# kimwin2/ORB_SLAM2v2-1

Hardware: AMD Instinct MI355X
Metric: frames/s ORB extract+match @1241x376 8-lvl 1000-feat (higher is better)
Workload: dtype u8; 1 GPU; kitti_stereo_1241x376_1000feat; frame=stereo pair (2 images), width=1241, height=376, nlevels=8, nfeatures=1000, ini_th_fast=20, min_th_fast=7, clock_ramp_steps=200, match=Frame::ComputeStereoMatches, parallelism=frames sharded over 1 GPU(s), world_size_observed=1, gauss_flavour=half_up

## Files before the change

include/orbx_dev.h:

```cpp
#ifndef ORBX_DEV_H
#define ORBX_DEV_H
#include "orbx.h"
#ifdef __cplusplus
extern "C" {
#endif

int orbx_debug_level_points(orbx_extractor_t *h, int b, int level, int stage, int32_t *out_xys, int cap,
                            int *n_out);

int orbx_debug_blur_patches(orbx_extractor_t *h, int enable, uint8_t *out, int n);
int orbx_debug_octree_fallbacks(orbx_extractor_t *h, int32_t *out, int n);
int orbx_debug_blurred_level(orbx_extractor_t *h, int b, int level, uint8_t *dst, int dst_stride, unsigned *mask_out);
int orbm_debug_features_in_area(const orbx_keypoint_t *kun, int n, const orbm_grid_geom_t *g, float x, float y, float r,
                                int min_level, int max_level, int32_t *out_idx, int *n_out, int device);
int orbx_debug_sincosf(const float *angles, int n, float *sin_out, float *cos_out, int device);

#define ORBM_PATH_RES_NONE 0
#define ORBM_PATH_RES_PAR_Q2 1
#define ORBM_PATH_RES_PAR_Q4 2
#define ORBM_PATH_RES_WAVE 3
#define ORBM_PATH_RES_EXACT 4
#define ORBM_PATH_FB_NONE 0
#define ORBM_PATH_FB_N 1
#define ORBM_PATH_FB_INIT_SIZE 2
#define ORBM_PATH_FB_CAND_CAP 3
#define ORBM_PATH_FB_QK 4
#define ORBM_PATH_FB_LDS 5
#define ORBM_PATH_FB_OPTION 6
int orbm_debug_match_path(int64_t *out);
int orbm_debug_resolve_plan(int mode, int m, int n, int device, int64_t *out);
int orbm_debug_stereo_path(int32_t *out);

#define ORBX_DEBUG_PLAN_INPUT_INTS 64
#define ORBX_DEBUG_CHUNK_PLAN_INTS 43
int orbx_debug_plan_chunk(const int32_t *in, int n_in, int32_t *out, int n_out);
int orbx_debug_last_plan(const orbx_extractor_t *h, int32_t *out, int n_out);

#define ORBX_DEBUG_SIZE_PLAN_INTS 176
int orbx_debug_size_plan(int nfeatures, float scale_factor, int nlevels, int w, int h, int pyr_tile, float *tables, int32_t *nfeat_umax,
                         uint8_t *geom, int geom_bytes, int32_t *tab, int tab_cap, int64_t *scalars, int n_scalars);

#define ORBM_DEBUG_THREAD_SCRATCH_INTS 9
int orbm_debug_thread_scratch(int64_t *out, int n_out);

int orbx_debug_set_alloc_fill(int enable, uint32_t word);
int orbx_debug_alloc_fill_stats(int64_t out[2]);

int orbx_debug_stall_stream(void *stream, int microseconds, int device);
int orbx_debug_streams(orbx_extractor_t *h, void **out, int n_out);

#ifdef __cplusplus
}
#endif
#endif
```

orb_slam2v2-1_amd/__init__.py:

```python
import ctypes as C
import os
import numpy as np

_HERE = os.path.dirname(os.path.abspath(__file__))
LIB_PATH = os.environ.get("ORBX_LIB") or os.path.join(_HERE, "lib", "liborbx_hip.so")
DEV_LIB_PATH = os.path.join(_HERE, "lib", "liborbx_hip_dev.so")
default_developer = False

KP_DTYPE = np.dtype([("x", "<f4"), ("y", "<f4"), ("size", "<f4"), ("angle", "<f4"),
                     ("response", "<f4"), ("octave", "<i4"), ("class_id", "<i4")])
MP_DTYPE = np.dtype([("in_view", "<i4"), ("proj_x", "<f4"), ("proj_y", "<f4"), ("proj_xr", "<f4"),
                     ("level", "<i4"), ("view_cos", "<f4"), ("observations", "<i4")])
LASTPT_DTYPE = np.dtype([("has_mp", "<i4"), ("wx", "<f4"), ("wy", "<f4"), ("wz", "<f4"),
                         ("observations", "<i4"), ("octave", "<i4"), ("angle", "<f4")])
WINDOW_DTYPE = np.dtype([("valid", "<i4"), ("u", "<f4"), ("v", "<f4"), ("radius", "<f4"), ("min_level", "<i4"),
                         ("max_level", "<i4"), ("angle", "<f4"), ("blocks", "<i4"), ("ur_c", "<f4"), ("ur_tol", "<f4")])

CLOUD_DTYPE = np.dtype([("x", "<f4"), ("y", "<f4"), ("z", "<f4"), ("b", "u1"), ("g", "u1"), ("r", "u1"), ("a", "u1")])

OCTREE_LEAF_DTYPE = np.dtype([("kx", "<u2"), ("ky", "<u2"), ("kz", "<u2"), ("depth", "<u2")])
OCTOMAP_AXIS_SWAP = np.array([[0, 0, 1, 0], [-1, 0, 0, 0], [0, -1, 0, 0], [0, 0, 0, 1]], np.float32)
POSE_OBS_DTYPE = np.dtype([("valid", "<i4"), ("u", "<f4"), ("v", "<f4"), ("ur", "<f4"), ("inv_sigma2", "<f4"),
                           ("wx", "<f4"), ("wy", "<f4"), ("wz", "<f4")])
POSE_WORLDPOS_DTYPE = np.dtype([("valid", "<i4"), ("wx", "<f4"), ("wy", "<f4"), ("wz", "<f4")])
POSE_INFO_DTYPE = np.dtype({"names": ["correspondences", "bad", "iterations", "trials", "rounds", "t", "q"],
                            "formats": ["<i4", "<i4", ("<i4", 4), ("<i4", 4), "<i4", ("<f8", 3), ("<f8", 4)],
                            "offsets": [0, 4, 8, 24, 40, 48, 72], "itemsize": 104})
INIT_INFO_DTYPE = np.dtype([("SH", "<f4"), ("SF", "<f4"), ("RH", "<f4"), ("model", "<i4"), ("best_iteration", "<i4", (2,)),
                            ("inliers", "<i4", (2,)), ("best_good", "<i4"), ("second_good", "<i4"), ("parallax", "<f4"), ("ncand", "<i4"),
                            ("ngood", "<i4", (8,)), ("cand_parallax", "<f4", (8,)), ("H21", "<f4", (9,)), ("F21", "<f4", (9,))])
SIM3_PAIR_DTYPE = np.dtype([("w1", "<f4", (3,)), ("w2", "<f4", (3,)), ("sigma2_1", "<f4"), ("sigma2_2", "<f4")])
SIM3_PROBLEM_DTYPE = np.dtype([("Tcw1", "<f4", (16,)), ("Tcw2", "<f4", (16,)), ("K1", "<f4", (4,)), ("K2", "<f4", (4,)),
                               ("fix_scale", "<i4"), ("min_inliers", "<i4")])
SIM3_INFO_DTYPE = np.dtype([("n", "<i4"), ("iterations", "<i4"), ("hit_iteration", "<i4"), ("best_iteration", "<i4"),
                            ("best_inliers", "<i4"), ("s", "<f4"), ("R", "<f4", (9,)), ("t", "<f4", (3,)), ("T12", "<f4", (16,))])
SIM3OPT_MATCH_DTYPE = np.dtype([("w1", "<f4", (3,)), ("w2", "<f4", (3,)), ("u1", "<f4"), ("v1", "<f4"), ("u2", "<f4"), ("v2", "<f4"),
                                ("inv_sigma2_1", "<f4"), ("inv_sigma2_2", "<f4")])
SIM3OPT_PROBLEM_DTYPE = np.dtype([("Tcw1", "<f4", (16,)), ("Tcw2", "<f4", (16,)), ("K1", "<f4", (4,)), ("K2", "<f4", (4,)), ("s", "<f4"),
                                  ("R", "<f4", (9,)), ("t", "<f4", (3,)), ("th2", "<f4"), ("fix_scale", "<i4")])
SIM3OPT_INFO_DTYPE = np.dtype([("correspondences", "<i4"), ("bad", "<i4"), ("rounds", "<i4"), ("iterations", "<i4", (2,)),
                               ("trials", "<i4", (2,)), ("reserved", "<i4"), ("q", "<f8", (4,)), ("t", "<f8", (3,)), ("s", "<f8")])
LBA_KEYFRAME_DTYPE = np.dtype([("Tcw", "<f4", (16,)), ("fx", "<f4"), ("fy", "<f4"), ("cx", "<f4"), ("cy", "<f4"), ("bf", "<f4"), ("fixed", "<i4")])
LBA_POINT_DTYPE = np.dtype([("x", "<f4"), ("y", "<f4"), ("z", "<f4")])
LBA_OBSERVATION_DTYPE = np.dtype([("kf", "<i4"), ("pt", "<i4"), ("u", "<f4"), ("v", "<f4"), ("ur", "<f4"), ("inv_sigma2", "<f4")])
LBA_SCHEDULE_DTYPE = np.dtype([("rounds", "<i4"), ("iterations", "<i4", (2,)), ("robust", "<i4", (2,)), ("delta_mono", "<f4"), ("delta_stereo", "<f4"),
                               ("classify", "<i4"), ("check_stop_first", "<i4")])
LBA_INFO_DTYPE = np.dtype([("rounds", "<i4"), ("iterations", "<i4", (2,)), ("trials", "<i4", (2,)), ("free_poses", "<i4", (2,)), ("stopped_at", "<i4"),
                           ("stop_poll", "<i4"), ("polls", "<i4"), ("erased", "<i4")])
LBA_STOP_BEFORE, LBA_STOP_ROUND1, LBA_STOP_BETWEEN, LBA_STOP_ROUND2 = 1, 2, 3, 4
LBA_MAX_ITERATIONS = 100
EG_SIM3_DTYPE = np.dtype([("q", "<f8", (4,)), ("t", "<f8", (3,)), ("s", "<f8")])
EG_VERTEX_DTYPE = np.dtype([("Scw", EG_SIM3_DTYPE), ("Snc", EG_SIM3_DTYPE), ("has_nc", "<i4"), ("fixed", "<i4")])
EG_EDGE_DTYPE = np.dtype([("i", "<i4"), ("j", "<i4"), ("kind", "<i4")])
EG_POINT_DTYPE = np.dtype([("x", "<f4"), ("y", "<f4"), ("z", "<f4"), ("ref", "<i4")])
EG_MAX_ITERATIONS = 64
EG_INFO_DTYPE = np.dtype([("iterations", "<i4"), ("trials", "<i4"), ("end", "<i4"), ("free_vertices", "<i4"), ("blocks", "<i4"), ("levels", "<i4"),
                          ("launches", "<i4"), ("pad", "<i4"), ("chi2_first", "<f8"), ("chi2_last", "<f8"), ("trials_it", "<i4", (EG_MAX_ITERATIONS,))])
EG_END_ITERATIONS, EG_END_QMAX, EG_END_RHO0, EG_END_SOLVER, EG_END_NBAD = 0, 1, 2, 3, 4
NEWPOINT_VIEW_DTYPE = np.dtype([("Tcw", "<f4", (16,)), ("Ow", "<f4", (3,)), ("fx", "<f4"), ("fy", "<f4"), ("cx", "<f4"), ("cy", "<f4"),
                                ("invfx", "<f4"), ("invfy", "<f4"), ("mb", "<f4"), ("mbf", "<f4"), ("scale_factor", "<f4"), ("nlevels", "<i4")])
NEWPOINT_STEREO_DTYPE = np.dtype([("ur", "<f4"), ("depth", "<f4"), ("raw_u", "<f4"), ("raw_v", "<f4")])
NEWPOINT_DTYPE = np.dtype([("x", "<f4"), ("y", "<f4"), ("z", "<f4"), ("status", "<i4"), ("cos_rays", "<f4"), ("cos_stereo", "<f4"),
                           ("reserved", "<i4", (2,))])
NEWPOINT_TRIANGULATED, NEWPOINT_STEREO1, NEWPOINT_STEREO2 = 0, 1, 2
NEWPOINT_MAX_LEVELS = 16
PNP_CORR_DTYPE = np.dtype([("w", "<f4", (3,)), ("u", "<f4"), ("v", "<f4"), ("sigma2", "<f4")])
PNP_PROBLEM_DTYPE = np.dtype([("K", "<f4", (4,)), ("th2", "<f4"), ("min_inliers", "<i4"), ("max_iterations", "<i4"),
                              ("iterations_done", "<i4"), ("prior_best_inliers", "<i4")])
PNP_INFO_DTYPE = np.dtype([("n", "<i4"), ("iterations", "<i4"), ("hit_iteration", "<i4"), ("iterations_run", "<i4"),
                           ("best_iteration", "<i4"), ("best_inliers", "<i4"), ("refined_inliers", "<i4"), ("no_more", "<i4"),
                           ("pose", "<i4"), ("Tcw", "<f4", (16,)), ("best_Tcw", "<f4", (16,))])
PNP_POSE_NONE, PNP_POSE_REFINED, PNP_POSE_BEST, PNP_POSE_PRIOR_BEST = 0, 1, 2, 3
DB_HIT_DTYPE = np.dtype([("kf_id", "<i4"), ("words", "<i4"), ("flags", "<u4"), ("score", "<f4"), ("acc_score", "<f4"), ("best_kf", "<i4")])
DB_MAX_KF_ID, DB_MAX_QUERY, DB_MAX_COVISIBLE = (1 << 20) - 1, 8192, 10

ORBX_OK, ORBX_ERR_ARG, ORBX_ERR_NO_DEVICE, ORBX_ERR_HIP, ORBX_ERR_CAPACITY, ORBX_ERR_UNSUPPORTED = 0, -1, -2, -3, -4, -5
NUM_STAGES = 5

EXPORTS = [
    "orbx_create", "orbx_destroy", "orbx_get_levels", "orbx_get_scale_factor", "orbx_get_tables",
    "orbx_max_keypoints", "orbx_extract", "orbx_extract_batch", "orbx_extract_batch_device",
    "orbx_pyramid_host", "orbx_pyramid_device", "orbx_level_counts", "orbx_set_profiling",
    "orbx_get_stage_ms", "orbx_create_flavoured", "orbx_get_flavour", "orbx_set_option", "orbx_get_option", "orbm_set_thread_option", "orbm_hamming", "orbm_hamming_matrix_device", "orbm_stereo_batch_device",
    "orbm_stereo", "orbm_search_for_initialization", "orbm_search_by_projection_mp",
    "orbm_search_by_projection_frame", "orbm_match_windows", "orbm_best_in_windows", "orbm_distinctive_descriptors", "orbm_predict_scale_thresholds", "orbm_is_in_frustum",
    "orbm_search_local_points", "orbv_create", "orbv_load_text", "orbv_destroy", "orbv_info", "orbv_transform",
    "orbm_search_by_bow", "orbm_search_for_triangulation", "orbx_last_error", "orbx_version", "orbx_device_count",
    "orbx_record_bytes", "orbx_pack_records_device", "orbx_thread_release_scratch",
    "orbm_search_by_projection_frame_device", "orbm_search_local_points_device", "orbx_fast_kernels", "orbx_extract_batch_device_prefetch", "orbx_stream_wait_fast_stage", "orbx_side_stream", "orbm_stereo_batch_device_prev",
    "orbx_side_stream_for", "orbx_stereo_frame", "orbx_set_pyramid_buffers",
    "orbx_stereo_frame_view", "orbx_host_alloc", "orbx_host_free",
    "orbx_gray_from_color_device", "orbm_rgbd_batch_device", "orbx_rgbd_frame",
    "orbx_rectifier_create", "orbx_rectifier_destroy", "orbx_rectifier_maps", "orbx_rectifier_info", "orbx_rectify_device",
    "orbx_stereo_frame_rectified", "orbx_stereo_frame_view_rectified",
    "orbx_cloudmapper_create", "orbx_cloudmapper_destroy", "orbx_cloud_capacity", "orbx_cloud_generate_device",
    "orbx_cloud_voxel_device", "orbx_keyframe_cloud",
    "orbx_octree_device", "orbx_octomap_bt", "orbx_octomap_bytes_bound",
    "orbv_score_l1", "orbv_db_create", "orbv_db_destroy", "orbv_db_add", "orbv_db_erase", "orbv_db_clear", "orbv_db_set_covisible",
    "orbv_db_info", "orbv_db_score", "orbv_db_detect_loop", "orbv_db_detect_reloc",
]
POSE_EXPORTS = ["orbo_pose_optimization", "orbo_pose_optimization_batch", "orbo_pose_optimization_device"]
INIT_EXPORTS = ["orbi_initialize", "orbi_initialize_device", "orbi_search"]
SIM3_EXPORTS = ["orbs_sim3_iterations", "orbs_sim3_ransac", "orbs_sim3_ransac_batch"]
PNP_EXPORTS = ["orbp_pnp_parameters", "orbp_pnp_ransac", "orbp_pnp_ransac_batch"]
SIM3OPT_EXPORTS = ["orbz_optimize_sim3", "orbz_optimize_sim3_batch"]
NEWPOINTS_EXPORTS = ["orbl_triangulate", "orbl_triangulate_batch", "orbl_baseline_ok", "orbl_compute_f12", "orbl_create_new_map_points"]
LBA_EXPORTS = ["orbb_optimize", "orbb_local_bundle_adjustment", "orbb_bundle_adjustment"]
ESSENTIAL_EXPORTS = ["orbg_optimize_essential_graph"]
DEV_EXPORTS = ["orbx_debug_level_points", "orbx_debug_sincosf", "orbx_debug_blur_patches", "orbm_debug_features_in_area",
               "orbx_debug_blurred_level", "orbx_debug_octree_fallbacks", "orbm_debug_match_path", "orbm_debug_resolve_plan",
               "orbm_debug_stereo_path", "orbx_debug_plan_chunk", "orbx_debug_last_plan", "orbm_debug_thread_scratch",
               "orbx_debug_size_plan", "orbx_debug_set_alloc_fill", "orbx_debug_alloc_fill_stats", "orbx_debug_stall_stream",
               "orbx_debug_streams"]
SIZE_PLAN_FIELDS = ["max_kp", "totalCells", "maxNodeCap", "lvlKpCap", "pyrImgBytes", "slotsPerImg", "keysPerImg", "fastTileStride", "fastScoreStride",
                    "fastTileRows", "fastLdsPerWave", "totalStrips", "stripLevels", "octLdsBytes", "octPyrLdsBytes", "octPyrWords", "octBigMask",
                    "octDeepMax", "octSliceStride", "histStride", "pyrTilesX", "pyrTilesY", "pyrXSpanOff", "pyrYSpanOff", "pyrBufBytes", "pyrMaxDim",
                    "pyrMaxPar", "pyrLdsBytes", "nChains0", "nChains1", "tabWords"]
LEVEL_GEOM_DTYPE = np.dtype([("w", "<i4"), ("h", "<i4"), ("pstride", "<i4"), ("prows", "<i4"), ("poff", "<u8"), ("regW", "<i4"), ("regH", "<i4"),
                             ("nCols", "<i4"), ("nRows", "<i4"), ("wCell", "<i4"), ("hCell", "<i4"), ("cellBase", "<i4"), ("ncells", "<i4"),
                             ("capc", "<i4"), ("pad_", "<i4"), ("slotOff", "<u8"), ("N", "<i4"), ("nIni", "<i4"), ("nodeCap", "<i4"),
                             ("pyrDepth", "<i4"), ("keyOff", "<u8"), ("keyCap", "<i4"), ("lvlKpOff", "<i4"), ("xofsOff", "<i4"), ("xalphaOff", "<i4"),
                             ("yofsOff", "<i4"), ("ybetaOff", "<i4"), ("rootTabOff", "<i4"), ("rootBoxOff", "<i4"), ("xPathOff", "<i4"),
                             ("yPathOff", "<i4"), ("scale", "<f4"), ("size", "<f4")])
THREAD_SCRATCH_FIELDS = ["arena_cap", "arena_device", "arena_seq", "arena_stream", "arena_word", "stage_cap", "stage_device", "bow_cap",
                         "bow_device"]
PLAN_INPUT_FIELDS = ["B", "nl", "totalStrips", "stripLevels", "octBigMask", "lastChunks", "prof", "profFast", "skipPyr", "pfUsed", "evPyrDone",
                     "dbgBlur", "sliceScratch", "fastTileStride", "fastScoreStride", "sparseRecent"]
CHUNK_PLAN_FIELDS = ["usePyr", "strips", "stripLevels", "fastCells", "es", "histOct", "multiWg", "fused", "gather", "bigMask", "wideOct", "compact",
                     "sparseForm", "sparsePerCell", "rowFlags", "sparseHint", "earlyLv", "aSplit", "octForm", "sweepSlices", "sweepShared",
                     "orderKernel", "fastDoneAt", "fastPhase", "octPhase", "octStop", "descLdsPad"]
OCT_EXACT, OCT_BIG, OCT_EARLY, OCT_SPLIT, OCT_SINGLE = 0, 1, 2, 3, 4
HINT_NONE, HINT_OCT_SRC, HINT_GATHER = 0, 1, 2
RES_NONE, RES_PAR_Q2, RES_PAR_Q4, RES_WAVE, RES_EXACT = 0, 1, 2, 3, 4
FB_NONE, FB_N, FB_INIT_SIZE, FB_CAND_CAP, FB_QK, FB_LDS, FB_OPTION = 0, 1, 2, 3, 4, 5, 6


class OrbxError(RuntimeError):
    def __init__(self, status, msg):
        super().__init__("orbx status %d: %s" % (status, msg))
        self.status = status


class StereoView(C.Structure):
    _fields_ = [("nl", C.c_int32), ("nr", C.c_int32), ("nmatch", C.c_int32), ("cap", C.c_int32),
                ("kl", C.c_void_p), ("kr", C.c_void_p), ("dl", C.c_void_p), ("dr", C.c_void_p), ("uright", C.c_void_p), ("depth", C.c_void_p),
                ("d_kl", C.c_void_p), ("d_kr", C.c_void_p), ("d_dl", C.c_void_p), ("d_dr", C.c_void_p), ("d_uright", C.c_void_p),
                ("d_depth", C.c_void_p)]


class OctreeInfo(C.Structure):
    _fields_ = [("points_in", C.c_int64), ("points_dropped", C.c_int64), ("cells", C.c_int64), ("leaves", C.c_int64),
                ("tree_size", C.c_int64), ("data_bytes", C.c_int64), ("overflow", C.c_int32), ("reserved", C.c_int32)]

    def as_dict(self):
        return {f: int(getattr(self, f)) for f, _ in self._fields_ if f != "reserved"}


class GridGeom(C.Structure):
    _fields_ = [("min_x", C.c_float), ("min_y", C.c_float), ("max_x", C.c_float), ("max_y", C.c_float),
                ("inv_w", C.c_float), ("inv_h", C.c_float)]


class Camera(C.Structure):
    _fields_ = [("fx", C.c_float), ("fy", C.c_float), ("cx", C.c_float), ("cy", C.c_float),
                ("mbf", C.c_float), ("mb", C.c_float)]


class RGBDCamera(C.Structure):
    _fields_ = [("fx", C.c_float), ("fy", C.c_float), ("cx", C.c_float), ("cy", C.c_float), ("k1", C.c_float), ("k2", C.c_float),
                ("p1", C.c_float), ("p2", C.c_float), ("k3", C.c_float), ("mbf", C.c_float)]


DEPTH_U16, DEPTH_F32 = 2, 5
_DEPTH_TYPES = {np.dtype(np.uint16): DEPTH_U16, np.dtype(np.float32): DEPTH_F32}


def grid_geom(w, h):
    g = GridGeom()
    g.min_x, g.min_y, g.max_x, g.max_y = 0.0, 0.0, float(w), float(h)
    g.inv_w = np.float32(64) / np.float32(w)
    g.inv_h = np.float32(48) / np.float32(h)
    return g


class Flavour(C.Structure):
    _fields_ = [("gauss_rounding", C.c_int32), ("gauss_taps", C.c_int32 * 4), ("reserved", C.c_int32 * 3)]


GAUSS_FLAVOURS = {"half_up": 0, "sse2": 1}
GAUSS_FIXED_TAPS = 2


def parse_gauss(g):
    fl = Flavour()
    if isinstance(g, str) and g.startswith("taps:"):
        taps = [int(v) for v in g[5:].split(",")]
        if len(taps) != 4:
            raise ValueError("bad gauss flavour %r (taps:k0,k1,k2,k3)" % (g,))
        fl.gauss_rounding = GAUSS_FIXED_TAPS
        for i, v in enumerate(taps):
            fl.gauss_taps[i] = v
    elif g in GAUSS_FLAVOURS:
        fl.gauss_rounding = GAUSS_FLAVOURS[g]
    else:
        raise ValueError("bad gauss flavour %r" % (g,))
    return fl
default_gauss_flavour = os.environ.get("ORBX_TEST_GAUSS_FLAVOUR", "half_up")
_default_options = {}
_live = None


def set_default_option(key, value):
    if value:
        _default_options[int(key)] = int(value)
    else:
        _default_options.pop(int(key), None)
    for e in list(_live or ()):
        if getattr(e, "_h", None):
            e.set_option(key, value)


_lib = None
_dev_lib = None


def build(force=False):
    from . import build as _b
    return _b.build(force=force)


def _preload_shared_hip_runtime():
    import importlib.util
    import sys
    if "torch" in sys.modules:
        return
    try:
        spec = importlib.util.find_spec("torch")
    except (ImportError, ValueError):
        spec = None
    if spec and spec.submodule_search_locations:
        cand = os.path.join(list(spec.submodule_search_locations)[0], "lib", "libamdhip64.so")
        if os.path.exists(cand):
            try:
                C.CDLL(cand, mode=C.RTLD_GLOBAL)
            except OSError:
                pass


def lib(developer=False):
    global _lib, _dev_lib
    if developer:
        if _dev_lib is None:
            _dev_lib = _load(DEV_LIB_PATH, True)
        return _dev_lib
    if _lib is None:
        _lib = _load(LIB_PATH, os.path.basename(LIB_PATH) == "liborbx_hip_dev.so")
    return _lib


LBA_STOP_FN = C.CFUNCTYPE(C.c_int, C.c_void_p)


def matcher_lib():
    return lib(default_developer)


def _load(path, dev):
    if not os.path.exists(path):
        raise OrbxError(ORBX_ERR_NO_DEVICE, "HIP library %s is missing: run `python __graft_entry__.py` "
                                            "(build()) first; there is no CPU fallback" % path)
    _preload_shared_hip_runtime()
    L = C.CDLL(path)
    vp, i32, f32, sz = C.c_void_p, C.c_int, C.c_float, C.c_size_t
    L.orbx_create.restype = i32
    L.orbx_create.argtypes = [i32, f32, i32, i32, i32, i32, C.POINTER(vp)]
    L.orbx_destroy.argtypes = [vp]
    L.orbx_create_flavoured.argtypes = [i32, f32, i32, i32, i32, i32, C.POINTER(Flavour), C.POINTER(vp)]
    L.orbx_get_flavour.argtypes = [vp, C.POINTER(Flavour)]
    L.orbx_set_option.argtypes = [vp, i32, i32]
    L.orbx_get_option.argtypes = [vp, i32, C.POINTER(i32)]
    L.orbm_set_thread_option.argtypes = [i32, i32]
    L.orbx_get_levels.argtypes = [vp]
    L.orbx_get_scale_factor.restype = f32
    L.orbx_get_scale_factor.argtypes = [vp]
    L.orbx_get_tables.argtypes = [vp, vp, vp, vp, vp, vp, vp]
    L.orbx_max_keypoints.argtypes = [vp]
    L.orbx_extract.argtypes = [vp, vp, i32, i32, i32, vp, vp, i32, C.POINTER(i32)]
    L.orbx_extract_batch.argtypes = [vp, vp, i32, i32, i32, i32, vp, vp, i32, vp]
    L.orbx_extract_batch_device.argtypes = [vp, vp, i32, i32, i32, i32, sz, vp, vp, vp, i32, vp]
    L.orbx_extract_batch_device_prefetch.argtypes = [vp, vp, i32, i32, i32, i32, sz, vp]
    L.orbx_stream_wait_fast_stage.argtypes = [vp, vp]
    L.orbx_side_stream.argtypes = [vp]
    L.orbx_side_stream.restype = vp
    L.orbx_stereo_frame.argtypes = [vp, vp, vp, i32, i32, i32, f32, f32, i32, vp, vp, C.POINTER(i32), vp, vp, C.POINTER(i32), vp, vp,
                                    C.POINTER(i32)]
    L.orbx_stereo_frame_view.argtypes = [vp, vp, vp, i32, i32, i32, f32, f32, vp]
    L.orbx_gray_from_color_device.argtypes = [vp, i32, i32, i32, i32, i32, i32, sz, vp, i32, sz, vp]
    L.orbm_rgbd_batch_device.argtypes = [vp, vp, i32, i32, vp, i32, i32, i32, i32, sz, f32, C.POINTER(RGBDCamera), vp, vp, vp, vp]
    L.orbx_rgbd_frame.argtypes = [vp, vp, i32, i32, i32, i32, i32, vp, i32, i32, f32, C.POINTER(RGBDCamera), i32, vp, vp,
                                  C.POINTER(i32), vp, vp, vp]
    L.orbx_rectifier_create.argtypes = [vp, vp, i32, vp, vp, i32, i32, i32, C.POINTER(vp)]
    L.orbx_rectifier_destroy.argtypes = [vp]
    L.orbx_rectifier_maps.argtypes = [vp, vp, vp]
    L.orbx_rectifier_info.argtypes = [vp, C.POINTER(i32), C.POINTER(i32), C.POINTER(sz)]
    L.orbx_rectify_device.argtypes = [vp, vp, i32, vp, i32, i32, i32, i32, i32, i32, sz, vp, i32, sz, vp]
    L.orbx_stereo_frame_rectified.argtypes = [vp, vp, vp, vp, vp, i32, i32, i32, i32, i32, f32, f32, i32, vp, vp, C.POINTER(i32), vp, vp,
                                              C.POINTER(i32), vp, vp, C.POINTER(i32)]
    L.orbx_stereo_frame_view_rectified.argtypes = [vp, vp, vp, vp, vp, i32, i32, i32, i32, i32, f32, f32, vp]
    L.orbx_cloudmapper_create.argtypes = [f32, i32, i32, i32, C.POINTER(vp)]
    L.orbx_cloudmapper_destroy.argtypes = [vp]
    L.orbx_cloud_capacity.argtypes = [i32, i32, i32]
    L.orbx_cloud_generate_device.argtypes = [vp, vp, i32, i32, sz, f32, vp, i32, i32, sz, i32, i32, i32, f32, f32, f32, f32, vp, vp, i32, vp, vp]
    L.orbx_cloud_voxel_device.argtypes = [vp, vp, vp, i32, i32, vp, i32, vp, vp]
    L.orbx_keyframe_cloud.argtypes = [vp, vp, i32, i32, vp, i32, i32, f32, i32, i32, f32, f32, f32, f32, vp, i32, vp, C.POINTER(i32), vp,
                                      C.POINTER(i32)]
    L.orbx_octree_device.argtypes = [vp, vp, vp, i32, i32, vp, C.c_double, vp, C.c_int64, vp, C.c_int64, vp, vp]
    L.orbx_octomap_bt.argtypes = [vp, vp, i32, vp, C.c_double, vp, sz, C.POINTER(sz), C.POINTER(OctreeInfo)]
    L.orbx_octomap_bytes_bound.argtypes = [C.c_int64]
    L.orbx_octomap_bytes_bound.restype = sz
    L.orbx_host_alloc.argtypes = [sz]
    L.orbx_host_alloc.restype = vp
    L.orbx_host_free.argtypes = [vp]
    L.orbx_host_free.restype = None
    L.orbx_set_pyramid_buffers.argtypes = [vp, i32]
    L.orbx_side_stream_for.argtypes = [vp, vp]
    L.orbx_side_stream_for.restype = vp
    L.orbx_pyramid_host.argtypes = [vp, i32, i32, i32, vp, i32, C.POINTER(i32), C.POINTER(i32)]
    L.orbx_pyramid_device.argtypes = [vp, i32, i32, C.POINTER(vp), C.POINTER(i32), C.POINTER(i32), C.POINTER(i32)]
    L.orbx_level_counts.argtypes = [vp, i32, vp, vp]
    L.orbx_set_profiling.argtypes = [vp, i32]
    L.orbx_fast_kernels.argtypes = [vp, i32, C.POINTER(i32), C.POINTER(i32), C.POINTER(i32)]
    L.orbx_record_bytes.argtypes = [i32]
    L.orbx_pack_records_device.argtypes = [vp, vp, vp, vp, vp, i32, i32, vp, vp]
    L.orbx_get_stage_ms.argtypes = [vp, vp, C.POINTER(i32)]
    L.orbm_hamming.argtypes = [vp, vp]
    L.orbm_hamming_matrix_device.argtypes = [vp, i32, vp, i32, vp, vp]
    L.orbm_stereo_batch_device.argtypes = [vp, vp, i32, i32, i32, vp, vp, vp, vp, vp, vp, i32, f32, f32, vp, vp, vp, vp]
    L.orbm_stereo_batch_device_prev.argtypes = L.orbm_stereo_batch_device.argtypes
    L.orbm_stereo.argtypes = [vp, vp, vp, vp, i32, vp, vp, i32, f32, f32, vp, vp, C.POINTER(i32)]
    L.orbm_search_for_initialization.argtypes = [vp, vp, i32, vp, vp, i32, C.POINTER(GridGeom), vp, vp, i32, f32,
                                                 i32, i32, C.POINTER(i32)]
    L.orbm_search_by_projection_mp.argtypes = [vp, vp, vp, i32, C.POINTER(GridGeom), vp, i32, vp, vp, i32, vp, vp,
                                               f32, f32, i32, C.POINTER(i32)]
    L.orbm_search_by_projection_frame.argtypes = [vp, vp, vp, i32, C.POINTER(GridGeom), vp, i32, C.POINTER(Camera),
                                                  vp, vp, vp, vp, i32, vp, vp, f32, i32, i32, i32, C.POINTER(i32)]
    L.orbm_search_by_projection_frame_device.argtypes = L.orbm_search_by_projection_frame.argtypes + [vp]
    L.orbm_match_windows.argtypes = [vp, vp, vp, i32, C.POINTER(GridGeom), C.POINTER(GridGeom), vp, vp, i32, vp, vp, i32, i32, i32, C.POINTER(i32)]
    L.orbm_distinctive_descriptors.argtypes = [vp, vp, i32, vp, vp, i32]
    L.orbm_predict_scale_thresholds.argtypes = [f32, i32, vp]
    L.orbv_create.argtypes = [i32, i32, i32, i32, i32, vp, vp, vp, vp, i32, C.POINTER(vp)]
    L.orbv_load_text.argtypes = [C.c_char_p, i32, C.POINTER(vp)]
    L.orbv_destroy.argtypes = [vp]
    L.orbv_destroy.restype = None
    L.orbv_info.argtypes = [vp] + [C.POINTER(i32)] * 6
    L.orbv_transform.argtypes = [vp, vp, i32, i32, vp, vp, vp]
    L.orbv_score_l1.argtypes = [vp, vp, i32, vp, vp, i32, vp]
    L.orbv_db_create.argtypes = [i32, i32, i32, C.POINTER(vp)]
    L.orbv_db_destroy.argtypes = [vp]
    L.orbv_db_destroy.restype = None
    L.orbv_db_add.argtypes = [vp, i32, vp, vp, i32]
    L.orbv_db_erase.argtypes = [vp, i32]
    L.orbv_db_clear.argtypes = [vp]
    L.orbv_db_set_covisible.argtypes = [vp, i32, vp, i32]
    L.orbv_db_info.argtypes = [vp, C.POINTER(i32), C.POINTER(C.c_int64), C.POINTER(C.c_int64), C.POINTER(sz)]
    L.orbv_db_score.argtypes = [vp, vp, vp, i32, vp, i32, vp]
    L.orbv_db_detect_loop.argtypes = [vp, vp, vp, i32, vp, i32, f32, vp, i32, C.POINTER(i32), vp, i32, C.POINTER(i32)]
    L.orbv_db_detect_reloc.argtypes = [vp, vp, vp, i32, vp, i32, C.POINTER(i32), vp, i32, C.POINTER(i32)]
    L.orbm_search_for_triangulation.argtypes = [vp, vp, vp, i32, vp, vp, vp, i32, vp, vp, vp, vp, i32, vp, f32, f32, vp, vp, i32, i32, i32, vp,
                                                C.POINTER(i32), i32]
    L.orbm_search_by_bow.argtypes = [vp, vp, vp, i32, vp, vp, vp, i32, vp, vp, vp, vp, i32, i32, f32, i32, vp, C.POINTER(i32), i32]
    L.orbm_is_in_frustum.argtypes = [vp, i32, vp, C.POINTER(Camera), C.POINTER(GridGeom), f32, vp, i32, vp, i32]
    L.orbm_search_local_points.argtypes = [vp, vp, vp, i32, C.POINTER(GridGeom), vp, i32, vp, vp, i32, vp, C.POINTER(Camera), f32,
                                           vp, vp, vp, f32, f32, i32, C.POINTER(i32), vp]
    L.orbm_search_local_points_device.argtypes = L.orbm_search_local_points.argtypes + [vp]
    L.orbo_pose_optimization.argtypes = [vp, i32, C.POINTER(Camera), vp, vp, vp, C.POINTER(i32), vp, i32]
    L.orbo_pose_optimization_batch.argtypes = [vp, vp, i32, vp, vp, vp, vp, vp, vp, i32]
    L.orbo_pose_optimization_device.argtypes = [vp, vp, i32, vp, i32, vp, C.POINTER(Camera), vp, vp, vp, C.POINTER(i32), vp, i32, vp]
    L.orbm_best_in_windows.argtypes = [vp, vp, vp, i32, C.POINTER(GridGeom), C.POINTER(GridGeom), vp, vp, i32, vp, i32, vp, vp, i32]
    L.orbi_initialize.argtypes = [vp, i32, vp, i32, vp, i32, vp, i32, vp, f32, f32, i32, C.POINTER(i32), vp, vp, vp, vp, vp, i32]
    L.orbi_initialize_device.argtypes = L.orbi_initialize.argtypes + [vp]
    L.orbi_search.argtypes = [vp, i32, vp, i32, vp, i32, vp, i32, f32, vp, vp, vp, vp, i32]
    L.orbs_sim3_iterations.argtypes = [i32, C.c_double, i32, i32]
    L.orbs_sim3_ransac.argtypes = [vp, i32, vp, vp, i32, vp, vp, vp, vp, vp, i32]
    L.orbs_sim3_ransac_batch.argtypes = [vp, vp, i32, vp, vp, vp, vp, vp, vp, vp, vp, i32]
    L.orbz_optimize_sim3.argtypes = [vp, i32, vp, vp, vp, C.POINTER(i32), vp, i32]
    L.orbz_optimize_sim3_batch.argtypes = [vp, vp, i32, vp, vp, vp, vp, vp, i32]
    L.orbl_triangulate.argtypes = [vp, vp, vp, i32, vp, vp, vp, vp, vp, i32, vp, vp, vp, i32, vp, C.POINTER(i32), i32]
    L.orbl_triangulate_batch.argtypes = [vp, vp, i32, vp, vp, vp, vp, i32]
    L.orbl_baseline_ok.argtypes = [vp, vp, i32, f32]
    L.orbl_compute_f12.argtypes = [vp, vp, vp, vp, vp]
    L.orbl_create_new_map_points.argtypes = [vp, vp, vp, vp, i32, i32, i32, i32, vp, vp, vp, vp, vp, vp, i32]
    L.orbb_optimize.argtypes = [vp, i32, vp, i32, vp, i32, vp, LBA_STOP_FN, vp, vp, vp, vp, vp, vp, vp, i32]
    L.orbb_local_bundle_adjustment.argtypes = [vp, i32, vp, i32, vp, i32, LBA_STOP_FN, vp, vp, vp, vp, vp, vp, vp, i32]
    L.orbb_bundle_adjustment.argtypes = [vp, i32, vp, i32, vp, i32, i32, i32, LBA_STOP_FN, vp, vp, vp, vp, vp, vp, i32]
    L.orbg_optimize_essential_graph.argtypes = [vp, i32, vp, i32, vp, i32, i32, i32, vp, vp, vp, vp, i32]
    L.orbp_pnp_parameters.argtypes = [i32, C.c_double, i32, i32, i32, f32, C.POINTER(i32), C.POINTER(i32)]
    L.orbp_pnp_ransac.argtypes = [vp, i32, vp, vp, i32, vp, vp, vp, vp, vp, vp, vp, vp, vp, vp, i32]
    L.orbp_pnp_ransac_batch.argtypes = [vp, vp, i32, vp, vp, vp, vp, vp, vp, vp, vp, vp, vp, vp, vp, vp, i32]
    if dev:
        L.orbx_debug_level_points.argtypes = [vp, i32, i32, i32, vp, i32, C.POINTER(i32)]
        L.orbx_debug_sincosf.argtypes = [vp, i32, vp, vp, i32]
        L.orbx_debug_blur_patches.argtypes = [vp, i32, vp, i32]
        L.orbx_debug_octree_fallbacks.argtypes = [vp, vp, i32]
        L.orbx_debug_blurred_level.argtypes = [vp, i32, i32, vp, i32, vp]
        L.orbm_debug_features_in_area.argtypes = [vp, i32, C.POINTER(GridGeom), f32, f32, f32, i32, i32, vp, C.POINTER(i32), i32]
        L.orbm_debug_match_path.argtypes = [vp]
        L.orbm_debug_resolve_plan.argtypes = [i32, i32, i32, i32, vp]
        L.orbm_debug_stereo_path.argtypes = [vp]
        L.orbx_debug_plan_chunk.argtypes = [vp, i32, vp, i32]
        L.orbx_debug_last_plan.argtypes = [vp, vp, i32]
        L.orbm_debug_thread_scratch.argtypes = [vp, i32]
        L.orbx_debug_size_plan.argtypes = [i32, f32, i32, i32, i32, i32, vp, vp, vp, i32, vp, i32, vp, i32]
        L.orbx_debug_set_alloc_fill.argtypes = [i32, C.c_uint32]
        L.orbx_debug_alloc_fill_stats.argtypes = [vp]
        L.orbx_debug_stall_stream.argtypes = [vp, i32, i32]
        L.orbx_debug_streams.argtypes = [vp, vp, i32]
    L.orbx_last_error.restype = C.c_char_p
    L.orbx_version.restype = C.c_char_p
    L._orbx_developer = bool(dev)
    return L


def _check(rc, L=None):
    if rc != 0:
        raise OrbxError(rc, (L or matcher_lib()).orbx_last_error().decode())


def _p(a):
    return a.ctypes.data if a is not None else None


def blur_reach_mask():
    d = np.abs(np.arange(-18, 19))
    t = np.where(d > 0, 2 * d - 1, 0)
    return (t[:, None] ** 2 + t[None, :] ** 2) <= 4 * 340


def device_count():
    return lib().orbx_device_count()


class ORBextractor:

    def __init__(self, nfeatures, scaleFactor, nlevels, iniThFAST, minThFAST, device=0, gauss=None, developer=None):
        global _live
        self._L = lib(default_developer if developer is None else developer)
        h = C.c_void_p()
        self.gauss = default_gauss_flavour if gauss is None else gauss
        fl = parse_gauss(self.gauss)
        self._ck(self._L.orbx_create_flavoured(int(nfeatures), float(scaleFactor), int(nlevels), int(iniThFAST),
                                             int(minThFAST), int(device), C.byref(fl), C.byref(h)))
        self._h = h
        self.nfeatures, self.nlevels, self.device = int(nfeatures), int(nlevels), int(device)
        self._shape = None
        if _live is None:
            import weakref
            _live = weakref.WeakSet()
        _live.add(self)
        for k, v in _default_options.items():
            self.set_option(k, v)

    def _ck(self, rc):
        _check(rc, self._L)

    def _hooks(self):
        if not self._L._orbx_developer:
            raise OrbxError(ORBX_ERR_ARG, "stage hooks (debug_*) exist in the developer build only: ORBextractor(..., developer=True)")

    def level_counts(self, b=0):
        c, k = np.zeros(self.nlevels, np.int32), np.zeros(self.nlevels, np.int32)
        self._ck(self._L.orbx_level_counts(self._h, int(b), _p(c), _p(k)))
        return c, k

    def set_option(self, key, value):
        self._ck(self._L.orbx_set_option(self._h, int(key), int(value)))

    def get_option(self, key):
        v = C.c_int(0)
        self._ck(self._L.orbx_get_option(self._h, int(key), C.byref(v)))
        return v.value

    def flavour(self):
        fl = Flavour()
        self._ck(self._L.orbx_get_flavour(self._h, C.byref(fl)))
        if fl.gauss_rounding == GAUSS_FIXED_TAPS:
            return "taps:" + ",".join(str(int(v)) for v in fl.gauss_taps)
        return {v: k for k, v in GAUSS_FLAVOURS.items()}[fl.gauss_rounding]

    def close(self):
        if getattr(self, "_h", None):
            self._L.orbx_destroy(self._h)
            self._h = None

    def __del__(self):
        try:
            self.close()
        except Exception:
            pass

    def GetLevels(self):
        return self._L.orbx_get_levels(self._h)

    def GetScaleFactor(self):
        return self._L.orbx_get_scale_factor(self._h)

    def _tables(self):
        n = self.nlevels
        t = [np.zeros(n, np.float32) for _ in range(4)] + [np.zeros(n, np.int32), np.zeros(16, np.int32)]
        self._ck(self._L.orbx_get_tables(self._h, *[_p(a) for a in t]))
        return t

    def GetScaleFactors(self): return self._tables()[0]
    def GetInverseScaleFactors(self): return self._tables()[1]
    def GetScaleSigmaSquares(self): return self._tables()[2]
    def GetInverseScaleSigmaSquares(self): return self._tables()[3]
    @property
    def mnFeaturesPerLevel(self): return self._tables()[4]
    @property
    def umax(self): return self._tables()[5]

    def max_keypoints(self):
        return self._L.orbx_max_keypoints(self._h)

    def __call__(self, image):
        image = np.asarray(image)
        if image.size == 0:
            return np.zeros(0, KP_DTYPE), np.zeros((0, 32), np.uint8)
        assert image.dtype == np.uint8 and image.ndim == 2, "CV_8UC1 expected (:1050)"
        if image.strides[1] != 1 or image.strides[0] < image.shape[1]:
            image = np.ascontiguousarray(image)
        h, w = image.shape
        cap = max(self.nfeatures + 8 * self.nlevels, 64) + 260
        kps = np.zeros(cap, KP_DTYPE)
        desc = np.zeros((cap, 32), np.uint8)
        n = C.c_int(0)
        self._ck(self._L.orbx_extract(self._h, _p(image), w, h, image.strides[0], _p(kps), _p(desc), cap, C.byref(n)))
        self._shape = (h, w)
        return kps[:n.value].copy(), desc[:n.value].copy()

    def extract_batch(self, images):
        images = np.ascontiguousarray(images, dtype=np.uint8)
        B, h, w = images.shape
        cap = max(self.nfeatures + 8 * self.nlevels, 64) + 260
        kps = np.zeros((B, cap), KP_DTYPE)
        desc = np.zeros((B, cap, 32), np.uint8)
        n = np.zeros(B, np.int32)
        ptrs = (C.c_void_p * B)(*[images[b].ctypes.data for b in range(B)])
        self._ck(self._L.orbx_extract_batch(self._h, C.cast(ptrs, C.c_void_p), B, w, h, w, _p(kps), _p(desc), cap, _p(n)))
        self._shape = (h, w)
        return [(kps[b, :n[b]].copy(), desc[b, :n[b]].copy()) for b in range(B)]

    def extract_batch_device(self, d_imgs, B, w, h, stride, image_stride, d_kps, d_desc, d_counts, cap, stream=0):
        self._ck(self._L.orbx_extract_batch_device(self._h, d_imgs, B, w, h, stride, image_stride, d_kps, d_desc,
                                                 d_counts, cap, stream))
        self._shape = (h, w)

    def prefetch_batch_device(self, d_imgs, B, w, h, stride, image_stride, side_stream=0):
        self._ck(self._L.orbx_extract_batch_device_prefetch(self._h, d_imgs, B, w, h, stride, image_stride, side_stream))

    def side_stream(self):
        return self._L.orbx_side_stream(self._h)

    def stereo_frame(self, left, right, mbf, mb):
        left = np.ascontiguousarray(left, np.uint8); right = np.ascontiguousarray(right, np.uint8)
        assert left.shape == right.shape and left.ndim == 2
# ... 106 lines not shown
        self._ck(self._L.orbx_stereo_frame_view_rectified(self._h, _rect_handle(rect_left), _rect_handle(rect_right), la[0], ra[0],
                                                          int(ch), int(bool(rgb)), w, hgt, w * ch if stride is None else int(stride),
                                                          float(mbf), float(mb), C.byref(v)))
        self._shape = (hgt, w)
        a, b = v.nl, v.nr
        view = lambda p, n, dt: np.frombuffer((C.c_char * (n * np.dtype(dt).itemsize)).from_address(p), dt) if n > 0 else np.zeros(0, dt)
        return {"kl": view(v.kl, a, KP_DTYPE), "dl": view(v.dl, a * 32, np.uint8).reshape(a, 32), "kr": view(v.kr, b, KP_DTYPE),
                "dr": view(v.dr, b * 32, np.uint8).reshape(b, 32), "uright": view(v.uright, a, np.float32),
                "depth": view(v.depth, a, np.float32), "nmatch": v.nmatch, "view": v}

    def set_pyramid_buffers(self, n):
        self._ck(self._L.orbx_set_pyramid_buffers(self._h, int(n)))

    def side_stream_for(self, main_stream):
        return self._L.orbx_side_stream_for(self._h, main_stream)

    def stream_wait_fast_stage(self, stream):
        self._ck(self._L.orbx_stream_wait_fast_stage(self._h, stream))

    def pyramid_level(self, level, b=0, padded=False):
        w, h = C.c_int(), C.c_int()
        self._ck(self._L.orbx_pyramid_host(self._h, b, level, int(padded), None, 0, C.byref(w), C.byref(h)))
        out = np.zeros((h.value, w.value), np.uint8)
        self._ck(self._L.orbx_pyramid_host(self._h, b, level, int(padded), _p(out), w.value, C.byref(w), C.byref(h)))
        return out

    @property
    def mvImagePyramid(self):
        return [self.pyramid_level(l) for l in range(self.nlevels)]

    def pyramid_device(self, level, b=0):
        ptr, w, h, s = C.c_void_p(), C.c_int(), C.c_int(), C.c_int()
        self._ck(self._L.orbx_pyramid_device(self._h, b, level, C.byref(ptr), C.byref(w), C.byref(h), C.byref(s)))
        return ptr.value, w.value, h.value, s.value

    def debug_level_points(self, level, stage, b=0):
        self._hooks()
        n = C.c_int()
        self._ck(self._L.orbx_debug_level_points(self._h, b, level, stage, None, 0, C.byref(n)))
        out = np.zeros((max(n.value, 1), 3), np.int32)
        if n.value:
            self._ck(self._L.orbx_debug_level_points(self._h, b, level, stage, _p(out), n.value, C.byref(n)))
        return out[:n.value]

    def fast_kernels(self, B):
        st, ce, ipl = C.c_int(0), C.c_int(0), C.c_int(0)
        self._ck(self._L.orbx_fast_kernels(self._h, int(B), C.byref(st), C.byref(ce), C.byref(ipl)))
        self.fast_images_per_launch = ipl.value
        return [n for n, f in (("k_fast_strips", st.value), ("k_fast_cells", ce.value)) if f]

    def octree_fallbacks(self, B=1):
        self._hooks()
        out = np.zeros((B, self.nlevels), np.int32)
        self._ck(self._L.orbx_debug_octree_fallbacks(self._h, _p(out), B * self.nlevels))
        return out

    def blurred_mask(self):
        m = C.c_uint()
        self._ck(self._L.orbx_debug_blurred_level(self._h, 0, 0, None, 0, C.byref(m)))
        return m.value

    def blurred_level(self, level, b=0):
        self._hooks()
        w, h = C.c_int(), C.c_int()
        self._ck(self._L.orbx_pyramid_host(self._h, b, level, 0, None, 0, C.byref(w), C.byref(h)))
        out = np.zeros((h.value, w.value), np.uint8)
        self._ck(self._L.orbx_debug_blurred_level(self._h, b, level, _p(out), w.value, None))
        return out

    def debug_blur_patches(self, image):
        self._hooks()
        self._ck(self._L.orbx_debug_blur_patches(self._h, 1, None, 0))
        try:
            k, d = self(image)
            out = np.zeros((max(len(k), 1), 37, 37), np.uint8)
            if len(k):
                self._ck(self._L.orbx_debug_blur_patches(self._h, 1, _p(out), len(k)))
        finally:
            self._L.orbx_debug_blur_patches(self._h, 0, None, 0)
        return k, d, out[:len(k)]

    def debug_last_plan(self):
        self._hooks()
        out = np.zeros(len(CHUNK_PLAN_FIELDS) + 16, np.int32)
        self._ck(self._L.orbx_debug_last_plan(self._h, _p(out), len(out)))
        return _plan_dict(out)

    def set_profiling(self, mode=1):
        self._ck(self._L.orbx_set_profiling(self._h, int(mode)))

    def stage_ms(self):
        ms = np.zeros(NUM_STAGES, np.float32)
        n = C.c_int(0)
        self._ck(self._L.orbx_get_stage_ms(self._h, _p(ms), C.byref(n)))
        return ms, n.value


def debug_features_in_area(kun, geom, x, y, r, min_level=-1, max_level=-1, device=0):
    kun = np.ascontiguousarray(kun, KP_DTYPE)
    out = np.zeros(max(len(kun), 1), np.int32)
    n = C.c_int(0)
    _check(lib(True).orbm_debug_features_in_area(_p(kun), len(kun), C.byref(geom), float(x), float(y), float(r), int(min_level),
                                             int(max_level), _p(out), C.byref(n), int(device)), lib(True))
    return out[:n.value].copy()


def debug_match_path():
    out = np.zeros(3, np.int64)
    _check(lib(True).orbm_debug_match_path(_p(out)), lib(True))
    return int(out[0]), int(out[1]), int(out[2])


def debug_resolve_plan(mode, m, n, device=0):
    out = np.zeros(4, np.int64)
    _check(lib(True).orbm_debug_resolve_plan(int(mode), int(m), int(n), int(device), _p(out)), lib(True))
    return tuple(int(v) for v in out)


def _plan_dict(out):
    d = {k: int(v) for k, v in zip(CHUNK_PLAN_FIELDS, out)}
    d["nslice"] = tuple(int(v) for v in out[len(CHUNK_PLAN_FIELDS):])
    return d


def debug_plan_chunk(ncells=(), opt=None, **fields):
    a = np.zeros(len(PLAN_INPUT_FIELDS) + 16 + 32, np.int32)
    for k, v in fields.items():
        a[PLAN_INPUT_FIELDS.index(k)] = int(v)
    a[len(PLAN_INPUT_FIELDS):len(PLAN_INPUT_FIELDS) + len(ncells)] = ncells
    for k, v in (opt or {}).items():
        a[len(PLAN_INPUT_FIELDS) + 16 + int(k)] = int(v)
    out = np.zeros(len(CHUNK_PLAN_FIELDS) + 16, np.int32)
    rc = lib(True).orbx_debug_plan_chunk(_p(a), len(a), _p(out), len(out))
    return rc, _plan_dict(out)


def debug_size_plan(nfeatures, scale_factor, nlevels, w, h, tile=0):
    L = lib(True)
    tables, nu = np.zeros((4, 16), np.float32), np.zeros(32, np.int32)
    geom, sc = np.zeros(16, LEVEL_GEOM_DTYPE), np.zeros(len(SIZE_PLAN_FIELDS) + 17 + 128, np.int64)
    tab = np.zeros(0, np.int32)
    for _ in range(2):
        rc = L.orbx_debug_size_plan(nfeatures, scale_factor, nlevels, w, h, tile, _p(tables), _p(nu), _p(geom), geom.nbytes, _p(tab), len(tab),
                                    _p(sc), len(sc))
        if rc != ORBX_OK or len(tab) == sc[SIZE_PLAN_FIELDS.index("tabWords")]:
            break
        tab = np.zeros(int(sc[SIZE_PLAN_FIELDS.index("tabWords")]), np.int32)
    d = dict(status=rc, message=L.orbx_last_error().decode() if rc else "", sf=tables[0], isf=tables[1], sig2=tables[2], isig2=tables[3],
             nfeat=nu[:16], umax=nu[16:])
    if rc == ORBX_OK:
        n = len(SIZE_PLAN_FIELDS)
        d.update({k: int(v) for k, v in zip(SIZE_PLAN_FIELDS, sc)}, geom=geom, tab=tab, stripBase=sc[n:n + 17].astype(np.int32),
                 chains=sc[n + 17:].astype(np.int32).reshape(2, 8, 8))
    return d


def debug_thread_scratch():
    out = np.zeros(len(THREAD_SCRATCH_FIELDS), np.int64)
    _check(lib(True).orbm_debug_thread_scratch(_p(out), len(out)), lib(True))
    return {k: int(v) for k, v in zip(THREAD_SCRATCH_FIELDS, out)}


def debug_set_alloc_fill(enable, word=0):
    _check(lib(True).orbx_debug_set_alloc_fill(int(bool(enable)), int(word) & 0xFFFFFFFF), lib(True))


def debug_alloc_fill_stats():
    out = np.zeros(2, np.int64)
    _check(lib(True).orbx_debug_alloc_fill_stats(_p(out)), lib(True))
    return int(out[0]), int(out[1])


def debug_stall_stream(stream, microseconds, device=0):
    _check(lib(True).orbx_debug_stall_stream(int(stream) if stream else None, int(microseconds), int(device)), lib(True))


DEBUG_STREAM_FIELDS = ("main", "side0", "side1", "arena", "staging")


def debug_streams(extractor=None):
    if extractor is not None:
        extractor._hooks()
    out = (C.c_void_p * 5)()
    _check(lib(True).orbx_debug_streams(extractor._h if extractor is not None else None, out, 5), lib(True))
    return {k: int(v or 0) for k, v in zip(DEBUG_STREAM_FIELDS, out)}


def debug_stereo_path():
    out = np.zeros(4, np.int32)
    _check(lib(True).orbm_debug_stereo_path(_p(out)), lib(True))
    return tuple(int(v) for v in out)


def debug_sincosf(angles, device=0):
    a = np.ascontiguousarray(angles, np.float32)
    s, c = np.zeros_like(a), np.zeros_like(a)
    _check(lib(True).orbx_debug_sincosf(_p(a), len(a), _p(s), _p(c), int(device)), lib(True))
    return s, c


def pack_records_device(d_kps, d_desc, d_uright, d_depth, d_counts, B, cap, d_records, stream=0):
    _check(lib().orbx_pack_records_device(d_kps, d_desc, d_uright, d_depth, d_counts, B, cap, d_records, stream))


def stereo_batch_device(ex_left, ex_right, B, left_slot0, right_slot0, d_kl, d_dl, d_nl, d_kr, d_dr, d_nr, cap,
                        mbf, mb, d_uright, d_depth, d_nmatch, stream=0, prev=False):
    L = ex_left._L
    fn = L.orbm_stereo_batch_device_prev if prev else L.orbm_stereo_batch_device
    _check(fn(ex_left._h, ex_right._h, B, left_slot0, right_slot0, d_kl, d_dl, d_nl, d_kr, d_dr, d_nr, cap, float(mbf), float(mb),
              d_uright, d_depth, d_nmatch, stream), L)


def gray_from_color_device(d_color, B, w, h, channels, rgb, stride, image_stride, d_gray, gray_stride, gray_image_stride, stream=0):
    _check(lib().orbx_gray_from_color_device(d_color, int(B), int(w), int(h), int(channels), int(bool(rgb)), int(stride), int(image_stride),
                                             d_gray, int(gray_stride), int(gray_image_stride), stream))


def rgbd_batch_device(d_kps, d_counts, B, cap, d_depth, depth_type, w, h, depth_stride, depth_image_stride, depth_map_factor, cam,
                      d_kun, d_uright, d_depth_out, stream=0):
    _check(lib().orbm_rgbd_batch_device(d_kps, d_counts, int(B), int(cap), d_depth or None, int(depth_type), int(w), int(h),
                                        int(depth_stride), int(depth_image_stride), float(depth_map_factor), C.byref(cam), d_kun,
                                        d_uright, d_depth_out, stream))


class StereoRectifier:

    def __init__(self, K, D, R, P, w, h, device=0):
        self._L = lib()
        self._r = None
        K = np.ascontiguousarray(np.asarray(K, np.float64).reshape(3, 3))
        R = np.ascontiguousarray(np.asarray(R, np.float64).reshape(3, 3))
        P = np.asarray(P, np.float64)
        assert P.shape in ((3, 3), (3, 4)), "P: 3x3 or 3x4"
        P = np.ascontiguousarray(P[:, :3])
        D = np.ascontiguousarray(np.asarray(D, np.float64).ravel())
        r = C.c_void_p()
        _check(self._L.orbx_rectifier_create(_p(K), _p(D) if D.size else None, int(D.size), _p(R), _p(P), int(w), int(h), int(device),
                                             C.byref(r)), self._L)
        self._r = r
        self.w, self.h, self.device = int(w), int(h), int(device)

    @property
    def handle(self):
        return self._r.value

    def maps(self):
        mx, my = np.zeros((self.h, self.w), np.float32), np.zeros((self.h, self.w), np.float32)
        _check(self._L.orbx_rectifier_maps(self._r, _p(mx), _p(my)), self._L)
        return mx, my

    def info(self):
        t, g, b = C.c_int(), C.c_int(), C.c_size_t()
        _check(self._L.orbx_rectifier_info(self._r, C.byref(t), C.byref(g), C.byref(b)), self._L)
        return {"tiles": t.value, "gather_tiles": g.value, "device_bytes": b.value}

    def close(self):
        if self._r:
            self._L.orbx_rectifier_destroy(self._r)
            self._r = None

    def __del__(self):
        try:
            self.close()
        except Exception:
            pass


def _rect_handle(r):
    return None if r is None else (r.handle if isinstance(r, StereoRectifier) else r)


def rectify_device(r0, r1, B0, d_src, B, sw, sh, channels, rgb, stride, image_stride, d_gray, gray_stride, gray_image_stride, stream=0):
    _check(lib().orbx_rectify_device(_rect_handle(r0), _rect_handle(r1), int(B0), d_src, int(B), int(sw), int(sh), int(channels),
                                     int(bool(rgb)), int(stride), int(image_stride), d_gray, int(gray_stride), int(gray_image_stride),
                                     stream), lib())


def cloud_capacity(w, h, step=3):
    return lib().orbx_cloud_capacity(int(w), int(h), int(step))


class CloudMapper:

    def __init__(self, leaf=0.1, step=3, alpha=255, device=0):
        self._L = lib()
        self._m = None
        m = C.c_void_p()
        _check(self._L.orbx_cloudmapper_create(float(leaf), int(step), int(alpha), int(device), C.byref(m)), self._L)
        self._m = m
        self.leaf, self.step, self.alpha, self.device = float(np.float32(leaf)), int(step), int(alpha), int(device)

    def close(self):
        if self._m:
            self._L.orbx_cloudmapper_destroy(self._m)
            self._m = None

    def __del__(self):
        try:
            self.close()
        except Exception:
            pass

    def capacity(self, w, h):
        return self._L.orbx_cloud_capacity(int(w), int(h), self.step)

    def generate_device(self, d_depth, depth_type, depth_stride, depth_image_stride, depth_map_factor, d_color, channels, color_stride,
# ... 1020 lines not shown
```

orb_slam2v2-1_amd/build.py:

```python
import os
import subprocess
import sys

HERE = os.path.dirname(os.path.abspath(__file__))
ROOT = os.path.dirname(HERE)
CSRC = os.path.join(HERE, "csrc")
LIB = os.path.join(HERE, "lib", "liborbx_hip.so")
SOURCES = ["orbx_extract.hip", "orbx_pyramid.hip", "orbx_fast.hip", "orbx_octree.hip", "orbx_octree_wide.hip", "orbx_describe.hip",
           "orbx_match.hip", "orbx_match_fast.hip", "orbx_bow.hip", "orbx_rgbd.hip", "orbx_rectify.hip", "orbx_cloud.hip", "orbx_octomap.hip", "orbx_kfdb.hip", "orbx_poseopt.hip", "orbx_initializer.hip", "orbx_sim3.hip", "orbx_pnp.hip", "orbx_sim3opt.hip", "orbx_newpoints.hip", "orbx_lba.hip", "orbx_essential.hip"]
FLAGS = ["--offload-arch=gfx950", "-O3", "-ffp-contract=off", "-std=c++17", "-fPIC", "-shared",
         "-Wall", "-Wno-unused-value", "-Wno-unused-result"]


def needs_build():
    return _stale(LIB) or _stale(DEV_LIB)


HOST = os.path.join(HERE, "host")
HOST_LIB = os.path.join(HERE, "lib", "liborb_host.so")


def build_host(force=False, verbose=False):
    srcs = [os.path.join(HOST, f) for f in ("ORBextractor.cc", "ORBmatcher.cc", "ORBVocabulary.cc", "PointCloudMapping.cc", "KeyFrameDatabase.cc", "Optimizer.cc", "Initializer.cc", "Sim3Solver.cc", "PnPsolver.cc", "LocalMapping.cc")]
    deps = srcs + [os.path.join(HOST, f) for f in os.listdir(HOST)] + [LIB]
    if not force and os.path.exists(HOST_LIB) and all(os.path.getmtime(d) <= os.path.getmtime(HOST_LIB) for d in deps):
        return HOST_LIB
    cmd = ["g++", "-std=c++11", "-O2", "-Wall", "-fPIC", "-shared", "-I" + os.path.join(ROOT, "include"), "-I" + HOST,
           "-o", HOST_LIB] + srcs + ["-L" + os.path.dirname(LIB), "-lorbx_hip", "-Wl,-rpath,$ORIGIN"]
    if verbose:
        print(" ".join(cmd))
    subprocess.check_call(cmd)
    return HOST_LIB


DEV_LIB = os.path.join(HERE, "lib", "liborbx_hip_dev.so")
OBJ = os.path.join(HERE, "lib", "obj")


def _deps():
    return [os.path.join(CSRC, f) for f in os.listdir(CSRC)] + [
        os.path.join(ROOT, "include", f) for f in ("orbx.h", "orbx_dev.h", "orb_pattern_31.inc")]


def _compile_link(out, defines, verbose):
    from concurrent.futures import ThreadPoolExecutor
    hipcc = os.environ.get("HIPCC", "/opt/rocm/bin/hipcc")
    tag = "dev" if defines else "rel"
    os.makedirs(OBJ, exist_ok=True)
    cflags = [f for f in FLAGS if f != "-shared"] + defines + ["-I" + os.path.join(ROOT, "include"), "-I" + CSRC]
    tdep = max(os.path.getmtime(d) for d in _deps() if not d.endswith(".hip"))
    jobs = []
    for src in SOURCES:
        sp, op = os.path.join(CSRC, src), os.path.join(OBJ, src.replace(".hip", "." + tag + ".o"))
        if not os.path.exists(op) or os.path.getmtime(op) < max(os.path.getmtime(sp), tdep) or \
                (src == "orbx_octree_wide.hip" and os.path.getmtime(op) < os.path.getmtime(os.path.join(CSRC, "orbx_octree.hip"))):
            jobs.append([hipcc] + cflags + ["-c", sp, "-o", op])
    if verbose:
        for j in jobs:
            print(" ".join(j))
    with ThreadPoolExecutor(max_workers=min(8, max(1, len(jobs)))) as ex:
        for rc, j in zip(ex.map(lambda c: subprocess.call(c), jobs), jobs):
            if rc != 0:
                raise subprocess.CalledProcessError(rc, j)
    objs = [os.path.join(OBJ, s.replace(".hip", "." + tag + ".o")) for s in SOURCES]
    cmd = [hipcc, "--offload-arch=gfx950", "-shared", "-fPIC", "-o", out] + objs
    if verbose:
        print(" ".join(cmd))
    subprocess.check_call(cmd)
    return out


def _stale(lib):
    return not os.path.exists(lib) or any(os.path.getmtime(d) > os.path.getmtime(lib) for d in _deps())


def build(force=False, verbose=False):
    os.makedirs(os.path.dirname(LIB), exist_ok=True)
    if force or _stale(LIB):
        _compile_link(LIB, [], verbose)
        build_host(True, verbose)
    else:
        build_host(False, verbose)
    if force or _stale(DEV_LIB):
        _compile_link(DEV_LIB, ["-DORBX_DEVELOPER"], verbose)
    return LIB


def build_developer(verbose=False):
    if _stale(DEV_LIB):
        _compile_link(DEV_LIB, ["-DORBX_DEVELOPER"], verbose)
    return DEV_LIB


if __name__ == "__main__":
    if "--developer" in sys.argv:
        print(build_developer(verbose=True))
    else:
        build(force="--force" in sys.argv, verbose=True)
        print(LIB)
```

orb_slam2v2-1_amd/csrc/orbx_extract.hip:

```cpp
#include "orbx_extract_dev.h"
#ifdef ORBX_DEVELOPER
#include "orbx_dev.h"
#endif
#include <math.h>
#include <float.h>
#include <stdarg.h>
#include <algorithm>

static thread_local char g_err[512] = "";
void orbx_set_error(const char *fmt, ...) {
    va_list ap;
    va_start(ap, fmt);
    vsnprintf(g_err, sizeof(g_err), fmt, ap);
    va_end(ap);
}
extern "C" const char *orbx_last_error(void) { return g_err; }
extern "C" const char *orbx_version(void) { return "orbx 0.1 (gfx950)"; }
extern "C" int orbx_device_count(void) {
    int n = 0;
    if (hipGetDeviceCount(&n) != hipSuccess) return 0;
    return n;
}

extern "C" int orbx_thread_release_scratch(void) {
    orbx_internal_release_match_scratch();
    orbx_internal_release_arena();
    orbx_internal_release_bow_scratch();
    orbx_internal_release_pose_scratch();
    orbx_internal_release_init_scratch();
    orbx_internal_release_sim3_scratch();
    orbx_internal_release_pnp_scratch();
    orbx_internal_release_sim3opt_scratch();
    orbx_internal_release_newpoints_scratch();
    orbx_internal_release_lba_scratch();
    orbx_internal_release_essential_scratch();
    return ORBX_OK;
}
#ifdef ORBX_DEVELOPER
extern "C" int orbm_debug_thread_scratch(int64_t *out, int n_out) {
    if (!out || n_out != ORBM_DEBUG_THREAD_SCRATCH_INTS) { orbx_set_error("orbm_debug_thread_scratch: bad arguments"); return ORBX_ERR_ARG; }
    orbx_internal_arena_info(out);
    orbx_internal_match_scratch_info(out + 5);
    orbx_internal_bow_scratch_info(out + 7);
    return ORBX_OK;
}

static int g_fillOn = 0;
static uint32_t g_fillWord = 0;
static long long g_fillBlocks = 0, g_fillBytes = 0;
extern "C" int orbx_debug_set_alloc_fill(int enable, uint32_t word) {
    __atomic_store_n(&g_fillOn, 0, __ATOMIC_SEQ_CST);
    __atomic_store_n(&g_fillWord, word, __ATOMIC_SEQ_CST);
    __atomic_store_n(&g_fillBlocks, 0, __ATOMIC_SEQ_CST);
    __atomic_store_n(&g_fillBytes, 0, __ATOMIC_SEQ_CST);
    __atomic_store_n(&g_fillOn, enable ? 1 : 0, __ATOMIC_SEQ_CST);
    return ORBX_OK;
}
extern "C" int orbx_debug_alloc_fill_stats(int64_t out[2]) {
    if (!out) { orbx_set_error("orbx_debug_alloc_fill_stats: bad arguments"); return ORBX_ERR_ARG; }
    out[0] = __atomic_load_n(&g_fillBlocks, __ATOMIC_SEQ_CST);
    out[1] = __atomic_load_n(&g_fillBytes, __ATOMIC_SEQ_CST);
    return ORBX_OK;
}
hipError_t orbx_internal_scratch_filled(void *p, size_t bytes, bool pinned) {
    if (!__atomic_load_n(&g_fillOn, __ATOMIC_SEQ_CST) || !p || bytes == 0) return hipSuccess;
    const uint32_t word = __atomic_load_n(&g_fillWord, __ATOMIC_SEQ_CST);
    const size_t nw = bytes / 4;
    if (pinned) {
        for (size_t i = 0; i < nw; i++) ((volatile uint32_t *)p)[i] = word;
        for (size_t i = nw * 4; i < bytes; i++) ((volatile uint8_t *)p)[i] = (uint8_t)(word >> (8 * (i & 3)));
    } else {
        hipError_t e = nw ? hipMemsetD32((hipDeviceptr_t)p, (int)word, nw) : hipSuccess;
        for (size_t i = nw * 4; i < bytes && e == hipSuccess; i++) e = hipMemset((uint8_t *)p + i, (int)((word >> (8 * (i & 3))) & 255u), 1);
        if (e == hipSuccess) e = hipDeviceSynchronize();
        if (e != hipSuccess) return e;
    }
    __atomic_fetch_add(&g_fillBlocks, 1, __ATOMIC_SEQ_CST);
    __atomic_fetch_add(&g_fillBytes, (long long)bytes, __ATOMIC_SEQ_CST);
    return hipSuccess;
}
#endif

extern "C" int orbx_set_option(orbx_extractor_t *h, int key, int value) {
    static const signed char maxv[ORBX_NUM_OPTIONS] = { -1, -1, -2, 64, 3, 4, 3, -1, ORBX_MAX_CHUNKS, 1, 3, 2, 1, 2, 127, ORBX_MAX_LEVELS,
                                                        2, -2, 1, ORBX_MAX_LEVELS, 2, 40, 2, 1, 2, 3, 1, 1, -2, -2, -2, -2};
    if (!h || key < 0 || key >= ORBX_NUM_OPTIONS || maxv[key] == -2) { orbx_set_error("orbx_set_option: unknown key %d", key); return ORBX_ERR_ARG; }
#ifdef ORBX_DEVELOPER
    if (maxv[key] == -1) { if (value < 0) return ORBX_ERR_ARG; h->opt[key] = value; return ORBX_OK; }
#else
    if (maxv[key] == -1) { orbx_set_error("orbx_set_option: key %d needs a library built with -DORBX_DEVELOPER", key); return ORBX_ERR_ARG; }
#endif
    if (value < 0 || (key != ORBX_OPT_BLUR_THRESHOLD && value > maxv[key])) { orbx_set_error("orbx_set_option: key %d does not take %d", key, value); return ORBX_ERR_ARG; }
    h->opt[key] = value;
    return ORBX_OK;
}
extern "C" int orbx_get_option(const orbx_extractor_t *h, int key, int *value) {
    if (!h || !value || key < 0 || key >= ORBX_NUM_OPTIONS) return ORBX_ERR_ARG;
    *value = h->opt[key];
    return ORBX_OK;
}

extern "C" int orbx_create(int nfeatures, float scale_factor, int nlevels, int ini_th, int min_th,
                           int device, orbx_extractor_t **out) {
    return orbx_create_flavoured(nfeatures, scale_factor, nlevels, ini_th, min_th, device, nullptr, out);
}
extern "C" int orbx_get_flavour(const orbx_extractor_t *h, orbx_flavour_t *out) {
    if (!h || !out) return ORBX_ERR_ARG;
    *out = h->flavour;
    return ORBX_OK;
}
extern "C" int orbx_create_flavoured(int nfeatures, float scale_factor, int nlevels, int ini_th, int min_th,
                                     int device, const orbx_flavour_t *flavour, orbx_extractor_t **out) {
    if (!out) { orbx_set_error("orbx_create: out is NULL"); return ORBX_ERR_ARG; }
    *out = nullptr;
    if (flavour) {
        bool ok = flavour->gauss_rounding == ORBX_GAUSS_ROUND_HALF_UP || flavour->gauss_rounding == ORBX_GAUSS_ROUND_SSE2 ||
                  flavour->gauss_rounding == ORBX_GAUSS_FIXED_TAPS;
        for (int i = 0; i < 3; i++) ok = ok && flavour->reserved[i] == 0;
        const int32_t *k = flavour->gauss_taps;
        if (flavour->gauss_rounding == ORBX_GAUSS_FIXED_TAPS) {
            for (int i = 0; i < 4; i++) ok = ok && k[i] >= 0 && k[i] <= 255;
            ok = ok && k[0] >= 1 && k[0] + 2 * (k[1] + k[2] + k[3]) <= 257;
        } else
            for (int i = 0; i < 4; i++) ok = ok && k[i] == 0;
        if (!ok) {
            orbx_set_error("orbx_create_flavoured: unknown flavour (gauss_rounding=%d, gauss_taps=%d %d %d %d)", flavour->gauss_rounding, k[0], k[1], k[2], k[3]);
            return ORBX_ERR_ARG;
        }
    }
    if (nfeatures < 1 || nlevels < 1 || nlevels > ORBX_MAX_LEVELS || !(scale_factor > 1.0f) || ini_th < 0 ||
        min_th < 0 || ini_th > 255 || min_th > 255) {
        orbx_set_error("orbx_create: bad arguments (nfeatures=%d scale=%f nlevels=%d ini=%d min=%d)", nfeatures,
                       scale_factor, nlevels, ini_th, min_th);
        return ORBX_ERR_ARG;
    }
    int ndev = 0;
    hipError_t e = hipGetDeviceCount(&ndev);
    if (e != hipSuccess || ndev == 0 || device < 0 || device >= ndev) {
        orbx_set_error("orbx_create: no usable HIP device (count=%d, requested %d): %s", ndev, device,
                       e == hipSuccess ? "ok" : hipGetErrorString(e));
        return ORBX_ERR_NO_DEVICE;
    }
    ORBX_HIP(hipSetDevice(device));
    orbx_extractor *h = new orbx_extractor();
    h->nfeatures = nfeatures; h->nlevels = nlevels; h->ini_th = ini_th; h->min_th = min_th;
    h->device = device; h->scale_factor = scale_factor;
    if (flavour) h->flavour = *flavour;
    extractor_tables(nfeatures, h->scale_factor, nlevels, &h->tb);
    ORBX_HIP(hipStreamCreateWithFlags(&h->stream, hipStreamNonBlocking));
    ORBX_HIP(scratch_host_malloc((void **)&h->h_sparseSeen, sizeof(int32_t), hipHostMallocMapped | hipHostMallocCoherent));
    *h->h_sparseSeen = (int32_t)0xC0000000u;
    ORBX_HIP(hipHostGetDevicePointer((void **)&h->d_sparseSeen, h->h_sparseSeen, 0));
    for (int i = 0; i < ORBX_SIDE_STREAMS; i++) {
        ORBX_HIP(hipStreamCreateWithFlags(&h->side[i], hipStreamNonBlocking));
        ORBX_HIP(hipEventCreateWithFlags(&h->evJoin[i], hipEventDisableTiming));
    }
    for (int i = 0; i < ORBX_MAX_CHUNKS; i++) ORBX_HIP(hipEventCreateWithFlags(&h->evPyr[i], hipEventDisableTiming));
    ORBX_HIP(hipEventCreateWithFlags(&h->evFastDone, hipEventDisableTiming | hipEventDisableSystemFence));
    ORBX_HIP(hipEventCreateWithFlags(&h->evGather, hipEventDisableTiming));
    ORBX_HIP(hipEventCreateWithFlags(&h->evOctA, hipEventDisableTiming));
    ORBX_HIP(hipEventCreateWithFlags(&h->evPrefetch, hipEventDisableTiming | hipEventDisableSystemFence));
    for (int r = 0; r < ORBX_EV_RING; r++)
        for (int i = 0; i < ORBX_NUM_STAGES; i++) ORBX_HIP(hipEventCreateWithFlags(&h->ev[r][i], hipEventDisableSystemFence));
    *out = h;
    return ORBX_OK;
}

struct PlanBuffer { void **ptr; size_t bytes; bool zero; };
static std::vector<PlanBuffer> plan_buffers(orbx_extractor *h, const SizePlan &sp, int B) {
    const size_t Bz = (size_t)B, lv = (size_t)ORBX_MAX_LEVELS * Bz, slots = Bz * h->nlevels;
    const size_t hist = (size_t)ORBX_HIST_IMAGES * h->nlevels * sp.histStride;
    std::vector<PlanBuffer> v = {
        {(void **)&h->d_geom, sizeof(LevelGeom) * ORBX_MAX_LEVELS, false},
        {(void **)&h->d_tab, sizeof(int32_t) * std::max<size_t>(sp.tab.size(), 1), false},
        {(void **)&h->d_pyr, sp.pyrImgBytes * Bz, false},
        {(void **)&h->d_cellCnt, sizeof(uint32_t) * sp.totalCells * Bz, false},
        {(void **)&h->d_cellRaw, sizeof(uint32_t) * sp.totalCells * Bz, false},
        {(void **)&h->d_slots, sizeof(uint32_t) * (sp.slotsPerImg * Bz + 64), false},
        {(void **)&h->d_cand, sizeof(uint32_t) * sp.keysPerImg * Bz, false},
        {(void **)&h->d_nodeOf, sizeof(uint16_t) * sp.keysPerImg * Bz, false},
        {(void **)&h->d_candCnt, sizeof(int32_t) * lv, false},
        {(void **)&h->d_lvlCnt, sizeof(int32_t) * lv, false},
        {(void **)&h->d_sparse, sizeof(int32_t) * lv, true},
        {(void **)&h->d_lvlKp, sizeof(uint32_t) * (size_t)sp.lvlKpCap * Bz, false},
        {(void **)&h->d_octFallback, sizeof(int32_t) * lv, true},
        {(void **)&h->d_histCnt, sizeof(uint32_t) * hist, true},
        {(void **)&h->d_histBest, sizeof(uint32_t) * hist, true},
        {(void **)&h->d_octPart, sizeof(uint32_t) * slots * OCT_BIG_K * (size_t)sp.octDeepMax, false},
        {(void **)&h->d_octLeaf, sizeof(uint32_t) * slots * (size_t)sp.octPyrWords, false},
        {(void **)&h->d_octBest, sizeof(uint32_t) * slots * (size_t)sp.maxNodeCap, false},
        {(void **)&h->d_octState, sizeof(int32_t) * slots * 4, true},
    };
    if (sp.octSliceStride > 0) {
        v.push_back({(void **)&h->d_octPartBest, sizeof(uint32_t) * slots * OCT_MAX_SLICES * (size_t)sp.octSliceStride, false});
        v.push_back({(void **)&h->d_octPartCnt, sizeof(uint32_t) * slots * OCT_MAX_SLICES * (size_t)sp.octSliceStride, false});
        v.push_back({(void **)&h->d_octSliceState, sizeof(int32_t) * slots, true});
    }
    return v;
}

static void free_plan(orbx_extractor *h) {
    for (const PlanBuffer &b : plan_buffers(h, h->sp, h->pB)) { hipFree(*b.ptr); *b.ptr = nullptr; }
    hipFree(h->d_pyrAlt); h->d_pyrAlt = nullptr; h->pyrAltBytes = 0; h->pfValid = 0; h->prevPyrValid = 0;
    hipFree(h->d_pyrNext); h->d_pyrNext = nullptr; h->pyrNextBytes = 0;
    hipFree(h->d_blur); hipFree(h->d_blurAlt); h->d_blur = h->d_blurAlt = nullptr; h->blurBytes = h->blurAltBytes = 0; h->blurMaskLast = h->blurMaskAlt = 0;
    h->sp = SizePlan();
    h->pw = h->ph = h->pB = 0;
}

extern "C" int orbx_destroy(orbx_extractor_t *h) {
    if (!h) return ORBX_OK;
    hipSetDevice(h->device);
    hipStreamSynchronize(h->stream);
    if (h->last_valid) hipStreamSynchronize(h->last_stream);
    if (h->st_stream) hipStreamSynchronize(h->st_stream);
    orbx_internal_free_stereo_scratch(h);
    orbx_internal_free_rgbd_scratch(h);
    orbx_internal_free_rect_scratch(h);
    free_plan(h);
    hipFree(h->d_in); hipFree(h->d_kps); hipFree(h->d_desc); hipFree(h->d_counts); hipFree(h->d_dbgBlur);
    hipFree(h->d_sfr); if (h->h_sfr) hipHostFree(h->h_sfr);
    for (int i = 0; i < 2; i++) { hipFree(h->fv_d[i]); if (h->fv_h[i]) hipHostFree(h->fv_h[i]); }
    if (h->fv_stage) hipHostFree(h->fv_stage);
    if (h->fv_flag) hipHostFree(h->fv_flag);
    if (h->h_sparseSeen) hipHostFree(h->h_sparseSeen);
    if (h->h_kps) { hipHostFree(h->h_kps); hipHostFree(h->h_desc); hipHostFree(h->h_counts); }
    for (int r = 0; r < ORBX_EV_RING; r++)
        for (int i = 0; i < ORBX_NUM_STAGES; i++) hipEventDestroy(h->ev[r][i]);
    for (int i = 0; i < ORBX_SIDE_STREAMS; i++) { hipStreamSynchronize(h->side[i]); hipStreamDestroy(h->side[i]); hipEventDestroy(h->evJoin[i]); }
    for (int i = 0; i < ORBX_MAX_CHUNKS; i++) hipEventDestroy(h->evPyr[i]);
    hipEventDestroy(h->evFastDone); hipEventDestroy(h->evPrefetch); hipEventDestroy(h->evGather); hipEventDestroy(h->evOctA);
    hipFree(h->d_kpsB); hipFree(h->d_descB);
    hipStreamDestroy(h->stream);
    delete h;
    return ORBX_OK;
}

extern "C" int orbx_get_levels(const orbx_extractor_t *h) { return h ? h->nlevels : ORBX_ERR_ARG; }
extern "C" float orbx_get_scale_factor(const orbx_extractor_t *h) { return h ? (float)h->scale_factor : 0.f; }
extern "C" int orbx_get_tables(const orbx_extractor_t *h, float *sf, float *isf, float *s2, float *is2,
                               int32_t *nf, int32_t *umax16) {
    if (!h) return ORBX_ERR_ARG;
    for (int i = 0; i < h->nlevels; i++) {
        if (sf) sf[i] = h->tb.sf[i];
        if (isf) isf[i] = h->tb.isf[i];
        if (s2) s2[i] = h->tb.sig2[i];
        if (is2) is2[i] = h->tb.isig2[i];
        if (nf) nf[i] = h->tb.nfeat[i];
    }
    if (umax16) memcpy(umax16, h->tb.umax, sizeof(int32_t) * 16);
    return ORBX_OK;
}
extern "C" int orbx_max_keypoints(const orbx_extractor_t *h) {
    if (!h) return ORBX_ERR_ARG;
    return h->sp.max_kp > 0 ? h->sp.max_kp : h->nfeatures + 3 * h->nlevels;
}

static int ensure_plan(orbx_extractor *h, int w, int hgt, int B) {
    if (h->pw == w && h->ph == hgt && h->pB >= B) return ORBX_OK;
    SizePlan sp;
    const SizeInput in = {w, hgt, h->nlevels, h->scale_factor, h->tb, h->opt[3]};
    const int rc = plan_size(in, &sp);
    if (rc) return rc;
    ORBX_HIP(hipSetDevice(h->device));
    if (h->last_valid) ORBX_HIP(hipStreamSynchronize(h->last_stream));
    for (int i = 0; i < ORBX_SIDE_STREAMS; i++) ORBX_HIP(hipStreamSynchronize(h->side[i]));
    if (h->pw == w && h->ph == hgt) B = std::max(B, h->pB);
    free_plan(h);
    h->sp = std::move(sp);
    for (const PlanBuffer &b : plan_buffers(h, h->sp, B)) {
        ORBX_HIP(scratch_malloc(b.ptr, b.bytes));
        if (b.zero) ORBX_HIP(hipMemset(*b.ptr, 0, b.bytes));
    }
    ORBX_HIP(hipMemcpy(h->d_geom, h->sp.geom, sizeof(LevelGeom) * ORBX_MAX_LEVELS, hipMemcpyHostToDevice));
    if (!h->sp.tab.empty()) ORBX_HIP(hipMemcpy(h->d_tab, h->sp.tab.data(), sizeof(int32_t) * h->sp.tab.size(), hipMemcpyHostToDevice));
    h->pw = w; h->ph = hgt; h->pB = B;
    return ORBX_OK;
}

static int harvest_events(orbx_extractor *h, int slot) {
    hipEvent_t *ev = h->ev[slot];
    if (h->ev_pending[slot] == 2) {
        float ms = 0;
        ORBX_HIP(hipEventSynchronize(ev[2]));
        ORBX_HIP(hipEventElapsedTime(&ms, ev[1], ev[2]));
        h->acc_ms[1] += ms;
        h->acc_n++;
        h->ev_pending[slot] = 0;
        return ORBX_OK;
    }
    ORBX_HIP(hipEventSynchronize(ev[4]));
    for (int i = 0; i < 4; i++) {
        float ms = 0;
        ORBX_HIP(hipEventElapsedTime(&ms, ev[i], ev[i + 1]));
        h->acc_ms[i] += ms;
    }
    float tot = 0;
    ORBX_HIP(hipEventElapsedTime(&tot, ev[0], ev[4]));
    h->acc_ms[4] += tot;
    h->acc_n++;
    h->ev_pending[slot] = 0;
    return ORBX_OK;
}

__global__ void k_nop() {}

#define ORBX_BLUR_THR 100000000
static unsigned blur_plan(const orbx_extractor *h, BlurPlan &bp, int &totalTiles) {
    unsigned mask = 0;
    totalTiles = 0;
    const long thr = h->opt[14] > 0 ? h->opt[14] : ORBX_BLUR_THR;
    for (int l = 0; l <= ORBX_MAX_LEVELS; l++) {
        bp.tileBase[l] = totalTiles;
        if (l >= h->nlevels) continue;
        const LevelGeom &g = h->sp.geom[l];
        const bool on = h->opt[13] == 2 || (h->opt[13] == 0 && (long)g.N * 1369 * 100 >= thr * (long)g.w * g.h);
        bp.tilesX[l] = 0;
        if (!on) continue;
        mask |= 1u << l;
        const int ndw = ((g.w + ORBX_EDGE - 1) >> 2) - 4 + 1;
        bp.tilesX[l] = (ndw + 63) / 64;
        totalTiles += bp.tilesX[l] * ((g.h + BLUR_R - 1) / BLUR_R);
    }
    return mask;
}
static uint32_t gauss_taps_packed(const orbx_extractor *h) {
    if (h->flavour.gauss_rounding != ORBX_GAUSS_FIXED_TAPS) return ORBX_GAUSS_TAPS_DEFAULT;
    const int32_t *k = h->flavour.gauss_taps;
    return (uint32_t)k[3] | ((uint32_t)k[2] << 8) | ((uint32_t)k[1] << 16) | ((uint32_t)k[0] << 24);
}
static int ensure_blur(orbx_extractor *h, uint8_t **buf, size_t *bytes) {
    const size_t need = h->sp.pyrImgBytes * (size_t)h->pB;
    if (*bytes >= need) return ORBX_OK;
    if (h->last_valid) ORBX_HIP(hipStreamSynchronize(h->last_stream));
    for (int i = 0; i < ORBX_SIDE_STREAMS; i++) ORBX_HIP(hipStreamSynchronize(h->side[i]));
    hipFree(*buf); *buf = nullptr; *bytes = 0;
    ORBX_HIP(scratch_malloc(buf, need));
    *bytes = need;
    return ORBX_OK;
}
static int launch_blur(orbx_extractor *h, const uint8_t *pyr, uint8_t **blurBuf, size_t *blurBytes, int b0, int B, hipStream_t st, unsigned *maskOut) {
    BlurPlan bp;
    int tiles = 0;
    const unsigned mask = blur_plan(h, bp, tiles);
    *maskOut = mask;
    if (!mask) return ORBX_OK;
    int rc = ensure_blur(h, blurBuf, blurBytes);
    if (rc) return rc;
    const size_t off = (size_t)b0 * h->sp.pyrImgBytes;
    hipLaunchKernelGGL(k_blur_levels, dim3((tiles + 3) / 4, B), dim3(256), 0, st, pyr + off, *blurBuf + off, h->sp.pyrImgBytes, h->d_geom, h->nlevels, tiles, bp,
                       h->flavour.gauss_rounding, gauss_taps_packed(h));
    return ORBX_OK;
}

static bool pyramid_fused_all(const orbx_extractor *h) { return h->opt[5] == 1 || h->scale_factor > 3.0; }
static void launch_pyramid(orbx_extractor *h, const uint8_t *d_imgs, uint8_t *pyr, int B, int stride, size_t img_stride, hipStream_t st) {
    const int nl = h->nlevels;
    if (pyramid_fused_all(h)) {
        hipLaunchKernelGGL(k_pyramid_fused, dim3(h->sp.pyrTilesX * h->sp.pyrTilesY, B), dim3(256), h->sp.pyrLdsBytes, st, d_imgs,
                           stride, img_stride, pyr, h->sp.pyrImgBytes, h->d_geom, nl, h->d_tab, h->sp.pyrXSpanOff,
                           h->sp.pyrYSpanOff, h->sp.pyrTilesX, h->sp.pyrTilesY, h->sp.pyrBufBytes, h->sp.pyrMaxPar, 0);
        return;
    }
    const bool hybrid = h->opt[5] == 3;
    const int lastSingle = hybrid ? std::min(2, nl - 1) : nl - 1;
    const LevelGeom &g0 = h->sp.geom[0];
    const size_t padLds = (size_t)PAD_ROWS_PER_BLOCK * stride + 32;
    if ((h->opt[24] == 2 || (h->opt[24] == 0 && B <= ORBX_HIST_IMAGES)) && padLds <= 60 * 1024)
        hipLaunchKernelGGL(k_pyr_pad_rows, dim3((g0.h + PAD_ROWS_PER_BLOCK - 1) / PAD_ROWS_PER_BLOCK, B), dim3(256), padLds, st, d_imgs, stride, img_stride, pyr,
                           h->sp.pyrImgBytes, h->d_geom);
    else {
        const int pc = g0.pstride >> 4, cI0 = (ORBX_EDGE + 15) >> 4, cI1 = std::max((g0.w + ORBX_EDGE) >> 4, cI0), nI = cI1 - cI0, nE = pc - nI;
        const int threads = std::min(256, std::max(64, (nI + 63) & ~63)), gx = std::max(1, (nI + threads - 1) / threads);
        const int rowBlocks = (g0.prows + PAD_FULL_ROWS - 1) / PAD_FULL_ROWS, edgeRows = (nE * g0.prows + gx * threads - 1) / (gx * threads);
        hipLaunchKernelGGL(k_pyr_pad<true>, dim3(gx, rowBlocks + edgeRows, B), dim3(threads), 0, st, d_imgs, stride, img_stride, pyr,
                           h->sp.pyrImgBytes, h->d_geom, 0);
    }
    const int cv = h->opt[25] == 3 ? 1 : 0;
    if (h->sp.nChains[cv] > 0 && !hybrid && (h->opt[5] == 4 || (h->opt[5] == 0 && h->opt[25] != 1 && B <= ORBX_HIST_IMAGES))) {
        for (int c = 0; c < h->sp.nChains[cv]; c++) {
            const ChainPlan &cp = h->sp.chains[cv][c];
            const size_t lds = 2 * (size_t)cp.bufBytes + (size_t)(cp.lb - cp.la) * cp.maxRows * 8;
            hipLaunchKernelGGL(k_pyr_chain, dim3(cp.tilesX * cp.tilesY, B), dim3(256), lds, st, pyr, h->sp.pyrImgBytes, h->d_geom, h->d_tab, cp);
        }
        return;
    }
    for (int l = 1; l <= lastSingle; l++) {
        const int nxc = (h->sp.geom[l].w + 1 + 127) / 128, nb16 = (h->sp.geom[l].h + 15) / 16, nb8 = (h->sp.geom[l].h + 7) / 8;
        const bool tall = h->scale_factor <= 1.25f && (h->opt[22] == 0 ? (size_t)nxc * nb16 * B >= 8192 : h->opt[22] == 2);
        if (tall)
            hipLaunchKernelGGL((k_pyr_level<16, 22>), dim3((nxc * nb16 + 3) / 4, B), dim3(256), 0, st, pyr, h->sp.pyrImgBytes, h->d_geom, l, h->d_tab, nxc, nb16);
        else
            hipLaunchKernelGGL((k_pyr_level<8, 12>), dim3((nxc * nb8 + 3) / 4, B), dim3(256), 0, st, pyr, h->sp.pyrImgBytes, h->d_geom, l, h->d_tab, nxc, nb8);
    }
    if (lastSingle < nl - 1)
        hipLaunchKernelGGL(k_pyramid_fused, dim3(h->sp.pyrTilesX * h->sp.pyrTilesY, B), dim3(256), h->sp.pyrLdsBytes, st, d_imgs,
                           stride, img_stride, pyr, h->sp.pyrImgBytes, h->d_geom, nl, h->d_tab, h->sp.pyrXSpanOff,
                           h->sp.pyrYSpanOff, h->sp.pyrTilesX, h->sp.pyrTilesY, h->sp.pyrBufBytes, h->sp.pyrMaxPar, lastSingle);
}

struct ChunkView {
    const uint8_t *imgs; uint8_t *pyr; uint32_t *cellCnt, *cellRaw, *slots, *cand, *lvlKp; uint16_t *nodeOf;
    int32_t *candCnt, *lvlCnt, *octFallback, *sparse; orbx_keypoint_t *kps; uint8_t *desc; int32_t *counts;
    int b0;
    size_t octSlot0;
};
static ChunkView chunk_view(const orbx_extractor *h, const uint8_t *d_imgs, size_t img_stride, orbx_keypoint_t *d_kps, uint8_t *d_desc,
                            int32_t *d_counts, int cap, int b0) {
    ChunkView v;
    const size_t z = (size_t)b0;
    v.imgs = d_imgs + z * img_stride; v.pyr = h->d_pyr + z * h->sp.pyrImgBytes;
    v.cellCnt = h->d_cellCnt + z * h->sp.totalCells; v.cellRaw = h->d_cellRaw + z * h->sp.totalCells;
    v.slots = h->d_slots + z * h->sp.slotsPerImg; v.cand = h->d_cand + z * h->sp.keysPerImg; v.nodeOf = h->d_nodeOf + z * h->sp.keysPerImg;
    v.lvlKp = h->d_lvlKp + z * h->sp.lvlKpCap;
    v.sparse = h->d_sparse + z * h->nlevels;
    v.candCnt = h->d_candCnt + z * h->nlevels; v.lvlCnt = h->d_lvlCnt + z * h->nlevels; v.octFallback = h->d_octFallback + z * h->nlevels;
    v.kps = d_kps + z * cap; v.desc = d_desc + z * cap * 32; v.counts = d_counts + b0;
    v.octSlot0 = z * h->nlevels; v.b0 = b0;
    return v;
}

static PlanInput plan_input(const orbx_extractor *h, int B, int nch, bool prof, bool profFast, bool skipPyr, bool evPyrDone) {
    PlanInput in = {};
    in.B = B; in.nl = h->nlevels; in.totalStrips = h->sp.totalStrips; in.stripLevels = (int32_t)h->sp.stripLevels; in.octBigMask = (int32_t)h->sp.octBigMask;
    in.lastChunks = nch; in.prof = prof; in.profFast = profFast; in.skipPyr = skipPyr; in.pfUsed = h->pfUsed != 0; in.evPyrDone = evPyrDone;
    in.dbgBlur = h->d_dbgBlur != nullptr; in.sliceScratch = h->d_octPartBest != nullptr;
    in.fastTileStride = h->sp.fastTileStride; in.fastScoreStride = h->sp.fastScoreStride;
    in.sparseRecent = h->h_sparseSeen && (uint32_t)h->callSeq - (uint32_t)*(volatile int32_t *)h->h_sparseSeen <= 16u;
    for (int l = 0; l < h->nlevels; l++) in.ncells[l] = h->sp.geom[l].ncells;
    memcpy(in.opt, h->opt, sizeof(in.opt));
    return in;
}

#define ORBX_OCT_LAUNCH_ON(STREAM, KERN, KERNW, GRID, LDS, ...)                                                         \
    do {                                                                                                                \
        if (p.wideOct) {                                                                                                \
            ORBX_HIP(hipFuncSetAttribute((const void *)KERNW, hipFuncAttributeMaxDynamicSharedMemorySize, (int)(LDS))); \
            hipLaunchKernelGGL(KERNW, GRID, dim3(OCT_T_WIDE), LDS, STREAM, __VA_ARGS__);                                \
        } else {                                                                                                        \
            ORBX_HIP(hipFuncSetAttribute((const void *)KERN, hipFuncAttributeMaxDynamicSharedMemorySize, (int)(LDS)));  \
            hipLaunchKernelGGL(KERN, GRID, dim3(OCT_T), LDS, STREAM, __VA_ARGS__);                                      \
        }                                                                                                               \
    } while (0)
#define ORBX_OCT_PYR_ON(STREAM, GRID, STOP, PHASE, LV0, SRC)                                                                        \
    ORBX_OCT_LAUNCH_ON(STREAM, k_octree_pyr, k_octree_pyr_wide, GRID, ldsOct, h->d_geom, nl, v.cand, h->sp.keysPerImg, v.candCnt, v.lvlKp, \
                       h->sp.lvlKpCap, v.lvlCnt, h->d_tab, h->sp.maxNodeCap, pow2, h->sp.octPyrWords, v.octFallback, STOP, v.nodeOf, scratch,   \
                       PHASE, 0u, LV0, SRC)
#define ORBX_LAUNCH_FAST(EST, SP, LDSW)                                                                                  \
    hipLaunchKernelGGL((k_fast_cells<EST, SP>), dim3((h->sp.totalCells + FAST_WAVES - 1) / FAST_WAVES, B), dim3(64 * FAST_WAVES), \
                       (size_t)(LDSW) * FAST_WAVES, st, v.pyr, h->sp.pyrImgBytes, h->d_geom, nl, h->sp.totalCells, v.cellCnt, v.cellRaw, v.slots, \
                       h->sp.slotsPerImg, h->ini_th, h->min_th, h->sp.fastTileStride, h->sp.fastScoreStride, h->sp.fastTileRows, \
                       (LDSW), p.fastPhase, cb, (unsigned)p.stripLevels, v.sparse, (SP) ? FastHist{} : fhist)
#define ORBX_LAUNCH_FAST_ES(SP, LDSW)                         \
    switch (p.es) {                                           \
    case 44: ORBX_LAUNCH_FAST(44, SP, LDSW); break;           \
    case 48: ORBX_LAUNCH_FAST(48, SP, LDSW); break;           \
    case 52: ORBX_LAUNCH_FAST(52, SP, LDSW); break;           \
    default: ORBX_LAUNCH_FAST(0, SP, LDSW); break;            \
    }

static int launch_chunk(orbx_extractor *h, const ChunkView &v, int B, int stride, size_t img_stride, int cap, hipStream_t st,
                        hipEvent_t *ev, bool prof, bool profFast, hipEvent_t evPyrDone, bool skipPyr) {
    ChunkPlan p;
    int rc = plan_chunk(plan_input(h, B, h->lastChunks, prof, profFast, skipPyr, evPyrDone != nullptr), &p);
    if (rc) return rc;
    if (v.b0 == 0) h->lastPlan = p;
    const int nl = h->nlevels;
    CellBases cb;
    for (int l = 0; l <= ORBX_MAX_LEVELS; l++) cb.v[l] = l < nl ? h->sp.geom[l].cellBase : h->sp.totalCells;
    StripBases sb;
    for (int l = 0; l <= ORBX_MAX_LEVELS; l++) sb.v[l] = h->sp.stripBase[l];
    orbx_keypoint_t *d_kps = v.kps; uint8_t *d_desc = v.desc; int32_t *d_counts = v.counts;
    if (prof) ORBX_HIP(hipEventRecord(ev[0], st));
    if (!skipPyr) {
        launch_pyramid(h, v.imgs, v.pyr, B, stride, img_stride, st);
        unsigned m = 0;
        rc = launch_blur(h, h->d_pyr, &h->d_blur, &h->blurBytes, v.b0, B, st, &m);
        if (rc) return rc;
        h->blurMaskLast = m;
    }
    if (evPyrDone) ORBX_HIP(hipEventRecord(evPyrDone, st));
    if (p.orderKernel) hipLaunchKernelGGL(k_nop, dim3(1), dim3(64), 0, st);
    if (profFast) ORBX_HIP(hipEventRecord(ev[1], st));
    if (p.fastDoneAt == ORBX_FASTDONE_WITH_FAST) ORBX_HIP(hipEventRecord(h->evFastDone, st));
    OctSrc osrc = {};
    if (p.fused) {
        osrc.cellCnt = v.cellCnt; osrc.cellRaw = v.cellRaw; osrc.slots = v.slots; osrc.slotsPerImg = h->sp.slotsPerImg;
        osrc.totalCells = h->sp.totalCells; osrc.iniTh = h->ini_th; osrc.minTh = h->min_th; osrc.candCntOut = v.candCnt;
        osrc.sparseFlag = v.sparse; osrc.sparsePerCell = p.sparsePerCell; osrc.candOut = v.cand;
        osrc.sparseSeen = p.sparseHint == ORBX_HINT_OCT_SRC ? h->d_sparseSeen : nullptr; osrc.callSeq = h->callSeq;
        h->candStale = std::max(h->candStale, v.b0 + B);
    }
    FastHist fhist = {};
    if (p.histOct) {
        fhist.cnt = h->d_histCnt; fhist.best = h->d_histBest; fhist.stride = h->sp.histStride; fhist.tab = h->d_tab;
        osrc.histCnt = h->d_histCnt; osrc.histBest = h->d_histBest; osrc.histStride = h->sp.histStride;
    }
    int pow2 = 1;
    while (pow2 < h->sp.maxNodeCap) pow2 <<= 1;
    int maxCellsL = 0;
    for (int l = 0; l < nl; l++) maxCellsL = std::max(maxCellsL, h->sp.geom[l].ncells);
    const int scratch = std::max(4 * h->sp.maxNodeCap, maxCellsL + 1);
    const size_t ldsOct = std::max(h->sp.octPyrLdsBytes, h->sp.octLdsBytes);
    hipStream_t s2 = h->side[1];
    {
        const int32_t *spf = p.rowFlags ? v.sparse : (const int32_t *)nullptr;
        const int sA = p.earlyLv ? h->sp.stripBase[p.earlyLv] : 0;
        if (p.earlyLv) {
            hipLaunchKernelGGL(k_fast_strips, dim3((sA + FAST_WAVES - 1) / FAST_WAVES, B), dim3(64 * FAST_WAVES), 0, st,
                               v.pyr, h->sp.pyrImgBytes, h->d_geom, nl, sA, h->sp.totalCells, v.cellCnt, v.cellRaw,
                               v.slots, h->sp.slotsPerImg, h->ini_th, h->min_th, sb, spf, 0, p.compact ? 1 : 0);
            ORBX_HIP(hipEventRecord(h->evGather, st));
            ORBX_HIP(hipStreamWaitEvent(s2, h->evGather, 0));
            ORBX_OCT_PYR_ON(s2, dim3(B, p.earlyLv), 0, 0, 0, osrc);
            ORBX_HIP(hipEventRecord(h->evOctA, s2));
        }
        if (p.strips && h->sp.totalStrips > sA)
            hipLaunchKernelGGL(k_fast_strips, dim3((h->sp.totalStrips - sA + FAST_WAVES - 1) / FAST_WAVES, B), dim3(64 * FAST_WAVES), 0, st,
                               v.pyr, h->sp.pyrImgBytes, h->d_geom, nl, h->sp.totalStrips, h->sp.totalCells, v.cellCnt, v.cellRaw,
                               v.slots, h->sp.slotsPerImg, h->ini_th, h->min_th, sb, spf, sA, p.compact ? 1 : 0);
        if (p.compact && p.sparseForm == 1) {
            hipLaunchKernelGGL(k_fast_strips_sparse, dim3((h->sp.totalStrips + FAST_WAVES - 1) / FAST_WAVES, B), dim3(64 * FAST_WAVES), 0, st,
                               v.pyr, h->sp.pyrImgBytes, h->d_geom, nl, h->sp.totalStrips, h->sp.totalCells, v.cellCnt, v.cellRaw,
                               v.slots, h->sp.slotsPerImg, h->ini_th, h->min_th, sb, v.sparse);
        } else if (p.compact) {
            const int ldsw = h->sp.fastLdsPerWave + ((32 * h->sp.fastTileRows + 15) & ~15);
            ORBX_LAUNCH_FAST_ES(true, ldsw);
        }
        if (p.fastCells) ORBX_LAUNCH_FAST_ES(false, h->sp.fastLdsPerWave);
    }
    if (profFast) ORBX_HIP(hipEventRecord(ev[2], st));
    if (p.fastDoneAt == ORBX_FASTDONE_BEHIND_FAST) ORBX_HIP(hipEventRecord(h->evFastDone, st));
    {
        if (p.gather)
            hipLaunchKernelGGL(k_gather, dim3((h->sp.totalCells + GATHER_CELLS_PER_BLOCK - 1) / GATHER_CELLS_PER_BLOCK, B),
                               dim3(256), 0, st, h->d_geom, nl, h->sp.totalCells, v.cellCnt, v.cellRaw, v.slots,
                               h->sp.slotsPerImg, v.cand, h->sp.keysPerImg, v.candCnt, h->ini_th, h->min_th, cb, v.sparse, p.sparsePerCell,
                               p.sparseHint == ORBX_HINT_GATHER ? h->d_sparseSeen : (int32_t *)nullptr, h->callSeq);
        if (p.aSplit > 0) {
            const size_t need = (size_t)h->pB * cap * 60;
            if (h->splitBytes < need) {
                ORBX_HIP(hipStreamSynchronize(st));
                ORBX_HIP(hipStreamSynchronize(s2));
                hipFree(h->d_kpsB); hipFree(h->d_descB); h->d_kpsB = nullptr; h->d_descB = nullptr; h->splitBytes = 0;
                ORBX_HIP(scratch_malloc(&h->d_kpsB, (size_t)h->pB * cap * sizeof(orbx_keypoint_t)));
                ORBX_HIP(scratch_malloc(&h->d_descB, (size_t)h->pB * cap * 32));
// ... 528 lines not shown
}

extern "C" int orbx_extract(orbx_extractor_t *h, const uint8_t *img, int w, int hgt, int stride,
                            orbx_keypoint_t *kps, uint8_t *desc, int cap, int *n_out) {
    if (!h || !n_out) { orbx_set_error("orbx_extract: bad arguments"); return ORBX_ERR_ARG; }
    if (!img || w <= 0 || hgt <= 0) { *n_out = 0; return ORBX_OK; }
    const uint8_t *imgs[1] = {img};
    return orbx_extract_batch(h, imgs, 1, w, hgt, stride, kps, desc, cap, n_out);
}

int orbx_internal_level(const orbx_extractor *h, int level, int *w, int *hgt, int *pstride,
                        unsigned long long *poff) {
    if (!h || level < 0 || level >= h->nlevels || h->pw == 0) return ORBX_ERR_ARG;
    const LevelGeom &g = h->sp.geom[level];
    *w = g.w; *hgt = g.h; *pstride = g.pstride; *poff = g.poff;
    return ORBX_OK;
}

static int ensure_frames(orbx_extractor *h) {
    if (h->framesStale <= 0) return ORBX_OK;
    const int nl = h->nlevels, B = h->framesStale;
    hipStream_t st = h->last_stream;
    const LevelGeom &g1 = h->sp.geom[1];
    const int p1 = (g1.w + 2 * ORBX_EDGE + 3) >> 2, tot1 = 2 * ORBX_EDGE * p1 + g1.h * 12;
    (void)hipGetLastError();
    hipLaunchKernelGGL(k_pyr_pad<false>, dim3((tot1 + 255) / 256, nl - 1, B), dim3(256), 0, st, (const uint8_t *)nullptr, 0, (size_t)0,
                       h->d_pyr, h->sp.pyrImgBytes, h->d_geom, 1);
    ORBX_HIP(hipGetLastError());
    h->framesStale = 0;
    return ORBX_OK;
}

extern "C" int orbx_pyramid_device(orbx_extractor_t *h, int b, int level, const uint8_t **d_ptr, int *w, int *hgt,
                                   int *stride) {
    if (!h || !d_ptr || level < 0 || level >= h->nlevels || h->pw == 0 || b < 0 || b >= h->pB) {
        orbx_set_error("orbx_pyramid_device: bad arguments or no frame extracted yet");
        return ORBX_ERR_ARG;
    }
    if (level > 0) {
        ORBX_HIP(hipSetDevice(h->device));
        const int rc = ensure_frames(h);
        if (rc) return rc;
    }
    const LevelGeom &g = h->sp.geom[level];
    *d_ptr = h->d_pyr + (size_t)b * h->sp.pyrImgBytes + g.poff + (size_t)ORBX_EDGE * g.pstride + ORBX_EDGE;
    if (w) *w = g.w;
    if (hgt) *hgt = g.h;
    if (stride) *stride = g.pstride;
    return ORBX_OK;
}

extern "C" int orbx_pyramid_host(orbx_extractor_t *h, int b, int level, int padded, uint8_t *dst, int dst_stride,
                                 int *w, int *hgt) {
    if (!h || level < 0 || level >= h->nlevels || h->pw == 0 || b < 0 || b >= h->pB) {
        orbx_set_error("orbx_pyramid_host: bad arguments or no frame extracted yet");
        return ORBX_ERR_ARG;
    }
    const LevelGeom &g = h->sp.geom[level];
    const int ow = padded ? g.w + 2 * ORBX_EDGE : g.w, oh = padded ? g.h + 2 * ORBX_EDGE : g.h;
    if (w) *w = ow;
    if (hgt) *hgt = oh;
    if (!dst) return ORBX_OK;
    if (dst_stride < ow) { orbx_set_error("dst_stride < width"); return ORBX_ERR_ARG; }
    ORBX_HIP(hipSetDevice(h->device));
    if (padded && level > 0) { const int rc = ensure_frames(h); if (rc) return rc; }
    if (h->last_valid) ORBX_HIP(hipStreamSynchronize(h->last_stream));
    const uint8_t *src = h->d_pyr + (size_t)b * h->sp.pyrImgBytes + g.poff +
                         (padded ? 0 : (size_t)ORBX_EDGE * g.pstride + ORBX_EDGE);
    const size_t span = (size_t)g.pstride * (oh - 1) + ow;
    static thread_local std::vector<uint8_t> tmp;
    if (tmp.size() < span) tmp.resize(span);
    ORBX_HIP(hipMemcpy(tmp.data(), src, span, hipMemcpyDeviceToHost));
    for (int r = 0; r < oh; r++) memcpy(dst + (size_t)r * dst_stride, tmp.data() + (size_t)r * g.pstride, ow);
    return ORBX_OK;
}

extern "C" int orbx_level_counts(orbx_extractor_t *h, int b, int32_t *candidates, int32_t *keypoints) {
    if (!h || h->pw == 0 || b < 0 || b >= h->pB || !h->last_valid) { orbx_set_error("orbx_level_counts: bad arguments or no frame extracted yet"); return ORBX_ERR_ARG; }
    ORBX_HIP(hipSetDevice(h->device));
    ORBX_HIP(hipStreamSynchronize(h->last_stream));
    if (candidates) ORBX_HIP(hipMemcpy(candidates, h->d_candCnt + (size_t)b * h->nlevels, sizeof(int32_t) * h->nlevels, hipMemcpyDeviceToHost));
    if (keypoints) ORBX_HIP(hipMemcpy(keypoints, h->d_lvlCnt + (size_t)b * h->nlevels, sizeof(int32_t) * h->nlevels, hipMemcpyDeviceToHost));
    return ORBX_OK;
}

#ifdef ORBX_DEVELOPER
static int ensure_cand(orbx_extractor *h) {
    if (h->candStale <= 0) return ORBX_OK;
    const int nl = h->nlevels, B = h->candStale;
    CellBases cb;
    for (int l = 0; l <= ORBX_MAX_LEVELS; l++) cb.v[l] = l < nl ? h->sp.geom[l].cellBase : h->sp.totalCells;
    (void)hipGetLastError();
    hipLaunchKernelGGL(k_gather, dim3((h->sp.totalCells + GATHER_CELLS_PER_BLOCK - 1) / GATHER_CELLS_PER_BLOCK, B), dim3(256), 0, h->last_stream,
                       h->d_geom, nl, h->sp.totalCells, h->d_cellCnt, h->d_cellRaw, h->d_slots, h->sp.slotsPerImg, h->d_cand, h->sp.keysPerImg,
                       h->d_candCnt, h->ini_th, h->min_th, cb, (int32_t *)nullptr, 0, (int32_t *)nullptr, 0);
    ORBX_HIP(hipGetLastError());
    h->candStale = 0;
    return ORBX_OK;
}

extern "C" int orbx_debug_octree_fallbacks(orbx_extractor_t *h, int32_t *out, int n) {
    if (!h || !out || n < 1 || h->pw == 0 || n > h->pB * h->nlevels) { orbx_set_error("orbx_debug_octree_fallbacks: bad arguments"); return ORBX_ERR_ARG; }
    ORBX_HIP(hipSetDevice(h->device));
    if (h->last_valid) ORBX_HIP(hipStreamSynchronize(h->last_stream));
    ORBX_HIP(hipMemcpy(out, h->d_octFallback, sizeof(int32_t) * (size_t)n, hipMemcpyDeviceToHost));
    return ORBX_OK;
}

extern "C" int orbx_debug_level_points(orbx_extractor_t *h, int b, int level, int stage, int32_t *out, int cap,
                                       int *n_out) {
    if (!h || !n_out || level < 0 || level >= h->nlevels || h->pw == 0 || b < 0 || b >= h->pB || stage < 0 || stage > 1) {
        orbx_set_error("orbx_debug_level_points: bad arguments");
        return ORBX_ERR_ARG;
    }
    ORBX_HIP(hipSetDevice(h->device));
    if (stage == 0) { const int rc = ensure_cand(h); if (rc) return rc; }
    if (h->last_valid) ORBX_HIP(hipStreamSynchronize(h->last_stream));
    const LevelGeom &g = h->sp.geom[level];
    int32_t n = 0;
    const int32_t *cntp = (stage == 0 ? h->d_candCnt : h->d_lvlCnt) + b * h->nlevels + level;
    ORBX_HIP(hipMemcpy(&n, cntp, sizeof(int32_t), hipMemcpyDeviceToHost));
    *n_out = n;
    if (!out || n == 0) return ORBX_OK;
    const int m = std::min(n, cap);
    std::vector<uint32_t> tmp(m);
    const uint32_t *src = stage == 0 ? h->d_cand + (size_t)b * h->sp.keysPerImg + g.keyOff
                                     : h->d_lvlKp + (size_t)b * h->sp.lvlKpCap + g.lvlKpOff;
    ORBX_HIP(hipMemcpy(tmp.data(), src, sizeof(uint32_t) * m, hipMemcpyDeviceToHost));
    for (int i = 0; i < m; i++) {
        out[3 * i] = (int32_t)(tmp[i] & 0xFFF);
        out[3 * i + 1] = (int32_t)((tmp[i] >> 12) & 0xFFF);
        out[3 * i + 2] = (int32_t)(tmp[i] >> 24);
    }
    return n > cap ? ORBX_ERR_CAPACITY : ORBX_OK;
}

#endif

extern "C" int orbx_fast_kernels(const orbx_extractor_t *h, int B, int *strips, int *cells, int *images_per_launch) {
    if (!h || h->pw == 0 || B < 1) { orbx_set_error("orbx_fast_kernels: no plan yet"); return ORBX_ERR_ARG; }
    const int nch = (h->last_valid && h->lastB == B) ? h->lastChunks : chunk_count(h->opt, B, h->profiling == 1, false);
    B = B / nch;
    if (images_per_launch) *images_per_launch = B;
    ChunkPlan p;
    const int rc = plan_chunk(plan_input(h, B, nch, h->profiling == 1, h->profiling != 0, false, false), &p);
    if (rc) return rc;
    if (strips) *strips = p.strips;
    if (cells) *cells = p.fastCells;
    return ORBX_OK;
}

#ifdef ORBX_DEVELOPER
static_assert(ORBX_DEBUG_SIZE_PLAN_INTS == 31 + ORBX_MAX_LEVELS + 1 + 2 * 8 * (int)(sizeof(ChainPlan) / sizeof(int)), "include/orbx_dev.h and orbx_size_plan.h disagree");
static_assert(ORBX_DEBUG_PLAN_INPUT_INTS == ORBX_PLAN_INPUT_INTS && ORBX_DEBUG_CHUNK_PLAN_INTS == ORBX_CHUNK_PLAN_INTS, "include/orbx_dev.h and orbx_plan.h disagree");
extern "C" int orbx_debug_plan_chunk(const int32_t *in, int n_in, int32_t *out, int n_out) {
    PlanInput pi;
    if (!in || !out || n_in != ORBX_PLAN_INPUT_INTS || n_out != ORBX_CHUNK_PLAN_INTS) { orbx_set_error("orbx_debug_plan_chunk: bad arguments"); return ORBX_ERR_ARG; }
    memcpy(&pi, in, sizeof(pi));
    if (pi.B < 1 || pi.nl < 1 || pi.nl > ORBX_MAX_LEVELS) { orbx_set_error("orbx_debug_plan_chunk: bad B or nl"); return ORBX_ERR_ARG; }
    ChunkPlan p;
    const int rc = plan_chunk(pi, &p);
    if (rc == ORBX_OK) memcpy(out, &p, sizeof(p));
    return rc;
}
extern "C" int orbx_debug_size_plan(int nfeatures, float scale_factor, int nlevels, int w, int hgt, int pyr_tile, float *tables, int32_t *nfeat_umax,
                                    uint8_t *geom, int geom_bytes, int32_t *tab, int tab_cap, int64_t *scalars, int n_scalars) {
    if (!tables || !nfeat_umax || !geom || geom_bytes != (int)sizeof(LevelGeom) * ORBX_MAX_LEVELS || !scalars || n_scalars != ORBX_DEBUG_SIZE_PLAN_INTS ||
        (tab_cap > 0 && !tab) || nfeatures < 1 || nlevels < 1 || nlevels > ORBX_MAX_LEVELS || !(scale_factor > 1.0f) || pyr_tile < 0 || pyr_tile > 64) {
        orbx_set_error("orbx_debug_size_plan: bad arguments");
        return ORBX_ERR_ARG;
    }
    SizeInput in = {};
    in.w = w; in.h = hgt; in.nlevels = nlevels; in.scale_factor = scale_factor; in.pyrTile = pyr_tile;
    extractor_tables(nfeatures, in.scale_factor, nlevels, &in.tb);
    memcpy(tables, in.tb.sf, sizeof(float) * 4 * ORBX_MAX_LEVELS);
    memcpy(nfeat_umax, in.tb.nfeat, sizeof(int32_t) * (ORBX_MAX_LEVELS + 16));
    SizePlan sp;
    const int rc = plan_size(in, &sp);
    if (rc) return rc;
    memcpy(geom, sp.geom, sizeof(sp.geom));
    if (tab_cap > 0) memcpy(tab, sp.tab.data(), sizeof(int32_t) * std::min((size_t)tab_cap, sp.tab.size()));
    const int64_t v[31] = {sp.max_kp, sp.totalCells, sp.maxNodeCap, sp.lvlKpCap, (int64_t)sp.pyrImgBytes, (int64_t)sp.slotsPerImg, (int64_t)sp.keysPerImg,
                           sp.fastTileStride, sp.fastScoreStride, sp.fastTileRows, sp.fastLdsPerWave, sp.totalStrips, sp.stripLevels,
                           (int64_t)sp.octLdsBytes, (int64_t)sp.octPyrLdsBytes, sp.octPyrWords, sp.octBigMask, sp.octDeepMax, sp.octSliceStride, sp.histStride,
                           sp.pyrTilesX, sp.pyrTilesY, sp.pyrXSpanOff, sp.pyrYSpanOff, sp.pyrBufBytes, sp.pyrMaxDim, sp.pyrMaxPar, (int64_t)sp.pyrLdsBytes,
                           sp.nChains[0], sp.nChains[1], (int64_t)sp.tab.size()};
    int64_t *o = std::copy(v, v + 31, scalars);
    o = std::copy(sp.stripBase, sp.stripBase + ORBX_MAX_LEVELS + 1, o);
    std::copy((const int *)sp.chains, (const int *)sp.chains + 2 * 8 * 8, o);
    return ORBX_OK;
}
extern "C" int orbx_debug_last_plan(const orbx_extractor_t *h, int32_t *out, int n_out) {
    if (!h || !out || n_out != ORBX_CHUNK_PLAN_INTS || !h->last_valid) { orbx_set_error("orbx_debug_last_plan: bad arguments or no call yet"); return ORBX_ERR_ARG; }
    memcpy(out, &h->lastPlan, sizeof(h->lastPlan));
    return ORBX_OK;
}
#endif

#ifdef ORBX_DEVELOPER
extern "C" int orbx_debug_blur_patches(orbx_extractor_t *h, int enable, uint8_t *out, int n) {
    if (!h) return ORBX_ERR_ARG;
    ORBX_HIP(hipSetDevice(h->device));
    if (h->last_valid) ORBX_HIP(hipStreamSynchronize(h->last_stream));
    if (out && n > 0) {
        if (!h->d_dbgBlur || n > h->dbgBlurCap) { orbx_set_error("orbx_debug_blur_patches: not enabled or n too large"); return ORBX_ERR_ARG; }
        ORBX_HIP(hipMemcpy(out, h->d_dbgBlur, (size_t)n * 37 * 37, hipMemcpyDeviceToHost));
        return ORBX_OK;
    }
    hipFree(h->d_dbgBlur); h->d_dbgBlur = nullptr; h->dbgBlurCap = 0;
    if (enable) {
        h->dbgBlurCap = h->sp.max_kp > 0 ? h->sp.max_kp + 300 : h->nfeatures + 3 * h->nlevels + 300;
        ORBX_HIP(scratch_malloc(&h->d_dbgBlur, (size_t)h->dbgBlurCap * 37 * 37));
    }
    return ORBX_OK;
}

extern "C" int orbx_debug_blurred_level(orbx_extractor_t *h, int b, int level, uint8_t *dst, int dst_stride, unsigned *mask_out) {
    if (!h || h->pw == 0 || b < 0 || b >= h->pB) { orbx_set_error("orbx_debug_blurred_level: bad arguments"); return ORBX_ERR_ARG; }
    if (mask_out) *mask_out = h->blurMaskLast;
    if (!dst) return ORBX_OK;
    if (level < 0 || level >= h->nlevels || !((h->blurMaskLast >> level) & 1u) || !h->d_blur) {
        orbx_set_error("orbx_debug_blurred_level: level %d was not blurred as a whole (mask 0x%x)", level, h->blurMaskLast);
        return ORBX_ERR_ARG;
    }
    const LevelGeom &g = h->sp.geom[level];
    if (dst_stride < g.w) { orbx_set_error("dst_stride < width"); return ORBX_ERR_ARG; }
    ORBX_HIP(hipSetDevice(h->device));
    if (h->last_valid) ORBX_HIP(hipStreamSynchronize(h->last_stream));
    const uint8_t *src = h->d_blur + (size_t)b * h->sp.pyrImgBytes + g.poff + (size_t)ORBX_EDGE * g.pstride + ORBX_EDGE;
    const size_t span = (size_t)g.pstride * (g.h - 1) + g.w;
    std::vector<uint8_t> tmp(span);
    ORBX_HIP(hipMemcpy(tmp.data(), src, span, hipMemcpyDeviceToHost));
    for (int r = 0; r < g.h; r++) memcpy(dst + (size_t)r * dst_stride, tmp.data() + (size_t)r * g.pstride, g.w);
    return ORBX_OK;
}

#endif

extern "C" int orbx_set_profiling(orbx_extractor_t *h, int enabled) {
    if (!h) return ORBX_ERR_ARG;
    ORBX_HIP(hipSetDevice(h->device));
    for (int r = 0; r < ORBX_EV_RING; r++)
        if (h->ev_pending[r]) { ORBX_HIP(hipEventSynchronize(h->ev[r][h->ev_pending[r] == 2 ? 2 : 4])); h->ev_pending[r] = 0; }
    if (enabled < 0 || enabled > 3) { orbx_set_error("orbx_set_profiling: mode %d", enabled); return ORBX_ERR_ARG; }
    h->profiling = enabled;
    if (enabled) {
        hipLaunchKernelGGL(k_nop, dim3(1), dim3(64), 0, h->stream);
        ORBX_HIP(hipStreamSynchronize(h->stream));
    }
    h->prof_calls = 0;
    h->ev_head = 0;
    h->acc_n = 0;
    for (int i = 0; i < ORBX_NUM_STAGES; i++) h->acc_ms[i] = 0;
    return ORBX_OK;
}
extern "C" int orbx_get_stage_ms(orbx_extractor_t *h, float *ms, int *ncalls) {
    if (!h || !ms) return ORBX_ERR_ARG;
    ORBX_HIP(hipSetDevice(h->device));
    for (int r = 0; r < ORBX_EV_RING; r++)
        if (h->ev_pending[r]) { int rc = harvest_events(h, r); if (rc) return rc; }
    if (h->acc_n == 0) { orbx_set_error("no profiled batch recorded"); return ORBX_ERR_ARG; }
    for (int i = 0; i < ORBX_NUM_STAGES; i++) ms[i] = (float)(h->acc_ms[i] / (double)h->acc_n);
    if (ncalls) *ncalls = (int)h->acc_n;
    return ORBX_OK;
}
```

orb_slam2v2-1_amd/csrc/orbx_extract_dev.h:

```cpp
#pragma once
#include "orbx_internal.h"

__device__ __forceinline__ void wave_sync() {
    __builtin_amdgcn_fence(__ATOMIC_ACQ_REL, "workgroup");
    __builtin_amdgcn_wave_barrier();
}

__device__ __forceinline__ int wave_incl_scan_i32(int v) {
    v += __builtin_amdgcn_update_dpp(0, v, 0x111, 0xf, 0xf, true);
    v += __builtin_amdgcn_update_dpp(0, v, 0x112, 0xf, 0xf, true);
    v += __builtin_amdgcn_update_dpp(0, v, 0x114, 0xf, 0xf, true);
    v += __builtin_amdgcn_update_dpp(0, v, 0x118, 0xf, 0xf, true);
    v += __builtin_amdgcn_update_dpp(0, v, 0x142, 0xa, 0xf, true);
    v += __builtin_amdgcn_update_dpp(0, v, 0x143, 0xc, 0xf, true);
    return v;
}
__device__ __forceinline__ int wave_total_i32(int v) { return __builtin_amdgcn_readlane(wave_incl_scan_i32(v), 63); }

__device__ __forceinline__ int reflect101(int i, int n) {
    if (i < 0) i = -i;
    if (i >= n) i = 2 * (n - 1) - i;
    return i;
}
__device__ __forceinline__ int reflect101c(int p, int n) {
    p = p < 0 ? -p : p;
    p = p >= n ? 2 * (n - 1) - p : p;
    return min(max(p, 0), n - 1);
}
typedef unsigned short ushort2v __attribute__((ext_vector_type(2)));
__device__ __forceinline__ uint32_t udot2_u16(uint32_t a, uint32_t b) {
    return __builtin_amdgcn_udot2(__builtin_bit_cast(ushort2v, a), __builtin_bit_cast(ushort2v, b), 0u, false);
}
__device__ __forceinline__ uint32_t udot2_u16_acc(uint32_t a, uint32_t b, uint32_t c) {
    return __builtin_amdgcn_udot2(__builtin_bit_cast(ushort2v, a), __builtin_bit_cast(ushort2v, b), c, false);
}

struct PyrSpan { short o0, o1, c0, c1; };
#define FAST_WAVES 4
#define GATHER_CELLS_PER_BLOCK 16
#ifndef OCT_T
#define OCT_T 512
#endif
#define OCT_T_WIDE 1024
#define DESC_WAVES 4
struct DescGroup {
    int lvBegin, lvEnd;
    int writeCounts;
    int copyBlock0;
    const orbx_keypoint_t *kpsScratch;
    const uint8_t *descScratch;
    uint32_t taps;
    long long hostDelta;
    int blk0[ORBX_MAX_LEVELS];
};
template <class Bound>
static inline int desc_level_blocks(int lvBegin, int lvEnd, Bound bound, int *blk0) {
    int nb = 0;
    for (int l = 0; l < ORBX_MAX_LEVELS; l++) {
        blk0[l] = l <= lvBegin ? 0 : l < lvEnd ? nb : 0x7fffffff;
        if (l >= lvBegin && l < lvEnd) nb += (bound(l) + DESC_WAVES - 1) / DESC_WAVES;
    }
    return nb;
}
#define DESC_COPY_PER_BLOCK 16
#define BLUR_R 16
#define BLUR_SRC (BLUR_R + 6)
struct BlurPlan { int tileBase[ORBX_MAX_LEVELS + 1]; int tilesX[ORBX_MAX_LEVELS]; };
__global__ void k_blur_levels(const uint8_t *pyr, uint8_t *blur, size_t pyrImgBytes, const LevelGeom *geom, int nlevels, int totalTiles,
                              BlurPlan bp, int gaussRounding, uint32_t taps);
struct CellBases { int v[ORBX_MAX_LEVELS + 1]; };
__device__ __forceinline__ int level_of_cell(const CellBases &cb, int nlevels, int gc) {
    int l = 0;
#pragma unroll
    for (int i = 1; i < ORBX_MAX_LEVELS; i++) l += (i < nlevels && gc >= cb.v[i]) ? 1 : 0;
    return l;
}

__global__ void k_pyramid_fused(const uint8_t *src, int sstride, size_t simg, uint8_t *pyr, size_t pyrImgBytes, const LevelGeom *geom,
                                int nlevels, const int32_t *tab, int xSpanOff, int ySpanOff, int tilesX, int tilesY, int bufBytes,
                                int maxPar, int l0);
template <int RW, int SR>
__global__ void k_pyr_level(uint8_t *pyr, size_t pyrImgBytes, const LevelGeom *geom, int l, const int32_t *tab, int nxc,
                            int nbands);
template <bool FULL>
__global__ void k_pyr_pad(const uint8_t *img, int sstride, size_t simg, uint8_t *pyr, size_t pyrImgBytes, const LevelGeom *geom,
                          int l0);
__global__ void k_pyr_chain(uint8_t *pyr, size_t pyrImgBytes, const LevelGeom *geom, const int32_t *tab, ChainPlan cp);
__global__ void k_pyr_pad_rows(const uint8_t *img, int sstride, size_t simg, uint8_t *pyr, size_t pyrImgBytes, const LevelGeom *geom);
#define PAD_ROWS_PER_BLOCK 4
#define PAD_FULL_ROWS 4
struct StripBases { int v[ORBX_MAX_LEVELS + 1]; };
__global__ void k_fast_strips(const uint8_t *pyr, size_t pyrImgBytes, const LevelGeom *geom, int nlevels, int totalStrips, int totalCells,
                              uint32_t *cellCnt, uint32_t *cellRaw, uint32_t *slots, size_t slotsPerImg, int iniTh, int minTh,
                              StripBases sb, const int32_t *sparseFlag, int strip0, int skipSparse);
__global__ void k_fast_strips_sparse(const uint8_t *pyr, size_t pyrImgBytes, const LevelGeom *geom, int nlevels, int totalStrips, int totalCells,
                                     uint32_t *cellCnt, uint32_t *cellRaw, uint32_t *slots, size_t slotsPerImg, int iniTh, int minTh,
                                     StripBases sb, const int32_t *sparseFlag);
struct FastHist { uint32_t *cnt, *best; int stride; const int32_t *tab; };
template <int ES_T, bool SPARSE>
__global__ void k_fast_cells(const uint8_t *pyr, size_t pyrImgBytes, const LevelGeom *geom, int nlevels, int totalCells,
                             uint32_t *cellCnt, uint32_t *cellRaw, uint32_t *slots, size_t slotsPerImg, int iniTh, int minTh, int ESrt,
                             int SSrt, int tileRows, int ldsPerWave, int phaseLimit, CellBases cb, unsigned stripLevels,
                             const int32_t *sparseFlag, FastHist fh);
__global__ void k_gather(const LevelGeom *geom, int nlevels, int totalCells, const uint32_t *cellCnt, const uint32_t *cellRaw,
                         const uint32_t *slots, size_t slotsPerImg, uint32_t *cand, size_t keysPerImg, int32_t *candCnt, int iniTh,
                         int minTh, CellBases cb, int32_t *sparseFlag, int sparsePerCell, int32_t *sparseSeen, int callSeq);
struct OctBig {
    uint32_t *part, *leaf, *best;
    int32_t *state;
    int K, nBig, deepMax, pyrMax;
    int levelOf[ORBX_MAX_LEVELS];
};
#define OCT_BIG_K 8
struct OctSrc {
    const uint32_t *cellCnt, *cellRaw, *slots;
    size_t slotsPerImg;
    int totalCells, iniTh, minTh;
    int32_t *candCntOut;
    int32_t *sparseFlag;
    int sparsePerCell;
    int32_t *sparseSeen;
    int callSeq;
    uint32_t *candOut;
    uint32_t *histCnt, *histBest; int histStride;
    unsigned char nslice[ORBX_MAX_LEVELS];
    uint32_t *partCnt, *partBest; int32_t *sliceState; int maxSlices, partStride;
    int linear, nImages, blkPrefix[ORBX_MAX_LEVELS + 1];
};
#define OCT_MAX_SLICES 4
__global__ void k_octree_pyr(const LevelGeom *geom, int nlevels, const uint32_t *cand, size_t keysPerImg, const int32_t *candCnt,
                             uint32_t *lvlKp, int lvlKpCap, int32_t *lvlCnt, const int32_t *tab, int capMax, int pow2cap,
                             int pyrWords, int32_t *fallback, int dbgStop, uint16_t *nodeOf, int scratchInts, int dbgStopExact,
                             unsigned bigMask, int l0, OctSrc src);
template <int MODE>
__global__ void k_octree_big(const LevelGeom *geom, int nlevels, const uint32_t *cand, size_t keysPerImg, const int32_t *candCnt,
                             uint32_t *lvlKp, int lvlKpCap, int32_t *lvlCnt, const int32_t *tab, int capMax, int pow2cap,
                             int pyrWords, int32_t *fallback, uint16_t *nodeOf, int scratchInts, OctBig big);
__global__ void k_octree(const LevelGeom *geom, int nlevels, const uint32_t *cand, uint16_t *nodeOf, size_t keysPerImg,
                         const int32_t *candCnt, uint32_t *lvlKp, int lvlKpCap, int32_t *lvlCnt, const int32_t *tab, int capMax,
                         int pow2cap, int scratchInts, int dbgStop);
__global__ void k_octree_pyr_wide(const LevelGeom *geom, int nlevels, const uint32_t *cand, size_t keysPerImg, const int32_t *candCnt,
                                  uint32_t *lvlKp, int lvlKpCap, int32_t *lvlCnt, const int32_t *tab, int capMax, int pow2cap,
                                  int pyrWords, int32_t *fallback, int dbgStop, uint16_t *nodeOf, int scratchInts, int dbgStopExact,
                                  unsigned bigMask, int l0, OctSrc src);
template <int MODE>
__global__ void k_octree_big_wide(const LevelGeom *geom, int nlevels, const uint32_t *cand, size_t keysPerImg, const int32_t *candCnt,
                                  uint32_t *lvlKp, int lvlKpCap, int32_t *lvlCnt, const int32_t *tab, int capMax, int pow2cap,
                                  int pyrWords, int32_t *fallback, uint16_t *nodeOf, int scratchInts, OctBig big);
__global__ void k_octree_wide(const LevelGeom *geom, int nlevels, const uint32_t *cand, uint16_t *nodeOf, size_t keysPerImg,
                              const int32_t *candCnt, uint32_t *lvlKp, int lvlKpCap, int32_t *lvlCnt, const int32_t *tab, int capMax,
                              int pow2cap, int scratchInts, int dbgStop);
template <int GAUSS, bool SPLIT>
__global__ void k_describe(const uint8_t *pyr, size_t pyrImgBytes, const LevelGeom *geom, int nlevels, const uint32_t *lvlKp,
                           int lvlKpCap, const int32_t *lvlCnt, orbx_keypoint_t *kps, uint8_t *desc, int32_t *counts,
                           int cap, uint8_t *dbgBlur, const uint8_t *blur, unsigned blurMask, DescGroup grp);
```

orb_slam2v2-1_amd/csrc/orbx_internal.h:

```cpp
#pragma once
#include <hip/hip_runtime.h>
#include <stdint.h>
#include <stdio.h>
#include <string.h>
#include <vector>
#include "orbx.h"
#include "orbx_size_plan.h"

#define ORBX_GAUSS_TAPS_DEFAULT (18u | (34u << 8) | (49u << 16) | (55u << 24))
#define ORBX_DESC_R 18
#define ORBX_EV_RING 32
#define ORBX_MAX_CHUNKS 4
#define ORBX_SIDE_STREAMS 2
#define ORBX_HIST_IMAGES 4

#include "orbx_plan.h"

#define ORBX_HIP(call)                                                                      \
    do {                                                                                    \
        hipError_t e_ = (call);                                                             \
        if (e_ != hipSuccess) {                                                             \
            orbx_set_error("%s failed: %s (%s:%d)", #call, hipGetErrorString(e_), __FILE__, \
                           __LINE__);                                                       \
            return (e_ == hipErrorNoDevice || e_ == hipErrorInvalidDevice ||                \
                    e_ == hipErrorNoBinaryForGpu || e_ == hipErrorInsufficientDriver)       \
                       ? ORBX_ERR_NO_DEVICE                                                 \
                       : ORBX_ERR_HIP;                                                      \
        }                                                                                   \
    } while (0)

#ifdef ORBX_DEVELOPER
hipError_t orbx_internal_scratch_filled(void *p, size_t bytes, bool pinned);
template <class T> static inline hipError_t scratch_malloc(T **p, size_t bytes) {
    const hipError_t e = hipMalloc((void **)p, bytes);
    return e != hipSuccess ? e : orbx_internal_scratch_filled((void *)*p, bytes, false);
}
template <class T> static inline hipError_t scratch_host_malloc(T **p, size_t bytes, unsigned flags) {
    const hipError_t e = hipHostMalloc((void **)p, bytes, flags);
    return e != hipSuccess ? e : orbx_internal_scratch_filled((void *)*p, bytes, true);
}
#else
template <class T> static inline hipError_t scratch_malloc(T **p, size_t bytes) { return hipMalloc((void **)p, bytes); }
template <class T> static inline hipError_t scratch_host_malloc(T **p, size_t bytes, unsigned flags) { return hipHostMalloc((void **)p, bytes, flags); }
#endif

struct orbx_extractor {
    int nfeatures, nlevels, ini_th, min_th, device;
    double scale_factor;
    ExtractorTables tb;
    orbx_flavour_t flavour;
    int opt[ORBX_NUM_OPTIONS];

    int pw, ph, pB;
    SizePlan sp;
    int32_t *d_octFallback;
    uint32_t *d_octPart, *d_octLeaf, *d_octBest; int32_t *d_octState;
    LevelGeom *d_geom;
    int32_t *d_tab;
    uint8_t *d_pyr;
    uint32_t *d_cellCnt, *d_cellRaw, *d_slots, *d_cand, *d_lvlKp;
    uint16_t *d_nodeOf;
    int32_t *d_candCnt, *d_lvlCnt;
    int candStale;
    int32_t *h_sparseSeen, *d_sparseSeen; int callSeq;
    uint32_t *d_octPartBest, *d_octPartCnt; int32_t *d_octSliceState;
    uint32_t *d_histCnt, *d_histBest;
    int32_t *d_sparse;
    uint8_t *d_in; size_t d_in_bytes;
    orbx_keypoint_t *d_kps; uint8_t *d_desc; int32_t *d_counts; int out_cap, out_B;
    orbx_keypoint_t *h_kps; uint8_t *h_desc; int32_t *h_counts;
    float *d_sfr; float *h_sfr; int sfr_cap;
    uint8_t *fv_d[2], *fv_h[2], *fv_hdev[2]; int fv_cap, fv_next;
    uint8_t *fv_stage, *fv_stage_dev; size_t fv_stage_bytes;
    int32_t *fv_flag, *fv_flag_dev; int fv_seq;
    long long descHostDelta;
    uint8_t *d_dbgBlur; int dbgBlurCap;
    hipStream_t stream;
    hipStream_t side[ORBX_SIDE_STREAMS]; hipEvent_t evPyr[ORBX_MAX_CHUNKS], evJoin[ORBX_SIDE_STREAMS]; int lastChunks;
    uint8_t *d_pyrAlt; size_t pyrAltBytes; int pfValid, pfUsed, pfB, pfW, pfH, pfStride; const uint8_t *pfImgs; size_t pfImgStride;
    uint8_t *d_blur, *d_blurAlt; size_t blurBytes, blurAltBytes; unsigned blurMaskLast, blurMaskAlt;
    orbx_keypoint_t *d_kpsB; uint8_t *d_descB; size_t splitBytes; hipEvent_t evGather, evOctA;
    uint8_t *d_pyrNext; size_t pyrNextBytes; int pyrBuffers;
    int prevPyrValid;
    hipEvent_t evFastDone, evPrefetch;
    hipStream_t last_stream;
    int last_valid;
    int lastB;
    ChunkPlan lastPlan;
    int framesStale;
    int32_t *st_sad; uint2 *st_rc; int32_t *st_binStart; uint4 *st_items; size_t st_n; int st_nB;
    hipStream_t st_stream;
    int profiling; unsigned prof_calls;
    hipEvent_t ev[ORBX_EV_RING][ORBX_NUM_STAGES];
    unsigned char ev_pending[ORBX_EV_RING];
    int ev_head;
    double acc_ms[ORBX_NUM_STAGES];
    long acc_n;
    struct RgbdScratch *rgbd;
    struct RectScratch *rect;
};

void orbx_internal_free_stereo_scratch(orbx_extractor *h);
void orbx_internal_free_rgbd_scratch(orbx_extractor *h);
void orbx_internal_free_rect_scratch(orbx_extractor *h);
int orbx_internal_stereo_frame_device(orbx_extractor *h, const uint8_t *d_pair, int w, int hgt, int stride, size_t img_bytes, float mbf,
                                      float mb, int cap, orbx_keypoint_t *kl, uint8_t *dl, int *nl, orbx_keypoint_t *kr, uint8_t *dr,
                                      int *nr, float *uright, float *depth, int *nmatch);
int orbx_internal_stereo_frame_record(orbx_extractor *h, uint8_t *d_rec, uint8_t *rec_hostdev, int cap, float mbf, float mb, hipStream_t st, bool recordsOnHost,
                                      int32_t *doneFlag, int doneSeq, int *flagArmed);
void orbx_internal_release_match_scratch();
void orbx_internal_release_arena();
void orbx_internal_release_bow_scratch();
void orbx_internal_release_pose_scratch();
void orbx_internal_release_init_scratch();
void orbx_internal_release_sim3_scratch();
void orbx_internal_release_pnp_scratch();
void orbx_internal_release_sim3opt_scratch();
void orbx_internal_release_newpoints_scratch();
void orbx_internal_release_lba_scratch();
void orbx_internal_release_essential_scratch();
int orbx_internal_tri_check(const char *fn, const int32_t *node_qstart, const int32_t *q_items, int nq, const int32_t *node_cstart,
                            const int32_t *c_items, int nc, int nnodes);
void orbx_internal_tri_launch(const orbx_keypoint_t *d_k1, const uint8_t *d_qd, const uint8_t *d_qf, float *d_qa, int nq, const orbx_keypoint_t *d_k2,
                              const uint8_t *d_cd, const uint8_t *d_cf, float *d_ca, int nc, const int32_t *d_nqs, const int32_t *d_qi,
                              const int32_t *d_ncs, const int32_t *d_ci, int nnodes, const float *F12_9, float ex, float ey,
                              const float *scale_factors, const float *level_sigma2, int nlevels, int max_dist, int check_orientation,
                              int32_t *d_match_q, int32_t *d_out2, hipStream_t st);
#ifdef ORBX_DEVELOPER
void orbx_internal_arena_info(int64_t *out5);
void orbx_internal_match_scratch_info(int64_t *out2);
void orbx_internal_bow_scratch_info(int64_t *out2);
void *orbx_internal_arena_stream();
void *orbx_internal_match_scratch_stream();
#endif
const uint8_t *orbx_internal_device_visible(const uint8_t *p);
int orbx_internal_level(const orbx_extractor *h, int level, int *w, int *hgt, int *pstride,
                        unsigned long long *poff);

int fast_search_for_initialization(const orbx_keypoint_t *k1, const uint8_t *d1, int n1, const orbx_keypoint_t *k2,
                                   const uint8_t *d2, int n2, const orbm_grid_geom_t *g2, float *prev, int32_t *m12,
                                   int window, float nnratio, int check_ori, int device, int *nmatches);
struct DevFrame { hipStream_t stream; };
struct FrustumArgs { const orbm_worldpoint_t *pts; const float *Tcw16; const orbm_camera_t *cam; float viewCosLimit; const float *thr; };
int fast_search_by_projection_mp(const orbx_keypoint_t *kun, const uint8_t *desc, const float *uright, int n,
                                 const orbm_grid_geom_t *g, const float *sf, int nlevels, const orbm_mappoint_t *mps,
                                 const uint8_t *mp_desc, int m, int32_t *frame_mp, const int32_t *ext_obs, float th,
                                 float nnratio, int device, int *nmatches, const FrustumArgs *world = nullptr,
                                 orbm_mappoint_t *proj_out = nullptr, const DevFrame *dev = nullptr);
int fast_is_in_frustum(const orbm_worldpoint_t *pts, int m, const float *Tcw16, const orbm_camera_t *cam,
                       const orbm_grid_geom_t *g, float viewCosLimit, const float *thr, int nlevels, orbm_mappoint_t *out,
                       int device);
int fast_search_by_projection_frame(const orbx_keypoint_t *kun, const uint8_t *desc, const float *uright, int n,
                                    const orbm_grid_geom_t *g, const float *sf, int nlevels, const orbm_camera_t *cam,
                                    const float *Tc16, const float *Tl16, const orbm_lastpoint_t *last,
                                    const uint8_t *last_desc, int nlast, int32_t *cur_mp, const int32_t *ext_obs,
                                    float th, int mono, int check_ori, int device, int *nmatches, const DevFrame *dev = nullptr);
int fast_match_windows(const orbx_keypoint_t *kun, const uint8_t *desc, const float *uright, int n,
                       const orbm_grid_geom_t *g, const orbm_grid_geom_t *ga, const orbm_window_query_t *q,
                       const uint8_t *qdesc, int m,
                       int32_t *holder, const int32_t *ext_blocks, int max_dist, int check_ori, int device, int *nmatches);
int fast_best_in_windows(const orbx_keypoint_t *kun, const uint8_t *desc, const float *uright, int n,
                         const orbm_grid_geom_t *g, const orbm_grid_geom_t *ga, const orbm_window_query_t *q,
                         const uint8_t *qdesc, int m, const float *inv_sigma2, int nlevels, int32_t *best_idx,
                         int32_t *best_dist, int device);
int fast_distinctive_descriptors(const uint8_t *desc, const int32_t *offsets, int npoints, int32_t *best_row,
                                 int32_t *best_median, int device);
extern thread_local int t_matchExact;
struct MatchPath { int resolver, fallback; long long lds; };
struct StereoPath { int useLds, bhShift, nbins, device; };
extern thread_local MatchPath t_matchPath;
extern thread_local StereoPath t_stereoPath;

__device__ __forceinline__ void xcd_block_map(int &bx, int &b) {
    const unsigned nbx = gridDim.x, total = nbx * gridDim.y, lin = blockIdx.y * nbx + blockIdx.x;
    const unsigned xcd = lin & 7u, idx = lin >> 3, q = total >> 3, r = total & 7u;
    const unsigned pos = xcd * q + min(xcd, r) + idx;
    b = __builtin_amdgcn_readfirstlane((int)(pos / nbx));
    bx = __builtin_amdgcn_readfirstlane((int)(pos - (unsigned)b * nbx));
}
```

orb_slam2v2-1_amd/csrc/orbx_pyramid.hip:

```cpp
#include "orbx_extract_dev.h"
#include "orbx_bufaddr.h"

__global__ __launch_bounds__(256) void k_pyramid_fused(
    const uint8_t *__restrict__ src, int sstride, size_t simg, uint8_t *__restrict__ pyr, size_t pyrImgBytes,
    const LevelGeom *__restrict__ geom, int nlevels, const int32_t *__restrict__ tab, int xSpanOff, int ySpanOff,
    int tilesX, int tilesY, int bufBytes, int maxPar, int l0) {
    extern __shared__ __align__(16) uint8_t smem[];
    uint2 *xpar = (uint2 *)(smem + 2 * bufBytes), *ypar = xpar + maxPar;
    __shared__ PyrSpan sX[ORBX_MAX_LEVELS], sY[ORBX_MAX_LEVELS];
    __shared__ int xo[ORBX_MAX_LEVELS + 1], yo[ORBX_MAX_LEVELS + 1];
    const int tid = threadIdx.x, tx = blockIdx.x % tilesX, ty = blockIdx.x / tilesX, b = blockIdx.y;
    if (tid < nlevels) sX[tid] = ((const PyrSpan *)(tab + xSpanOff))[tid * tilesX + tx];
    else if (tid >= 32 && tid < 32 + nlevels) sY[tid - 32] = ((const PyrSpan *)(tab + ySpanOff))[(tid - 32) * tilesY + ty];
    __syncthreads();
    if (tid == 0) {
        int ax = 0, ay = 0;
        for (int l = 0; l < nlevels; l++) {
            xo[l] = ax; yo[l] = ay;
            if (l > l0) { ax += sX[l].c1 - sX[l].c0; ay += sY[l].c1 - sY[l].c0; }
        }
        xo[nlevels] = ax; yo[nlevels] = ay;
    }
    __syncthreads();
    {
        const int nx = xo[nlevels], ny = yo[nlevels];
        for (int i = tid; i < nx + ny; i += 256) {
            const bool isx = i < nx;
            const int j = isx ? i : i - nx;
            const int *off = isx ? xo : yo;
            int l = l0 + 1;
            while (l + 1 <= nlevels && j >= off[l + 1]) l++;
            const LevelGeom *g = geom + l;
            const PyrSpan cs = isx ? sX[l] : sY[l], ps = isx ? sX[l - 1] : sY[l - 1];
            const int k = cs.c0 + (j - off[l]);
            uint2 q;
            if (isx) {
                const int sx = tab[g->xofsOff + k], sw = g[-1].w;
                q.x = (uint32_t)(sx - ps.c0) | ((uint32_t)(min(sx + 1, sw - 1) - ps.c0) << 16);
                q.y = (uint32_t)tab[g->xalphaOff + k];
                xpar[j] = q;
            } else {
                const int sy = tab[g->yofsOff + k], shh = g[-1].h;
                q.x = (uint32_t)(min(max(sy, 0), shh - 1) - ps.c0) | ((uint32_t)(min(max(sy + 1, 0), shh - 1) - ps.c0) << 16);
                q.y = (uint32_t)tab[g->ybetaOff + k];
                ypar[j] = q;
            }
        }
        const PyrSpan X = sX[l0], Y = sY[l0];
        const int cw = X.c1 - X.c0, ch = Y.c1 - Y.c0;
        const int ss = l0 == 0 ? sstride : geom[l0].pstride;
        const uint8_t *s = (l0 == 0 ? src + (size_t)b * simg
                                    : pyr + (size_t)b * pyrImgBytes + geom[l0].poff + (size_t)ORBX_EDGE * ss + ORBX_EDGE) + (size_t)Y.c0 * ss + X.c0;
        const unsigned M = ((1u << 20) + cw - 1) / cw;
        uint8_t *first = smem + (l0 & 1) * bufBytes;
        for (int i = tid; i < cw * ch; i += 256) {
            const int y = (int)(((unsigned)i * M) >> 20), x = i - y * cw;
            first[i] = s[(size_t)y * ss + x];
        }
    }
    __syncthreads();
    uint8_t *base = pyr + (size_t)b * pyrImgBytes;
    for (int l = l0; l < nlevels; l++) {
        const PyrSpan X = sX[l], Y = sY[l];
        const int cw = X.c1 - X.c0, ch = Y.c1 - Y.c0;
        uint8_t *cur = smem + (l & 1) * bufBytes;
        const LevelGeom *g = geom + l;
        const int lw = g->w, lh = g->h, pstride = g->pstride;
        if (l > l0) {
            const uint8_t *prev = smem + ((l & 1) ^ 1) * bufBytes;
            const int pw = sX[l - 1].c1 - sX[l - 1].c0;
            const uint2 *xp = xpar + xo[l], *yp = ypar + yo[l];
            const unsigned M = ((1u << 20) + cw - 1) / cw;
            for (int i = tid; i < cw * ch; i += 256) {
                const int y = (int)(((unsigned)i * M) >> 20), x = i - y * cw;
                const uint2 yq = yp[y], xq = xp[x];
                const uint8_t *S0 = prev + (yq.x & 0xFFFF) * pw, *S1 = prev + (yq.x >> 16) * pw;
                const int b0 = (int16_t)(yq.y & 0xFFFF), b1 = (int16_t)(yq.y >> 16);
                const int a0 = (int16_t)(xq.y & 0xFFFF), a1 = (int16_t)(xq.y >> 16);
                const int i0 = xq.x & 0xFFFF, i1 = xq.x >> 16;
                const int h0 = S0[i0] * a0 + S0[i1] * a1;
                const int h1 = S1[i0] * a0 + S1[i1] * a1;
                cur[i] = (uint8_t)((((b0 * (h0 >> 4)) >> 16) + ((b1 * (h1 >> 4)) >> 16) + 2) >> 2);
            }
            __syncthreads();
        }
        if (l == l0 && l0 > 0) continue;
        uint8_t *dst = base + g->poff;
        const int ow = X.o1 - X.o0, oh = Y.o1 - Y.o0;
        const unsigned Mo = ((1u << 20) + ow - 1) / max(ow, 1);
        const bool edgeX = X.o0 <= ORBX_EDGE || X.o1 >= lw - ORBX_EDGE, edgeY = Y.o0 <= ORBX_EDGE || Y.o1 >= lh - ORBX_EDGE;
        if (!edgeX && !edgeY) {
            for (int i = tid; i < ow * oh; i += 256) {
                const int iy = (int)(((unsigned)i * Mo) >> 20), ix = i - iy * ow;
                dst[(size_t)(Y.o0 + iy + ORBX_EDGE) * pstride + X.o0 + ix + ORBX_EDGE] = cur[(Y.o0 + iy - Y.c0) * cw + (X.o0 + ix - X.c0)];
            }
        } else {
            for (int i = tid; i < ow * oh; i += 256) {
                const int iy = (int)(((unsigned)i * Mo) >> 20), ix = i - iy * ow;
                const int x = X.o0 + ix, y = Y.o0 + iy;
                const uint8_t v = cur[(y - Y.c0) * cw + (x - X.c0)];
                const int px = x + ORBX_EDGE, py = y + ORBX_EDGE;
                const int mx = (x >= 1 && x <= ORBX_EDGE) ? ORBX_EDGE - x
                               : (x >= lw - 1 - ORBX_EDGE && x <= lw - 2) ? 2 * (lw - 1) - x + ORBX_EDGE : -1;
                const int my = (y >= 1 && y <= ORBX_EDGE) ? ORBX_EDGE - y
                               : (y >= lh - 1 - ORBX_EDGE && y <= lh - 2) ? 2 * (lh - 1) - y + ORBX_EDGE : -1;
                dst[(size_t)py * pstride + px] = v;
                if (mx >= 0) dst[(size_t)py * pstride + mx] = v;
                if (my >= 0) {
                    dst[(size_t)my * pstride + px] = v;
                    if (mx >= 0) dst[(size_t)my * pstride + mx] = v;
                }
            }
        }
    }
}


__device__ __forceinline__ uint32_t vmulhi24(uint32_t a, uint32_t b) { return __umulhi(a & 0xFFFFFFu, b & 0xFFFFFFu); }
template <int RW, int SR>
__global__ __launch_bounds__(256) void k_pyr_level(uint8_t *__restrict__ pyr, size_t pyrImgBytes,
                                                   const LevelGeom *__restrict__ geom, int l,
                                                   const int32_t *__restrict__ tab, int nxc, int nbands) {
    static_assert((RW == 8 || RW == 16) && SR <= 32, "row table: one lane per output row, a 32-bit mask of source rows");
    constexpr int RWM = RW - 1;
    int bx, b;
    xcd_block_map(bx, b);
    const int wave = __builtin_amdgcn_readfirstlane(bx * 4 + (threadIdx.x >> 6)), lane = threadIdx.x & 63;
    if (wave >= nxc * nbands) return;
    const int band = wave / nxc, xc = wave - band * nxc;
    const LevelGeom G = geom[l];
    const int sw = geom[l - 1].w, sh = geom[l - 1].h, sps = geom[l - 1].pstride;
    uint8_t *base = pyr + (size_t)b * pyrImgBytes;
    const uint8_t *srow0 = base + geom[l - 1].poff + (size_t)ORBX_EDGE * sps;
    uint8_t *drow0 = base + G.poff + (size_t)ORBX_EDGE * G.pstride + ORBX_EDGE;
    const int x0 = xc * 128 + 2 * lane - 1, x1 = x0 + 1;
    const bool vst = x0 < G.w;
    const int xa = min(max(x0, 0), G.w - 1), xb = min(x1, G.w - 1);
    const int ca = ORBX_EDGE + tab[G.xofsOff + xa], cb = ORBX_EDGE + tab[G.xofsOff + xb];
    const uint32_t aa = (uint32_t)tab[G.xalphaOff + xa], ab = (uint32_t)tab[G.xalphaOff + xb];
    const int A = ca & ~3;
    const uint32_t oa = (uint32_t)(ca - A), ob = (uint32_t)(cb - A);
    const uint32_t selA = oa | ((oa + 1) << 16) | 0x0C000C00u, selB = ob | ((ob + 1) << 16) | 0x0C000C00u;
    (void)sw;
    const int y0 = band * RW, nrow = min(RW, G.h - y0);
    const int yl = min(y0 + (lane & RWM), G.h - 1);
    const int vsy = tab[G.yofsOff + yl];
    const uint32_t vbt = (uint32_t)tab[G.ybetaOff + yl];
    const int rf = __builtin_amdgcn_readfirstlane(vsy);
    const int kk = vsy + 1 - rf;
    const int prevsy = __shfl_up(vsy, 1);
    const bool okl = (lane & RWM) >= nrow || (rf >= 0 && vsy + 1 <= sh - 1 && kk < SR && ((lane & RWM) == 0 || vsy > prevsy));
    constexpr unsigned long long rowLanes = (1ull << RW) - 1ull;
    const bool regular = (__ballot(okl) & rowLanes) == rowLanes;
    if (regular) {
        uint32_t m = (lane & RWM) < nrow ? 1u << (kk & 31) : 0u;
        m |= __shfl_xor(m, 1); m |= __shfl_xor(m, 2); m |= __shfl_xor(m, 4);
        if (RW == 16) m |= __shfl_xor(m, 8);
        const uint32_t mask = __builtin_amdgcn_readfirstlane(m);
        const int lastk = 31 - __builtin_clz(mask | 1u);
        const orbx_buf_t srcBuf = buf_make(srow0, (uint32_t)sps * (uint32_t)(geom[l - 1].prows - ORBX_EDGE));
        const orbx_buf_t dstBuf = buf_make(base + G.poff, (uint32_t)G.pstride * (uint32_t)G.prows);
        uint2 q[SR];
#pragma unroll
        for (int k = 0; k < SR; k++) {
            if (k > lastk) continue;
            q[k] = buf_load_b64(srcBuf, (uint32_t)A, (uint32_t)(min(rf + k, sh - 1) * sps));
        }
        uint32_t tpa = 0, tpb = 0;
        int cnt = 0;
        uint32_t drow = (uint32_t)((ORBX_EDGE + y0) * G.pstride + ORBX_EDGE - 1);
        const uint32_t xoff = (uint32_t)(x0 + 1);
#pragma unroll
        for (int k = 0; k < SR; k++) {
            if (k > lastk) continue;
            const uint32_t tca = udot2_u16(__builtin_amdgcn_perm(q[k].y, q[k].x, selA), aa) & 0x7FFF0u;
            const uint32_t tcb = udot2_u16(__builtin_amdgcn_perm(q[k].y, q[k].x, selB), ab) & 0x7FFF0u;
            if (k > 0 && ((mask >> k) & 1u)) {
                const uint32_t bb = (uint32_t)__builtin_amdgcn_readlane((int)vbt, cnt);
                const uint32_t b0 = (bb & 0xFFFu) << 12, b1 = ((bb >> 16) & 0xFFFu) << 12;
                const uint32_t pa = (vmulhi24(b0, tpa) + vmulhi24(b1, tca) + 2) >> 2;
                const uint32_t pb = (vmulhi24(b0, tpb) + vmulhi24(b1, tcb) + 2) >> 2;
                if (vst) buf_store_b16(dstBuf, xoff, drow, (uint16_t)(pa | (pb << 8)));
                drow += (uint32_t)G.pstride;
                cnt++;
            }
            tpa = tca; tpb = tcb;
        }
        return;
    }
    int cr0 = -1, cr1 = -1;
    uint32_t t0a = 0, t0b = 0, t1a = 0, t1b = 0;
    for (int y = y0; y < y0 + nrow; y++) {
        const int syy = tab[G.yofsOff + y];
        const uint32_t bb = (uint32_t)tab[G.ybetaOff + y];
        const int r0 = min(max(syy, 0), sh - 1), r1 = min(max(syy + 1, 0), sh - 1);
        if (r0 == cr1) { t0a = t1a; t0b = t1b; cr0 = cr1; }
        else if (r0 != cr0) {
            const uint2 q = *(const uint2 *)(srow0 + (size_t)r0 * sps + A);
            t0a = udot2_u16(__builtin_amdgcn_perm(q.y, q.x, selA), aa) & 0x7FFF0u;
            t0b = udot2_u16(__builtin_amdgcn_perm(q.y, q.x, selB), ab) & 0x7FFF0u;
            cr0 = r0;
        }
        if (r1 != cr1) {
            if (r1 == cr0) { t1a = t0a; t1b = t0b; }
            else {
                const uint2 q = *(const uint2 *)(srow0 + (size_t)r1 * sps + A);
                t1a = udot2_u16(__builtin_amdgcn_perm(q.y, q.x, selA), aa) & 0x7FFF0u;
                t1b = udot2_u16(__builtin_amdgcn_perm(q.y, q.x, selB), ab) & 0x7FFF0u;
            }
            cr1 = r1;
        }
        const uint32_t b0 = (bb & 0xFFFu) << 12, b1 = ((bb >> 16) & 0xFFFu) << 12;
        const uint32_t pa = (vmulhi24(b0, t0a) + vmulhi24(b1, t1a) + 2) >> 2;
        const uint32_t pb = (vmulhi24(b0, t0b) + vmulhi24(b1, t1b) + 2) >> 2;
        if (vst) *(uint16_t *)(drow0 + (size_t)y * G.pstride + x0) = (uint16_t)(pa | (pb << 8));
    }
}

template <bool FULL>
__global__ __launch_bounds__(256) void k_pyr_pad(const uint8_t *__restrict__ img, int sstride, size_t simg,
                                                 uint8_t *__restrict__ pyr, size_t pyrImgBytes,
                                                 const LevelGeom *__restrict__ geom, int l0) {
    const int l = FULL ? l0 : l0 + blockIdx.y;
    const LevelGeom G = geom[l];
    uint8_t *lvl = pyr + (size_t)blockIdx.z * pyrImgBytes + G.poff;
    const uint8_t *src = FULL ? img + (size_t)blockIdx.z * simg : lvl + (size_t)ORBX_EDGE * G.pstride + ORBX_EDGE;
    const int ss = FULL ? sstride : G.pstride;
    const int pw4 = (G.w + 2 * ORBX_EDGE + 3) >> 2, rows = G.h + 2 * ORBX_EDGE;
    const int LW = (ORBX_EDGE >> 2) + 1, R0 = (ORBX_EDGE + G.w) >> 2, side = LW + (pw4 - R0);
    if (FULL) {
        const int pc = G.pstride >> 4;
        const int cI0 = (ORBX_EDGE + 15) >> 4, cI1 = max((G.w + ORBX_EDGE) >> 4, cI0);
        const int nI = cI1 - cI0, nE = pc - nI;
        const int rowBlocks = (rows + PAD_FULL_ROWS - 1) / PAD_FULL_ROWS;
        if ((int)blockIdx.y < rowBlocks) {
            const int i = blockIdx.x * blockDim.x + threadIdx.x;
            if (i >= nI) return;
            const uint32_t off = (uint32_t)i * 16u;
            uint4 v[PAD_FULL_ROWS];
#pragma unroll
            for (int r = 0; r < PAD_FULL_ROWS; r++) {
                const int py = min((int)blockIdx.y * PAD_FULL_ROWS + r, rows - 1);
                const uint8_t *srow = src + (size_t)reflect101c(py - ORBX_EDGE, G.h) * ss + (cI0 * 16 - ORBX_EDGE);
                __builtin_memcpy(&v[r], srow + off, 16);
            }
#pragma unroll
            for (int r = 0; r < PAD_FULL_ROWS; r++) {
                const int py = min((int)blockIdx.y * PAD_FULL_ROWS + r, rows - 1);
                *(uint4 *)(lvl + (size_t)py * G.pstride + cI0 * 16 + off) = v[r];
            }
            return;
        }
        const int j = (((int)blockIdx.y - rowBlocks) * gridDim.x + blockIdx.x) * blockDim.x + threadIdx.x;
        if (j >= nE * rows) return;
        const int py = j / nE, k = j - py * nE;
        const int c = k < cI0 ? k : cI1 + (k - cI0);
        const uint8_t *srow = src + (size_t)reflect101c(py - ORBX_EDGE, G.h) * ss;
        const int px = c * 16 - ORBX_EDGE;
        uint32_t t[4];
#pragma unroll
        for (int u = 0; u < 4; u++)
            t[u] = (uint32_t)srow[reflect101c(px + 4 * u, G.w)] | ((uint32_t)srow[reflect101c(px + 4 * u + 1, G.w)] << 8) |
                   ((uint32_t)srow[reflect101c(px + 4 * u + 2, G.w)] << 16) | ((uint32_t)srow[reflect101c(px + 4 * u + 3, G.w)] << 24);
        *(uint4 *)(lvl + (size_t)py * G.pstride + c * 16) = make_uint4(t[0], t[1], t[2], t[3]);
        return;
    }
    const int total = 2 * ORBX_EDGE * pw4 + G.h * side;
    const unsigned Mp = (1u << 24) / (unsigned)pw4 + 1u, Ms = (1u << 24) / (unsigned)side + 1u;
    for (int i = blockIdx.x * 256 + threadIdx.x; i < total; i += gridDim.x * 256) {
        int py, p4;
        if (i < 2 * ORBX_EDGE * pw4) {
            const int r = (int)(((unsigned long long)(unsigned)i * Mp) >> 24);
            p4 = i - r * pw4;
            py = r < ORBX_EDGE ? r : G.h + r;
        } else {
            const int j = i - 2 * ORBX_EDGE * pw4, r = (int)(((unsigned long long)(unsigned)j * Ms) >> 24), k = j - r * side;
            py = ORBX_EDGE + r;
            p4 = k < LW ? k : R0 + (k - LW);
        }
        const uint8_t *srow = src + (size_t)reflect101c(py - ORBX_EDGE, G.h) * ss;
        const int px = p4 * 4 - ORBX_EDGE;
        const uint32_t v = (uint32_t)srow[reflect101c(px, G.w)] | ((uint32_t)srow[reflect101c(px + 1, G.w)] << 8) |
                           ((uint32_t)srow[reflect101c(px + 2, G.w)] << 16) | ((uint32_t)srow[reflect101c(px + 3, G.w)] << 24);
        *(uint32_t *)(lvl + (size_t)py * G.pstride + p4 * 4) = v;
    }
}

#define PAD_ROWS PAD_ROWS_PER_BLOCK
__global__ __launch_bounds__(256) void k_pyr_pad_rows(const uint8_t *__restrict__ img, int sstride, size_t simg, uint8_t *__restrict__ pyr,
                                                      size_t pyrImgBytes, const LevelGeom *__restrict__ geom) {
    extern __shared__ __align__(16) uint8_t rows_lds[];
    const LevelGeom G = geom[0];
    const int tid = threadIdx.x, r0 = blockIdx.x * PAD_ROWS, nr = min(PAD_ROWS, G.h - r0);
    const uint8_t *src = img + (size_t)blockIdx.y * simg;
    uint8_t *lvl = pyr + (size_t)blockIdx.y * pyrImgBytes + G.poff;
    const uintptr_t p0 = (uintptr_t)(src + (size_t)r0 * sstride), p1 = p0 + (size_t)(nr - 1) * sstride + G.w;
    const uintptr_t a0 = p0 & ~(uintptr_t)15;
    const int nch = (int)(((p1 + 15) & ~(uintptr_t)15) - a0) >> 4, lead = (int)(p0 - a0);
    for (int i0 = 0; i0 < nch; i0 += 4 * 256) {
        uint4 v[4];
#pragma unroll
        for (int k = 0; k < 4; k++) { const int i = i0 + tid + 256 * k; v[k] = ((const uint4 *)a0)[min(i, nch - 1)]; }
#pragma unroll
        for (int k = 0; k < 4; k++) { const int i = i0 + tid + 256 * k; if (i < nch) ((uint4 *)rows_lds)[i] = v[k]; }
    }
    __syncthreads();
    const int pc = G.pstride >> 4;
    for (int t = 0; t < 3; t++) {
        for (int i = tid; i < nr * pc; i += 256) {
            const int sr = i / pc, c = i - sr * pc, r = r0 + sr;
            int py;
            if (t == 0) py = r + ORBX_EDGE;
            else if (t == 1) { if (r < 1 || r > ORBX_EDGE) continue; py = ORBX_EDGE - r; }
            else { if (r < G.h - 1 - ORBX_EDGE || r > G.h - 2) continue; py = 2 * (G.h - 1) - r + ORBX_EDGE; }
            const uint8_t *row = rows_lds + lead + sr * sstride;
            const int px = c * 16 - ORBX_EDGE;
            uint4 v;
            if (px >= 0 && px + 15 < G.w) {
                const uint32_t off = (uint32_t)(row - rows_lds) + (uint32_t)px, sh = off & 3u;
                const uint32_t *d = (const uint32_t *)(rows_lds + (off & ~3u));
                const uint32_t d0 = d[0], d1 = d[1], d2 = d[2], d3 = d[3], d4 = d[4];
                v = make_uint4(__builtin_amdgcn_alignbyte(d1, d0, sh), __builtin_amdgcn_alignbyte(d2, d1, sh),
                               __builtin_amdgcn_alignbyte(d3, d2, sh), __builtin_amdgcn_alignbyte(d4, d3, sh));
            } else {
                uint32_t w4[4];
#pragma unroll
                for (int u = 0; u < 4; u++)
                    w4[u] = (uint32_t)row[reflect101c(px + 4 * u, G.w)] | ((uint32_t)row[reflect101c(px + 4 * u + 1, G.w)] << 8) |
                            ((uint32_t)row[reflect101c(px + 4 * u + 2, G.w)] << 16) | ((uint32_t)row[reflect101c(px + 4 * u + 3, G.w)] << 24);
                v = make_uint4(w4[0], w4[1], w4[2], w4[3]);
            }
            *(uint4 *)(lvl + (size_t)py * G.pstride + c * 16) = v;
        }
    }
}

__global__ __launch_bounds__(256) void k_pyr_chain(uint8_t *__restrict__ pyr, size_t pyrImgBytes, const LevelGeom *__restrict__ geom,
                                                   const int32_t *__restrict__ tab, ChainPlan cp) {
    extern __shared__ __align__(16) uint8_t smem[];
    __shared__ PyrSpan sX[PC_MAXL + 1], sY[PC_MAXL + 1];
    const int tid = threadIdx.x, wave = __builtin_amdgcn_readfirstlane(tid >> 6), lane = tid & 63;
    const int tx = blockIdx.x % cp.tilesX, ty = blockIdx.x / cp.tilesX, b = blockIdx.y;
    const int nb = cp.lb - cp.la;
    const int ntX = cp.tilesX, ntY = cp.tilesY;
    if (tid <= nb) sX[tid] = ((const PyrSpan *)(tab + cp.xSpanOff))[tid * ntX + tx];
    else if (tid >= 32 && tid <= 32 + nb) sY[tid - 32] = ((const PyrSpan *)(tab + cp.ySpanOff))[(tid - 32) * ntY + ty];
    __syncthreads();
    uint8_t *buf[2] = {smem, smem + cp.bufBytes};
    uint2 *ypar = (uint2 *)(smem + 2 * cp.bufBytes);
    uint8_t *base = pyr + (size_t)b * pyrImgBytes;
    int ia[PC_MAXL], ob[PC_MAXL]; uint32_t aa[PC_MAXL], ab[PC_MAXL];
#pragma unroll
    for (int k = 0; k < PC_MAXL; k++) {
        ia[k] = 0; ob[k] = 0; aa[k] = 0; ab[k] = 0;
        if (k < nb) {
            const LevelGeom *g = geom + cp.la + 1 + k;
            const PyrSpan X = sX[k + 1], Xp = sX[k];
            const int xa = min(X.c0 + 2 * lane, g->w - 1), xb = min(xa + 1, g->w - 1);
            const int sa = tab[g->xofsOff + xa], sb2 = tab[g->xofsOff + xb];
            aa[k] = (uint32_t)tab[g->xalphaOff + xa]; ab[k] = (uint32_t)tab[g->xalphaOff + xb];
            ia[k] = sa - Xp.c0;
            ob[k] = sb2 - sa;
            const PyrSpan Y = sY[k + 1], Yp = sY[k];
            const int sh = g[-1].h, ch = Y.c1 - Y.c0;
            for (int y = tid; y < ch; y += 256) {
                const int sy = tab[g->yofsOff + Y.c0 + y];
                uint2 q;
                q.x = (uint32_t)(min(max(sy, 0), sh - 1) - Yp.c0) | ((uint32_t)(min(max(sy + 1, 0), sh - 1) - Yp.c0) << 16);
                q.y = (uint32_t)tab[g->ybetaOff + Y.c0 + y];
                ypar[k * cp.maxRows + y] = q;
            }
        }
    }
    {
        const LevelGeom *g = geom + cp.la;
        const PyrSpan X = sX[0], Y = sY[0];
        const int cw = X.c1 - X.c0, ch = Y.c1 - Y.c0, pitch = (cw + 8 + 3) & ~3, nd = pitch >> 2;
        const uint8_t *s0 = base + g->poff + (size_t)(ORBX_EDGE + Y.c0) * g->pstride + ORBX_EDGE + X.c0;
        const uint32_t shf = (uint32_t)((uintptr_t)s0 & 3);
        const uint8_t *s0a = s0 - shf;
        const unsigned M = ((1u << 20) + nd - 1) / nd;
        for (int i = tid; i < nd * ch; i += 256) {
            const int r = (int)(((unsigned)i * M) >> 20), k = i - r * nd;
            const uint32_t *p = (const uint32_t *)(s0a + (size_t)r * g->pstride) + k;
            ((uint32_t *)(buf[0] + r * pitch))[k] = __builtin_amdgcn_alignbyte(p[1], p[0], shf);
        }
    }
    __syncthreads();
#pragma unroll
    for (int k = 0; k < PC_MAXL; k++) {
        if (k >= nb) break;
        const LevelGeom *g = geom + cp.la + 1 + k;
        const PyrSpan X = sX[k + 1], Y = sY[k + 1];
        const int cw = X.c1 - X.c0, ch = Y.c1 - Y.c0;
        const int ppitch = (sX[k].c1 - sX[k].c0 + 8 + 3) & ~3, pitch = (cw + 8 + 3) & ~3;
        const uint8_t *prev = buf[k & 1];
        uint8_t *cur = buf[(k & 1) ^ 1];
        const int A = ia[k] & ~3;
        const uint32_t oa = (uint32_t)(ia[k] - A), obb = oa + (uint32_t)ob[k];
        const uint32_t selA = oa | ((oa + 1) << 16) | 0x0C000C00u, selB = obb | ((obb + 1) << 16) | 0x0C000C00u;
        const bool act = 2 * lane < cw;
        const int xa = X.c0 + 2 * lane;
        const bool ownA = xa >= X.o0 && xa < X.o1, ownB = xa + 1 >= X.o0 && xa + 1 < X.o1 && 2 * lane + 1 < cw;
        uint8_t *drow0 = base + g->poff + (size_t)ORBX_EDGE * g->pstride + ORBX_EDGE + xa;
        const uint2 *yp = ypar + k * cp.maxRows;
        for (int y = wave; y < ch; y += 4) {
            const uint2 q = yp[y];
            const uint32_t r0 = q.x & 0xFFFFu, r1 = q.x >> 16;
            const uint32_t b0 = (q.y & 0xFFFu) << 12, b1 = ((q.y >> 16) & 0xFFFu) << 12;
            if (act) {
                const uint32_t *p0 = (const uint32_t *)(prev + r0 * ppitch + A), *p1 = (const uint32_t *)(prev + r1 * ppitch + A);
                const uint32_t d00 = p0[0], d01 = p0[1], d10 = p1[0], d11 = p1[1];
                const uint32_t t0a = udot2_u16(__builtin_amdgcn_perm(d01, d00, selA), aa[k]) & 0x7FFF0u;
                const uint32_t t0b = udot2_u16(__builtin_amdgcn_perm(d01, d00, selB), ab[k]) & 0x7FFF0u;
                const uint32_t t1a = udot2_u16(__builtin_amdgcn_perm(d11, d10, selA), aa[k]) & 0x7FFF0u;
                const uint32_t t1b = udot2_u16(__builtin_amdgcn_perm(d11, d10, selB), ab[k]) & 0x7FFF0u;
                const uint32_t pa = (vmulhi24(b0, t0a) + vmulhi24(b1, t1a) + 2) >> 2;
                const uint32_t pb = (vmulhi24(b0, t0b) + vmulhi24(b1, t1b) + 2) >> 2;
                *(uint16_t *)(cur + y * pitch + 2 * lane) = (uint16_t)(pa | (pb << 8));
                const int yy = Y.c0 + y;
                if (yy >= Y.o0 && yy < Y.o1) {
                    uint8_t *d = drow0 + (size_t)yy * g->pstride;
                    if (ownA) d[0] = (uint8_t)pa;
                    if (ownB) d[1] = (uint8_t)pb;
                }
            }
        }
        __syncthreads();
    }
}

template __global__ void k_pyr_level<8, 12>(uint8_t *, size_t, const LevelGeom *, int, const int32_t *, int, int);
template __global__ void k_pyr_level<16, 22>(uint8_t *, size_t, const LevelGeom *, int, const int32_t *, int, int);
template __global__ void k_pyr_pad<true>(const uint8_t *, int, size_t, uint8_t *, size_t, const LevelGeom *, int);
template __global__ void k_pyr_pad<false>(const uint8_t *, int, size_t, uint8_t *, size_t, const LevelGeom *, int);
```

orb_slam2v2-1_amd/csrc/orbx_size_plan.h:

```cpp
#pragma once
#include <math.h>
#include <stdint.h>
#include <string.h>
#include <algorithm>
#include <vector>
#include "orbx.h"

#define ORBX_MAX_LEVELS 16
#define ORBX_EDGE 19
#define ORBX_MINB 16
#define ORBX_HALF_PATCH 15
#define ORBX_MAX_ROOTS 64

void orbx_set_error(const char *fmt, ...);
#define ORBX_LDS_LIMIT (150 * 1024)
#define ORBX_CHAIN_LDS_LIMIT (60 * 1024)
#define ORBX_CHAIN_MAX_COLS 128
#define ORBX_MAX_CELL_WINDOW 65
#define ORBX_MAX_COORD 4095
#define ORBX_MAX_KEYS 0xFFFFFF
#define ORBX_PYR_MAX_CELLS 16384

struct LevelGeom {
    int w, h;
// ... 215 lines not shown
            maxBestWords = std::max(maxBestWords, g.nIni * (((1 << (2 * (d + 1))) - 1) / 3));
        }
        p.octPyrLdsBytes = oct_pyr_lds_bytes(p.maxNodeCap, p.octPyrWords, maxPath, maxBestWords, maxCells);
        if (p.octPyrLdsBytes <= ORBX_LDS_LIMIT || cellCap <= 64) break;
    }
    for (int l = 0; l < nl; l++) {
        const int deep = pyr_deep_cells(p.geom[l]);
        p.octDeepMax = std::max(p.octDeepMax, (deep + 1) / 2 + 1);
        p.histStride = std::max(p.histStride, (deep + 3) & ~3);
        if (p.geom[l].ncells >= 600) p.octSliceStride = std::max(p.octSliceStride, deep);
    }
    for (int l = 0; l < nl; l++) {
        LevelGeom &g = p.geom[l];
        if (l > 0) {
            const int sw = p.geom[l - 1].w, shh = p.geom[l - 1].h;
            const double inv_scale_x = (double)g.w / sw, inv_scale_y = (double)g.h / shh;
            const double scale_x = 1. / inv_scale_x, scale_y = 1. / inv_scale_y;
            g.xofsOff = (int)tab.size();
            tab.resize(tab.size() + g.w);
            g.xalphaOff = (int)tab.size();
            tab.resize(tab.size() + g.w);
            for (int dx = 0; dx < g.w; dx++) {
                float fx = (float)((dx + 0.5) * scale_x - 0.5);
                int sx = cv_floor(fx);
                fx -= sx;
                if (sx < 0) { fx = 0; sx = 0; }
                if (sx >= sw - 1) { fx = 0; sx = sw - 1; }
                const short a0 = sat_short_round((1.f - fx) * 2048), a1 = sat_short_round(fx * 2048);
                tab[g.xofsOff + dx] = sx;
                tab[g.xalphaOff + dx] = (int32_t)((uint32_t)(uint16_t)a0 | ((uint32_t)(uint16_t)a1 << 16));
            }
            g.yofsOff = (int)tab.size();
            tab.resize(tab.size() + g.h);
            g.ybetaOff = (int)tab.size();
            tab.resize(tab.size() + g.h);
            for (int dy = 0; dy < g.h; dy++) {
                float fy = (float)((dy + 0.5) * scale_y - 0.5);
                int sy = cv_floor(fy);
                fy -= sy;
                const short b0 = sat_short_round((1.f - fy) * 2048), b1 = sat_short_round(fy * 2048);
                tab[g.yofsOff + dy] = sy;
                tab[g.ybetaOff + dy] = (int32_t)((uint32_t)(uint16_t)b0 | ((uint32_t)(uint16_t)b1 << 16));
            }
        }
        const float hX = (float)g.regW / g.nIni;
        g.rootBoxOff = (int)tab.size();
        for (int i = 0; i <= g.nIni; i++) tab.push_back((int)(hX * (float)i));
        const int words = (g.regW + 3) / 4;
        g.rootTabOff = (int)(tab.size() * 4);
        const size_t base = tab.size();
        tab.resize(tab.size() + words, 0);
        uint8_t *rt = (uint8_t *)&tab[base];
        for (int x = 0; x < g.regW; x++) {
            size_t r = (size_t)((float)x / hX);
            if (r >= (size_t)g.nIni) r = g.nIni - 1;
            rt[x] = (uint8_t)r;
        }
        const int D = g.pyrDepth;
        g.xPathOff = (int)tab.size();
        for (int x = 0; x < g.regW; x++) {
            const int r = ((const uint8_t *)&tab[base])[x];
            int lo = tab[g.rootBoxOff + r], hi = tab[g.rootBoxOff + r + 1];
            uint32_t path = 0;
            for (int d = 0; d < D; d++) {
                const int mx = lo + ((hi - lo + 1) >> 1);
                const uint32_t bit = x < mx ? 0u : 1u;
                if (bit) lo = mx; else hi = mx;
                path = (path << 2) | bit;
            }
            tab.push_back((int32_t)(((uint32_t)r << (2 * D)) | path));
        }
        g.yPathOff = (int)tab.size();
        for (int y = 0; y < g.regH; y++) {
            int lo = 0, hi = g.regH;
            uint32_t path = 0;
            for (int d = 0; d < D; d++) {
                const int my = lo + ((hi - lo + 1) >> 1);
                const uint32_t bit = y < my ? 0u : 1u;
                if (bit) lo = my; else hi = my;
                path = (path << 2) | (bit << 1);
            }
            tab.push_back((int32_t)path);
        }
    }
    {
        const int Lc = nl - 1;
        int T = (int)lrintf((in.pyrTile > 0 ? (float)in.pyrTile : 64.0f) / tb.sf[Lc]);
        T = std::max(4, std::min(64, (T + 2) & ~3));
        int widest[ORBX_MAX_LEVELS] = {}, maxPar = 0;
        p.pyrTilesX = plan_spans(p.geom, tab, 0, Lc, T, 0, &p.pyrXSpanOff, widest, &maxPar);
        p.pyrTilesY = plan_spans(p.geom, tab, 0, Lc, T, 1, &p.pyrYSpanOff, widest, &maxPar);
        p.pyrMaxDim = (*std::max_element(widest, widest + nl) + 3) & ~3;
        p.pyrBufBytes = (p.pyrMaxDim * p.pyrMaxDim + 15) & ~15;
        p.pyrMaxPar = (maxPar + 3) & ~3;
        p.pyrLdsBytes = 2 * (size_t)p.pyrBufBytes + (size_t)p.pyrMaxPar * 16 + 16;
        if (p.pyrLdsBytes > ORBX_LDS_LIMIT) { orbx_set_error("pyramid tile needs %zu B of LDS", p.pyrLdsBytes); return ORBX_ERR_UNSUPPORTED; }
    }
    for (int variant = 0; variant < 2; variant++) {
        const int CL = variant == 0 ? 4 : PC_MAXL;
        const int nbTotal = nl - 1;
        if (nbTotal < 1 || !(in.scale_factor <= 2.0)) continue;
        const int nch = (nbTotal + CL - 1) / CL;
        bool ok = true;
        for (int c = 0, la = 0; c < nch && ok; c++) {
            const int nb = c == 0 ? nbTotal - CL * (nch - 1) : CL, lb = la + nb;
            ChainPlan cp = {};
            cp.la = la; cp.lb = lb;
            const int TY = nb <= 4 ? 8 : 16;
            bool fits = false;
            for (int TX = 96; TX >= 16 && !fits; TX -= 4) {
                const size_t mark = tab.size();
                int cw[PC_MAXL + 1] = {}, chh[PC_MAXL + 1] = {}, par = 0;
                cp.tilesX = plan_spans(p.geom, tab, la, lb, TX, 0, &cp.xSpanOff, cw, &par);
                cp.tilesY = plan_spans(p.geom, tab, la, lb, TY, 1, &cp.ySpanOff, chh, &par);
                int buf = 0, maxW = 0, maxRows = 0;
                for (int k = 0; k <= nb; k++) {
                    if (k > 0) { maxW = std::max(maxW, cw[k]); maxRows = std::max(maxRows, chh[k]); }
                    buf = std::max(buf, ((cw[k] + 8 + 3) & ~3) * chh[k]);
                }
                cp.bufBytes = (buf + 15) & ~15;
                cp.maxRows = maxRows;
                fits = maxW <= ORBX_CHAIN_MAX_COLS && 2 * (size_t)cp.bufBytes + (size_t)nb * maxRows * 8 <= ORBX_CHAIN_LDS_LIMIT;
                if (!fits) tab.resize(mark);
            }
            ok = fits;
            if (ok) p.chains[variant][p.nChains[variant]++] = cp;
            la = lb;
        }
        if (!ok) p.nChains[variant] = 0;
    }
    if (maxTw > ORBX_MAX_CELL_WINDOW || maxTh > ORBX_MAX_CELL_WINDOW) { orbx_set_error("cell window %dx%d exceeds 65", maxTw, maxTh); return ORBX_ERR_UNSUPPORTED; }
    for (int l = 0; l <= ORBX_MAX_LEVELS; l++) {
        p.stripBase[l] = p.totalStrips;
        if (l < nl && p.geom[l].wCell <= 32) {
            p.totalStrips += p.geom[l].nRows * ((p.geom[l].nCols + 3) / 4);
            p.stripLevels |= 1u << l;
        }
    }
    p.totalCells = cellBase;
    p.lvlKpCap = lvlKpOff;
    p.pyrImgBytes = (poff + 255) & ~(size_t)255;
    p.slotsPerImg = slotOff;
    p.keysPerImg = (keyOff + 7) & ~(size_t)7;
    p.fastTileStride = (maxTw + 6 + 3) & ~3;
    p.fastScoreStride = (maxTw - 6 + 4 + 3) & ~3;
    p.fastTileRows = maxTh;
    p.fastLdsPerWave = (4 * p.fastTileStride * maxTh + p.fastScoreStride * (maxTh - 4) + 15) & ~15;
    p.octLdsBytes = oct_exact_lds_bytes(p.maxNodeCap, maxCells);
    if (p.octPyrLdsBytes > ORBX_LDS_LIMIT) { orbx_set_error("quad-tree pyramid needs %zu B of LDS", p.octPyrLdsBytes); return ORBX_ERR_UNSUPPORTED; }
    if (p.octLdsBytes > ORBX_LDS_LIMIT) { orbx_set_error("quad-tree needs %zu B of LDS (features per level %d): unsupported", p.octLdsBytes, p.maxNodeCap); return ORBX_ERR_UNSUPPORTED; }
    *out = std::move(p);
    return ORBX_OK;
}
```

Baseline: 120,700 frames/s.

## Precompute pyramid column/band resize records on host and load them in k_pyr_level

```diff
diff --git a/include/orbx_dev.h b/include/orbx_dev.h
--- a/include/orbx_dev.h
+++ b/include/orbx_dev.h
@@ -40,6 +40,7 @@
 int orbx_debug_size_plan(int nfeatures, float scale_factor, int nlevels, int w, int h, int pyr_tile, float *tables, int32_t *nfeat_umax,
                          uint8_t *geom, int geom_bytes, int32_t *tab, int tab_cap, int64_t *scalars, int n_scalars);
 
+
 #define ORBM_DEBUG_THREAD_SCRATCH_INTS 9
 int orbm_debug_thread_scratch(int64_t *out, int n_out);
 
diff --git a/include/orbx_dev_pyr.h b/include/orbx_dev_pyr.h
--- /dev/null
+++ b/include/orbx_dev_pyr.h
@@ -0,0 +1,15 @@
+#ifndef ORBX_DEV_PYR_H
+#define ORBX_DEV_PYR_H
+#include "orbx.h"
+#ifdef __cplusplus
+extern "C" {
+#endif
+
+#define ORBX_DEBUG_PYR_RECORDS_INTS 98
+int orbx_debug_pyr_records(orbx_extractor_t *h, int nfeatures, float scale_factor, int nlevels, int w, int hgt, uint32_t *cols, int cols_cap,
+                           uint32_t *bands, int bands_cap, int32_t *index, int n_index);
+
+#ifdef __cplusplus
+}
+#endif
+#endif
diff --git a/orb_slam2v2-1_amd/__init__.py b/orb_slam2v2-1_amd/__init__.py
--- a/orb_slam2v2-1_amd/__init__.py
+++ b/orb_slam2v2-1_amd/__init__.py
@@ -112,6 +112,7 @@
                "orbm_debug_stereo_path", "orbx_debug_plan_chunk", "orbx_debug_last_plan", "orbm_debug_thread_scratch",
                "orbx_debug_size_plan", "orbx_debug_set_alloc_fill", "orbx_debug_alloc_fill_stats", "orbx_debug_stall_stream",
                "orbx_debug_streams"]
+DEV_PYR_EXPORTS = ["orbx_debug_pyr_records"]
 SIZE_PLAN_FIELDS = ["max_kp", "totalCells", "maxNodeCap", "lvlKpCap", "pyrImgBytes", "slotsPerImg", "keysPerImg", "fastTileStride", "fastScoreStride",
                     "fastTileRows", "fastLdsPerWave", "totalStrips", "stripLevels", "octLdsBytes", "octPyrLdsBytes", "octPyrWords", "octBigMask",
                     "octDeepMax", "octSliceStride", "histStride", "pyrTilesX", "pyrTilesY", "pyrXSpanOff", "pyrYSpanOff", "pyrBufBytes", "pyrMaxDim",
@@ -411,6 +412,7 @@
         L.orbx_debug_last_plan.argtypes = [vp, vp, i32]
         L.orbm_debug_thread_scratch.argtypes = [vp, i32]
         L.orbx_debug_size_plan.argtypes = [i32, f32, i32, i32, i32, i32, vp, vp, vp, i32, vp, i32, vp, i32]
+        L.orbx_debug_pyr_records.argtypes = [vp, i32, f32, i32, i32, i32, vp, i32, vp, i32, vp, i32]
         L.orbx_debug_set_alloc_fill.argtypes = [i32, C.c_uint32]
         L.orbx_debug_alloc_fill_stats.argtypes = [vp]
         L.orbx_debug_stall_stream.argtypes = [vp, i32, i32]
@@ -823,6 +825,24 @@
         n = len(SIZE_PLAN_FIELDS)
         d.update({k: int(v) for k, v in zip(SIZE_PLAN_FIELDS, sc)}, geom=geom, tab=tab, stripBase=sc[n:n + 17].astype(np.int32),
                  chains=sc[n + 17:].astype(np.int32).reshape(2, 8, 8))
+    return d
+
+
+def debug_pyr_records(nfeatures=0, scale_factor=0.0, nlevels=0, w=0, h=0, extractor=None):
+    L = extractor._L if extractor is not None else lib(True)
+    hh = extractor._h if extractor is not None else None
+    idx = np.zeros(2 + 6 * 16, np.int32)
+    cols, bands = np.zeros(0, np.uint32), np.zeros(0, np.uint32)
+    for _ in range(2):
+        rc = L.orbx_debug_pyr_records(hh, int(nfeatures), float(scale_factor), int(nlevels), int(w), int(h), _p(cols), len(cols), _p(bands), len(bands),
+                                      _p(idx), len(idx))
+        if rc != ORBX_OK or (len(cols) == idx[0] and len(bands) == idx[1]):
+            break
+        cols, bands = np.zeros(int(idx[0]), np.uint32), np.zeros(int(idx[1]), np.uint32)
+    d = dict(status=rc, message=L.orbx_last_error().decode() if rc else "")
+    if rc == ORBX_OK:
+        d.update(cols=cols.reshape(-1, 4), bands=bands, nxc=idx[2:18].copy(), colOff=idx[18:34].copy(), nbands=idx[34:66].reshape(2, 16).copy(),
+                 bandOff=idx[66:98].reshape(2, 16).copy())
     return d
 
 
diff --git a/orb_slam2v2-1_amd/build.py b/orb_slam2v2-1_amd/build.py
--- a/orb_slam2v2-1_amd/build.py
+++ b/orb_slam2v2-1_amd/build.py
@@ -39,7 +39,7 @@
 
 def _deps():
     return [os.path.join(CSRC, f) for f in os.listdir(CSRC)] + [
-        os.path.join(ROOT, "include", f) for f in ("orbx.h", "orbx_dev.h", "orb_pattern_31.inc")]
+        os.path.join(ROOT, "include", f) for f in ("orbx.h", "orbx_dev.h", "orbx_dev_pyr.h", "orb_pattern_31.inc")]
 
 
 def _compile_link(out, defines, verbose):
diff --git a/orb_slam2v2-1_amd/csrc/orbx_extract.hip b/orb_slam2v2-1_amd/csrc/orbx_extract.hip
--- a/orb_slam2v2-1_amd/csrc/orbx_extract.hip
+++ b/orb_slam2v2-1_amd/csrc/orbx_extract.hip
@@ -1,6 +1,7 @@
 #include "orbx_extract_dev.h"
 #ifdef ORBX_DEVELOPER
 #include "orbx_dev.h"
+#include "orbx_dev_pyr.h"
 #endif
 #include <math.h>
 #include <float.h>
@@ -190,6 +191,8 @@
         {(void **)&h->d_octLeaf, sizeof(uint32_t) * slots * (size_t)sp.octPyrWords, false},
         {(void **)&h->d_octBest, sizeof(uint32_t) * slots * (size_t)sp.maxNodeCap, false},
         {(void **)&h->d_octState, sizeof(int32_t) * slots * 4, true},
+        {(void **)&h->d_pyrCols, sizeof(PyrColRec) * std::max<size_t>(h->pr.cols.size(), 1), false},
+        {(void **)&h->d_pyrBands, sizeof(uint32_t) * std::max<size_t>(h->pr.bands.size(), 1), false},
     };
     if (sp.octSliceStride > 0) {
         v.push_back({(void **)&h->d_octPartBest, sizeof(uint32_t) * slots * OCT_MAX_SLICES * (size_t)sp.octSliceStride, false});
@@ -205,6 +208,7 @@
     hipFree(h->d_pyrNext); h->d_pyrNext = nullptr; h->pyrNextBytes = 0;
     hipFree(h->d_blur); hipFree(h->d_blurAlt); h->d_blur = h->d_blurAlt = nullptr; h->blurBytes = h->blurAltBytes = 0; h->blurMaskLast = h->blurMaskAlt = 0;
     h->sp = SizePlan();
+    h->pr = PyrRecords();
     h->pw = h->ph = h->pB = 0;
 }
 
@@ -262,18 +266,23 @@
     const SizeInput in = {w, hgt, h->nlevels, h->scale_factor, h->tb, h->opt[3]};
     const int rc = plan_size(in, &sp);
     if (rc) return rc;
+    PyrRecords pr;
+    plan_pyr_records(in, sp, &pr);
     ORBX_HIP(hipSetDevice(h->device));
     if (h->last_valid) ORBX_HIP(hipStreamSynchronize(h->last_stream));
     for (int i = 0; i < ORBX_SIDE_STREAMS; i++) ORBX_HIP(hipStreamSynchronize(h->side[i]));
     if (h->pw == w && h->ph == hgt) B = std::max(B, h->pB);
     free_plan(h);
     h->sp = std::move(sp);
+    h->pr = std::move(pr);
     for (const PlanBuffer &b : plan_buffers(h, h->sp, B)) {
         ORBX_HIP(scratch_malloc(b.ptr, b.bytes));
         if (b.zero) ORBX_HIP(hipMemset(*b.ptr, 0, b.bytes));
     }
     ORBX_HIP(hipMemcpy(h->d_geom, h->sp.geom, sizeof(LevelGeom) * ORBX_MAX_LEVELS, hipMemcpyHostToDevice));
     if (!h->sp.tab.empty()) ORBX_HIP(hipMemcpy(h->d_tab, h->sp.tab.data(), sizeof(int32_t) * h->sp.tab.size(), hipMemcpyHostToDevice));
+    if (!h->pr.cols.empty()) ORBX_HIP(hipMemcpy(h->d_pyrCols, h->pr.cols.data(), sizeof(PyrColRec) * h->pr.cols.size(), hipMemcpyHostToDevice));
+    if (!h->pr.bands.empty()) ORBX_HIP(hipMemcpy(h->d_pyrBands, h->pr.bands.data(), sizeof(uint32_t) * h->pr.bands.size(), hipMemcpyHostToDevice));
     h->pw = w; h->ph = hgt; h->pB = B;
     return ORBX_OK;
 }
@@ -388,10 +397,15 @@
     for (int l = 1; l <= lastSingle; l++) {
         const int nxc = (h->sp.geom[l].w + 1 + 127) / 128, nb16 = (h->sp.geom[l].h + 15) / 16, nb8 = (h->sp.geom[l].h + 7) / 8;
         const bool tall = h->scale_factor <= 1.25f && (h->opt[22] == 0 ? (size_t)nxc * nb16 * B >= 8192 : h->opt[22] == 2);
+        const PyrColRec *cols = h->d_pyrCols + h->pr.colOff[l];
+        const int f = tall ? 1 : 0, nb = tall ? nb16 : nb8, gx = (nxc * nb + 3) / 4;
+        const uint32_t *bands = h->d_pyrBands + h->pr.bandOff[f][l];
         if (tall)
-            hipLaunchKernelGGL((k_pyr_level<16, 22>), dim3((nxc * nb16 + 3) / 4, B), dim3(256), 0, st, pyr, h->sp.pyrImgBytes, h->d_geom, l, h->d_tab, nxc, nb16);
+            hipLaunchKernelGGL((k_pyr_level<16, 22>), dim3(gx, B), dim3(256), 0, st, pyr, h->sp.pyrImgBytes, h->d_geom, l, h->d_tab, nxc, nb, cols, bands,
+                               pyr_rcp((uint32_t)nxc), pyr_rcp((uint32_t)gx));
         else
-            hipLaunchKernelGGL((k_pyr_level<8, 12>), dim3((nxc * nb8 + 3) / 4, B), dim3(256), 0, st, pyr, h->sp.pyrImgBytes, h->d_geom, l, h->d_tab, nxc, nb8);
+            hipLaunchKernelGGL((k_pyr_level<8, 12>), dim3(gx, B), dim3(256), 0, st, pyr, h->sp.pyrImgBytes, h->d_geom, l, h->d_tab, nxc, nb, cols, bands,
+                               pyr_rcp((uint32_t)nxc), pyr_rcp((uint32_t)gx));
     }
     if (lastSingle < nl - 1)
         hipLaunchKernelGGL(k_pyramid_fused, dim3(h->sp.pyrTilesX * h->sp.pyrTilesY, B), dim3(256), h->sp.pyrLdsBytes, st, d_imgs,
@@ -1226,6 +1240,7 @@
 
 #ifdef ORBX_DEVELOPER
 static_assert(ORBX_DEBUG_SIZE_PLAN_INTS == 31 + ORBX_MAX_LEVELS + 1 + 2 * 8 * (int)(sizeof(ChainPlan) / sizeof(int)), "include/orbx_dev.h and orbx_size_plan.h disagree");
+static_assert(ORBX_DEBUG_PYR_RECORDS_INTS == 2 + 6 * ORBX_MAX_LEVELS && sizeof(PyrColRec) == 16, "include/orbx_dev_pyr.h and orbx_size_plan.h disagree");
 static_assert(ORBX_DEBUG_PLAN_INPUT_INTS == ORBX_PLAN_INPUT_INTS && ORBX_DEBUG_CHUNK_PLAN_INTS == ORBX_CHUNK_PLAN_INTS, "include/orbx_dev.h and orbx_plan.h disagree");
 extern "C" int orbx_debug_plan_chunk(const int32_t *in, int n_in, int32_t *out, int n_out) {
     PlanInput pi;
@@ -1264,6 +1279,46 @@
     std::copy((const int *)sp.chains, (const int *)sp.chains + 2 * 8 * 8, o);
     return ORBX_OK;
 }
+extern "C" int orbx_debug_pyr_records(orbx_extractor_t *h, int nfeatures, float scale_factor, int nlevels, int w, int hgt, uint32_t *cols, int cols_cap,
+                                      uint32_t *bands, int bands_cap, int32_t *index, int n_index) {
+    if (!index || n_index != ORBX_DEBUG_PYR_RECORDS_INTS || cols_cap < 0 || bands_cap < 0 || (cols_cap > 0 && !cols) || (bands_cap > 0 && !bands)) {
+        orbx_set_error("orbx_debug_pyr_records: bad arguments");
+        return ORBX_ERR_ARG;
+    }
+    PyrRecords built;
+    const PyrRecords *pr = &built;
+    if (h) {
+        if (h->pw == 0) { orbx_set_error("orbx_debug_pyr_records: the handle has no plan yet"); return ORBX_ERR_ARG; }
+        pr = &h->pr;
+    } else {
+        if (nfeatures < 1 || nlevels < 1 || nlevels > ORBX_MAX_LEVELS || !(scale_factor > 1.0f)) { orbx_set_error("orbx_debug_pyr_records: bad arguments"); return ORBX_ERR_ARG; }
+        SizeInput in = {};
+        in.w = w; in.h = hgt; in.nlevels = nlevels; in.scale_factor = scale_factor;
+        extractor_tables(nfeatures, in.scale_factor, nlevels, &in.tb);
+        SizePlan sp;
+        const int rc = plan_size(in, &sp);
+        if (rc) return rc;
+        plan_pyr_records(in, sp, &built);
+    }
+    const size_t colWords = pr->cols.size() * 4, bandWords = pr->bands.size();
+    const size_t nc = std::min((size_t)cols_cap, colWords), nb = std::min((size_t)bands_cap, bandWords);
+    if (h) {
+        ORBX_HIP(hipSetDevice(h->device));
+        if (h->last_valid) ORBX_HIP(hipStreamSynchronize(h->last_stream));
+        if (nc) ORBX_HIP(hipMemcpy(cols, h->d_pyrCols, sizeof(uint32_t) * nc, hipMemcpyDeviceToHost));
+        if (nb) ORBX_HIP(hipMemcpy(bands, h->d_pyrBands, sizeof(uint32_t) * nb, hipMemcpyDeviceToHost));
+    } else {
+        if (nc) memcpy(cols, pr->cols.data(), sizeof(uint32_t) * nc);
+        if (nb) memcpy(bands, pr->bands.data(), sizeof(uint32_t) * nb);
+    }
+    int32_t *o = index;
+    *o++ = (int32_t)colWords; *o++ = (int32_t)bandWords;
+    o = std::copy(pr->nxc, pr->nxc + ORBX_MAX_LEVELS, o);
+    o = std::copy(pr->colOff, pr->colOff + ORBX_MAX_LEVELS, o);
+    o = std::copy(pr->nbands[0], pr->nbands[0] + 2 * ORBX_MAX_LEVELS, o);
+    std::copy(pr->bandOff[0], pr->bandOff[0] + 2 * ORBX_MAX_LEVELS, o);
+    return ORBX_OK;
+}
 extern "C" int orbx_debug_last_plan(const orbx_extractor_t *h, int32_t *out, int n_out) {
     if (!h || !out || n_out != ORBX_CHUNK_PLAN_INTS || !h->last_valid) { orbx_set_error("orbx_debug_last_plan: bad arguments or no call yet"); return ORBX_ERR_ARG; }
     memcpy(out, &h->lastPlan, sizeof(h->lastPlan));
diff --git a/orb_slam2v2-1_amd/csrc/orbx_extract_dev.h b/orb_slam2v2-1_amd/csrc/orbx_extract_dev.h
--- a/orb_slam2v2-1_amd/csrc/orbx_extract_dev.h
+++ b/orb_slam2v2-1_amd/csrc/orbx_extract_dev.h
@@ -81,7 +81,7 @@
                                 int maxPar, int l0);
 template <int RW, int SR>
 __global__ void k_pyr_level(uint8_t *pyr, size_t pyrImgBytes, const LevelGeom *geom, int l, const int32_t *tab, int nxc,
-                            int nbands);
+                            int nbands, const PyrColRec *cols, const uint32_t *bands, uint32_t rcpNxc, uint32_t rcpNbx);
 template <bool FULL>
 __global__ void k_pyr_pad(const uint8_t *img, int sstride, size_t simg, uint8_t *pyr, size_t pyrImgBytes, const LevelGeom *geom,
                           int l0);
diff --git a/orb_slam2v2-1_amd/csrc/orbx_internal.h b/orb_slam2v2-1_amd/csrc/orbx_internal.h
--- a/orb_slam2v2-1_amd/csrc/orbx_internal.h
+++ b/orb_slam2v2-1_amd/csrc/orbx_internal.h
@@ -57,6 +57,8 @@
     uint32_t *d_octPart, *d_octLeaf, *d_octBest; int32_t *d_octState;
     LevelGeom *d_geom;
     int32_t *d_tab;
+    PyrRecords pr;
+    PyrColRec *d_pyrCols; uint32_t *d_pyrBands;
     uint8_t *d_pyr;
     uint32_t *d_cellCnt, *d_cellRaw, *d_slots, *d_cand, *d_lvlKp;
     uint16_t *d_nodeOf;
diff --git a/orb_slam2v2-1_amd/csrc/orbx_pyramid.hip b/orb_slam2v2-1_amd/csrc/orbx_pyramid.hip
--- a/orb_slam2v2-1_amd/csrc/orbx_pyramid.hip
+++ b/orb_slam2v2-1_amd/csrc/orbx_pyramid.hip
@@ -117,74 +117,70 @@
 
 
 __device__ __forceinline__ uint32_t vmulhi24(uint32_t a, uint32_t b) { return __umulhi(a & 0xFFFFFFu, b & 0xFFFFFFu); }
+__device__ __forceinline__ uint32_t udiv_rcp(uint32_t n, uint32_t d, uint32_t m) {
+    const uint32_t q = __umulhi(n, m);
+    return n - q * d >= d ? q + 1 : q;
+}
 template <int RW, int SR>
 __global__ __launch_bounds__(256) void k_pyr_level(uint8_t *__restrict__ pyr, size_t pyrImgBytes,
                                                    const LevelGeom *__restrict__ geom, int l,
-                                                   const int32_t *__restrict__ tab, int nxc, int nbands) {
-    static_assert((RW == 8 || RW == 16) && SR <= 32, "row table: one lane per output row, a 32-bit mask of source rows");
-    constexpr int RWM = RW - 1;
-    int bx, b;
-    xcd_block_map(bx, b);
-    const int wave = __builtin_amdgcn_readfirstlane(bx * 4 + (threadIdx.x >> 6)), lane = threadIdx.x & 63;
+                                                   const int32_t *__restrict__ tab, int nxc, int nbands,
+                                                   const PyrColRec *__restrict__ cols, const uint32_t *__restrict__ bands,
+                                                   uint32_t rcpNxc, uint32_t rcpNbx) {
+    static_assert((RW == 8 || RW == 16) && SR <= 32, "a 32-bit mask of source rows");
+    constexpr int BW = PYR_BAND_HEAD + SR;
+    const uint32_t nbx = gridDim.x, total = nbx * gridDim.y, lin = blockIdx.y * nbx + blockIdx.x;
+    const uint32_t xcd = lin & 7u, pos = xcd * (total >> 3) + min(xcd, total & 7u) + (lin >> 3);
+    const uint32_t b = udiv_rcp(pos, nbx, rcpNbx), bx = pos - b * nbx;
+    const int wave = __builtin_amdgcn_readfirstlane((int)(bx * 4 + (threadIdx.x >> 6))), lane = threadIdx.x & 63;
     if (wave >= nxc * nbands) return;
-    const int band = wave / nxc, xc = wave - band * nxc;
+    const int band = (int)udiv_rcp((uint32_t)wave, (uint32_t)nxc, rcpNxc), xc = wave - band * nxc;
+    const uint4 cr = ((const uint4 *)(cols + xc * 64))[lane];
+    const uint32_t vrec = (bands + (uint32_t)band * (uint32_t)BW)[lane];
+#define PYR_REC(i) ((uint32_t)__builtin_amdgcn_readlane((int)vrec, (i)))
+    const int nrow = (int)PYR_REC(PYR_BAND_NROW);
+    const uint32_t mask = PYR_REC(PYR_BAND_MASK), regular = PYR_REC(PYR_BAND_REGULAR);
+    const int lastk = (int)PYR_REC(PYR_BAND_LASTK);
     const LevelGeom G = geom[l];
-    const int sw = geom[l - 1].w, sh = geom[l - 1].h, sps = geom[l - 1].pstride;
+    const int sh = geom[l - 1].h, sps = geom[l - 1].pstride;
     uint8_t *base = pyr + (size_t)b * pyrImgBytes;
     const uint8_t *srow0 = base + geom[l - 1].poff + (size_t)ORBX_EDGE * sps;
     uint8_t *drow0 = base + G.poff + (size_t)ORBX_EDGE * G.pstride + ORBX_EDGE;
-    const int x0 = xc * 128 + 2 * lane - 1, x1 = x0 + 1;
-    const bool vst = x0 < G.w;
-    const int xa = min(max(x0, 0), G.w - 1), xb = min(x1, G.w - 1);
-    const int ca = ORBX_EDGE + tab[G.xofsOff + xa], cb = ORBX_EDGE + tab[G.xofsOff + xb];
-    const uint32_t aa = (uint32_t)tab[G.xalphaOff + xa], ab = (uint32_t)tab[G.xalphaOff + xb];
-    const int A = ca & ~3;
-    const uint32_t oa = (uint32_t)(ca - A), ob = (uint32_t)(cb - A);
-    const uint32_t selA = oa | ((oa + 1) << 16) | 0x0C000C00u, selB = ob | ((ob + 1) << 16) | 0x0C000C00u;
-    (void)sw;
-    const int y0 = band * RW, nrow = min(RW, G.h - y0);
-    const int yl = min(y0 + (lane & RWM), G.h - 1);
-    const int vsy = tab[G.yofsOff + yl];
-    const uint32_t vbt = (uint32_t)tab[G.ybetaOff + yl];
-    const int rf = __builtin_amdgcn_readfirstlane(vsy);
-    const int kk = vsy + 1 - rf;
-    const int prevsy = __shfl_up(vsy, 1);
-    const bool okl = (lane & RWM) >= nrow || (rf >= 0 && vsy + 1 <= sh - 1 && kk < SR && ((lane & RWM) == 0 || vsy > prevsy));
-    constexpr unsigned long long rowLanes = (1ull << RW) - 1ull;
-    const bool regular = (__ballot(okl) & rowLanes) == rowLanes;
+    const int x0 = xc * 128 + 2 * lane - 1;
+    const bool vst = cr.y >= 0x10000u;
+    const int A = (int)cr.x;
+    const uint32_t aa = cr.z, ab = cr.w;
+    const uint32_t selA = (cr.y & 0xFFu) * 0x10001u + 0x0C010C00u, selB = ((cr.y >> 8) & 0xFFu) * 0x10001u + 0x0C010C00u;
+    const int y0 = band * RW;
     if (regular) {
-        uint32_t m = (lane & RWM) < nrow ? 1u << (kk & 31) : 0u;
-        m |= __shfl_xor(m, 1); m |= __shfl_xor(m, 2); m |= __shfl_xor(m, 4);
-        if (RW == 16) m |= __shfl_xor(m, 8);
-        const uint32_t mask = __builtin_amdgcn_readfirstlane(m);
-        const int lastk = 31 - __builtin_clz(mask | 1u);
         const orbx_buf_t srcBuf = buf_make(srow0, (uint32_t)sps * (uint32_t)(geom[l - 1].prows - ORBX_EDGE));
         const orbx_buf_t dstBuf = buf_make(base + G.poff, (uint32_t)G.pstride * (uint32_t)G.prows);
         uint2 q[SR];
+        uint32_t srow = PYR_REC(PYR_BAND_SROW);
+#pragma unroll
+        for (int k = 0; k < SR - 1; k++) {
+            if (k > 1 && k > lastk) continue;
+            q[k] = buf_load_b64(srcBuf, (uint32_t)A, srow);
+            srow += (uint32_t)sps;
+        }
+        uint32_t tpa = 0, tpb = 0;
+        uint32_t drow = PYR_REC(PYR_BAND_DROW) + (uint32_t)xc * 128u;
+        const uint32_t xoff = 2u * (uint32_t)lane;
 #pragma unroll
         for (int k = 0; k < SR; k++) {
-            if (k > lastk) continue;
-            q[k] = buf_load_b64(srcBuf, (uint32_t)A, (uint32_t)(min(rf + k, sh - 1) * sps));
-        }
-        uint32_t tpa = 0, tpb = 0;
-        int cnt = 0;
-        uint32_t drow = (uint32_t)((ORBX_EDGE + y0) * G.pstride + ORBX_EDGE - 1);
-        const uint32_t xoff = (uint32_t)(x0 + 1);
-#pragma unroll
-        for (int k = 0; k < SR; k++) {
-            if (k > lastk) continue;
+            if (k > 1 && k > lastk) continue;
             const uint32_t tca = udot2_u16(__builtin_amdgcn_perm(q[k].y, q[k].x, selA), aa) & 0x7FFF0u;
             const uint32_t tcb = udot2_u16(__builtin_amdgcn_perm(q[k].y, q[k].x, selB), ab) & 0x7FFF0u;
             if (k > 0 && ((mask >> k) & 1u)) {
-                const uint32_t bb = (uint32_t)__builtin_amdgcn_readlane((int)vbt, cnt);
-                const uint32_t b0 = (bb & 0xFFFu) << 12, b1 = ((bb >> 16) & 0xFFFu) << 12;
-                const uint32_t pa = (vmulhi24(b0, tpa) + vmulhi24(b1, tca) + 2) >> 2;
-                const uint32_t pb = (vmulhi24(b0, tpb) + vmulhi24(b1, tcb) + 2) >> 2;
-                if (vst) buf_store_b16(dstBuf, xoff, drow, (uint16_t)(pa | (pb << 8)));
+                const uint32_t bw = PYR_REC(PYR_BAND_HEAD + k), b0 = bw & 0xFFF000u, b1 = (bw & 0xFFFu) << 12;
+                const uint32_t sa = vmulhi24(b0, tpa) + vmulhi24(b1, tca) + 2;
+                uint32_t sb = vmulhi24(b0, tpb) + vmulhi24(b1, tcb) + 2;
+                asm("" : "+v"(sb));
+                if (vst) buf_store_b16(dstBuf, xoff, drow, (uint16_t)(((sb & 0x3FCu) << 6) | (sa >> 2)));
                 drow += (uint32_t)G.pstride;
-                cnt++;
             }
             tpa = tca; tpb = tcb;
+            if (k == 1 && SR - 1 <= lastk) q[SR - 1] = buf_load_b64(srcBuf, (uint32_t)A, srow);
         }
         return;
     }
@@ -216,6 +212,7 @@
         if (vst) *(uint16_t *)(drow0 + (size_t)y * G.pstride + x0) = (uint16_t)(pa | (pb << 8));
     }
 }
+#undef PYR_REC
 
 template <bool FULL>
 __global__ __launch_bounds__(256) void k_pyr_pad(const uint8_t *__restrict__ img, int sstride, size_t simg,
@@ -430,7 +427,7 @@
     }
 }
 
-template __global__ void k_pyr_level<8, 12>(uint8_t *, size_t, const LevelGeom *, int, const int32_t *, int, int);
-template __global__ void k_pyr_level<16, 22>(uint8_t *, size_t, const LevelGeom *, int, const int32_t *, int, int);
+template __global__ void k_pyr_level<8, 12>(uint8_t *, size_t, const LevelGeom *, int, const int32_t *, int, int, const PyrColRec *, const uint32_t *, uint32_t, uint32_t);
+template __global__ void k_pyr_level<16, 22>(uint8_t *, size_t, const LevelGeom *, int, const int32_t *, int, int, const PyrColRec *, const uint32_t *, uint32_t, uint32_t);
 template __global__ void k_pyr_pad<true>(const uint8_t *, int, size_t, uint8_t *, size_t, const LevelGeom *, int);
 template __global__ void k_pyr_pad<false>(const uint8_t *, int, size_t, uint8_t *, size_t, const LevelGeom *, int);
diff --git a/orb_slam2v2-1_amd/csrc/orbx_size_plan.h b/orb_slam2v2-1_amd/csrc/orbx_size_plan.h
--- a/orb_slam2v2-1_amd/csrc/orbx_size_plan.h
+++ b/orb_slam2v2-1_amd/csrc/orbx_size_plan.h
@@ -391,3 +391,80 @@
     *out = std::move(p);
     return ORBX_OK;
 }
+
+struct PyrColRec {
+    uint32_t A;
+    uint32_t sel;
+    uint32_t aa, ab;
+};
+#define PYR_BAND_HEAD 8
+enum { PYR_BAND_RF = 0, PYR_BAND_MASK = 1, PYR_BAND_LASTK = 2, PYR_BAND_NROW = 3, PYR_BAND_REGULAR = 4, PYR_BAND_DROW = 5, PYR_BAND_SROW = 6 };
+static inline int pyr_band_sr(int rw) { return rw == 16 ? 22 : 12; }
+static inline int pyr_band_words(int rw) { return PYR_BAND_HEAD + pyr_band_sr(rw); }
+struct PyrRecords {
+    std::vector<PyrColRec> cols;
+    std::vector<uint32_t> bands;
+    int nxc[ORBX_MAX_LEVELS], colOff[ORBX_MAX_LEVELS];
+    int nbands[2][ORBX_MAX_LEVELS], bandOff[2][ORBX_MAX_LEVELS];
+};
+static inline uint32_t pyr_rcp(uint32_t d) { return 0xFFFFFFFFu / std::max(d, 1u); }
+
+static inline void plan_pyr_records(const SizeInput &in, const SizePlan &sp, PyrRecords *out) {
+    PyrRecords r = {};
+    const std::vector<int32_t> &tab = sp.tab;
+    for (int l = 0; l < ORBX_MAX_LEVELS; l++) r.bandOff[0][l] = r.bandOff[1][l] = -1;
+    for (int l = 1; l < in.nlevels; l++) {
+        const LevelGeom &G = sp.geom[l], &S = sp.geom[l - 1];
+        const int nxc = (G.w + 1 + 127) / 128;
+        r.nxc[l] = nxc;
+        r.colOff[l] = (int)r.cols.size();
+        for (int j = 0; j < nxc * 64; j++) {
+            const int x0 = 2 * j - 1, x1 = x0 + 1;
+            const int xa = std::min(std::max(x0, 0), G.w - 1), xb = std::min(x1, G.w - 1);
+            const int ca = ORBX_EDGE + tab[G.xofsOff + xa], cb = ORBX_EDGE + tab[G.xofsOff + xb];
+            PyrColRec c;
+            c.A = (uint32_t)(ca & ~3);
+            c.sel = (uint32_t)(ca - (int)c.A) | ((uint32_t)(cb - (int)c.A) << 8) | (x0 < G.w ? 1u << 16 : 0u);
+            c.aa = (uint32_t)tab[G.xalphaOff + xa];
+            c.ab = (uint32_t)tab[G.xalphaOff + xb];
+            r.cols.push_back(c);
+        }
+        for (int f = 0; f < 2; f++) {
+            const int RW = f ? 16 : 8, SR = pyr_band_sr(RW), words = pyr_band_words(RW);
+            if (f == 1 && !(in.scale_factor <= 1.25f)) continue;
+            const int nb = (G.h + RW - 1) / RW;
+            r.nbands[f][l] = nb;
+            r.bandOff[f][l] = (int)r.bands.size();
+            r.bands.resize(r.bands.size() + (size_t)nb * words, 0u);
+            for (int band = 0; band < nb; band++) {
+                uint32_t *w = &r.bands[(size_t)r.bandOff[f][l] + (size_t)band * words];
+                const int y0 = band * RW, nrow = std::min(RW, G.h - y0);
+                const int rf = tab[G.yofsOff + y0];
+                bool regular = rf >= 0;
+                uint32_t mask = 0;
+                for (int i = 0; i < nrow && regular; i++) {
+                    const int sy = tab[G.yofsOff + y0 + i], kk = sy + 1 - rf;
+                    regular = sy + 1 <= S.h - 1 && kk < SR && (i == 0 || sy > tab[G.yofsOff + y0 + i - 1]);
+                    if (regular) mask |= 1u << kk;
+                }
+                w[PYR_BAND_RF] = (uint32_t)rf;
+                w[PYR_BAND_NROW] = (uint32_t)nrow;
+                w[PYR_BAND_DROW] = (uint32_t)((ORBX_EDGE + y0) * G.pstride + ORBX_EDGE - 1);
+                if (!regular) continue;
+                w[PYR_BAND_REGULAR] = 1;
+                w[PYR_BAND_MASK] = mask;
+                int lastk = 0;
+                while ((mask >> lastk) > 1u) lastk++;
+                w[PYR_BAND_LASTK] = (uint32_t)lastk;
+                w[PYR_BAND_SROW] = (uint32_t)(rf * S.pstride);
+                for (int i = 0; i < nrow; i++) {
+                    const int kk = tab[G.yofsOff + y0 + i] + 1 - rf;
+                    const uint32_t bb = (uint32_t)tab[G.ybetaOff + y0 + i];
+                    w[PYR_BAND_HEAD + kk] = ((bb & 0xFFFu) << 12) | ((bb >> 16) & 0xFFFu);
+                }
+            }
+        }
+    }
+    r.bands.resize(r.bands.size() + 64, 0u);
+    *out = std::move(r);
+}
```

Measured after the change: 122,900 frames/s, median of 6. 1.9% higher.
